# Griffan/FASTQuick

Measured on AMD Instinct MI355X. Metric: paired_150bp_reads_aligned_per_sec, higher is better.
Workload: dtype u32

## Files before the change

### fastquick_amd/csrc/fq_align.cpp

```cpp
#include <algorithm>
#include <atomic>
#include <ctime>
#include <chrono>
#include <climits>
#include <cstdint>
#include <cmath>
#include <cstdio>
#include <cstdlib>
#include <cstring>
#include <memory>
#include <string>
#include <unordered_map>
#include <mutex>
#include <thread>
#include <vector>
#include <pthread.h>
#include <sched.h>

#include "../../include/fastquick_amd.h"
#include "fq_backend.h"
#include "fq_index.h"
#include "fq_pipeline.h"
#include "fq_pool.h"
#include "fq_text_batch.h"

using std::vector;

namespace {
double now_ms() { return std::chrono::duration<double, std::milli>(std::chrono::steady_clock::now().time_since_epoch()).count(); }

int cal_maxdiff(int l, double err, double thres) {
  double elambda = exp(-l * err), sum = elambda, y = 1.0;
  int x = 1;
  for (int k = 1; k < 1000; ++k) {
    y *= l * err;
    x = (int)((unsigned)x * (unsigned)k);
    sum += elambda * y / x;
    if (1.0 - sum < thres) return k;
  }
  return 2;
}
thread_local double tl_grow = 1.0;
struct GrowScope { double prev; explicit GrowScope(double g) : prev(tl_grow) { tl_grow = g; } ~GrowScope() { tl_grow = prev; } };
inline size_t grown(size_t n) { return tl_grow > 1.0 ? (size_t)((double)n * tl_grow * 1.02) : 0; }

struct Retired {
  struct B { void *p; size_t bytes; uint64_t call; bool host; };
  std::vector<B> v;
  uint64_t call = 0;
  static constexpr size_t kRetiredMax = (size_t)6 << 30;
  size_t bytes(bool host) const { size_t t = 0; for (auto &b : v) if (b.host == host) t += b.bytes; return t; }
  void drain() { for (auto &b : v) { if (b.host) fqdev::hfree(b.p); else fqdev::dfree(b.p); } v.clear(); }
  void next_call() { ++call; if (bytes(false) > kRetiredMax || bytes(true) > kRetiredMax / 8) drain(); }
  ~Retired() { drain(); }
};
thread_local Retired *tl_retired = nullptr;
struct RetiredScope { Retired *prev; explicit RetiredScope(Retired *r) : prev(tl_retired) { tl_retired = r; } ~RetiredScope() { tl_retired = prev; } };
inline void retire(void *p, size_t bytes, bool host) {
  if (!p) return;
  if (tl_retired) tl_retired->v.push_back({p, bytes, tl_retired->call, host});
  else if (host) fqdev::hfree(p); else fqdev::dfree(p);
}
inline void *obtain(size_t bytes, bool host, size_t *got) {
  if (tl_retired) {
    int best = -1;
    for (int i = 0; i < (int)tl_retired->v.size(); ++i) {
      const Retired::B &b = tl_retired->v[(size_t)i];
      if (b.host == host && b.call < tl_retired->call && b.bytes >= bytes && b.bytes <= bytes + bytes / 2 && (best < 0 || b.bytes < tl_retired->v[(size_t)best].bytes)) best = i;
    }
    if (best >= 0) { void *q = tl_retired->v[(size_t)best].p; *got = tl_retired->v[(size_t)best].bytes; tl_retired->v.erase(tl_retired->v.begin() + best); return q; }
  }
  void *q = host ? fqdev::hmalloc(bytes) : fqdev::dmalloc(bytes);
  if (!q && tl_retired && !tl_retired->v.empty()) { tl_retired->drain(); q = host ? fqdev::hmalloc(bytes) : fqdev::dmalloc(bytes); }
  *got = bytes;
  return q;
}

template <class T> struct DevBuf {
  T *p = nullptr;
  size_t cap = 0;
  ~DevBuf() { fqdev::dfree(p); }
  bool take(size_t want) { size_t got = 0; p = (T *)obtain(want * sizeof(T), false, &got); cap = p ? got / sizeof(T) : 0; return p != nullptr; }
  static size_t slack(size_t n) { return std::max(std::min<size_t>(n / 4, (size_t)16 << 20), n / 16); }
  bool ensure(size_t n) {
    if (n <= cap) return true;
    retire(p, cap * sizeof(T), false);
    p = nullptr; cap = 0;
    if (const size_t g = grown(n)) { if (take(g + 64)) return true; }
    if (take(n + slack(n) + 64)) return true;
    return take(n);
  }
  bool ensure_roomy(size_t n) {
    if (n <= cap) return true;
    retire(p, cap * sizeof(T), false);
    p = nullptr; cap = 0;
    if (take(std::max(n + n / 8, grown(n)) + 64)) return true;
    if (take(n + n / 8 + 64)) return true;
    return take(n);
  }
  bool ensure_keep(size_t n, size_t keep) {
    if (n <= cap) return true;
    DevBuf<T> q;
    if (!q.take(std::max(n + slack(n), grown(n)) + 64) && !q.take(n + 64)) return false;
    if (keep && (fqdev::d2d(q.p, p, keep * sizeof(T)) || fqdev::sync())) return false;
    retire(p, cap * sizeof(T), false);
    p = q.p; cap = q.cap;
    q.p = nullptr; q.cap = 0;
    return true;
  }
};
}

template <class T> struct PinBuf {
  T *p = nullptr;
  size_t cap = 0;
  ~PinBuf() { fqdev::hfree(p); }
  bool take(size_t want) { size_t got = 0; p = (T *)obtain(want * sizeof(T), true, &got); cap = p ? got / sizeof(T) : 0; return p != nullptr; }
  bool ensure(size_t n) {
    if (n <= cap) return true;
    retire(p, cap * sizeof(T), true);
    p = nullptr; cap = 0;
    if (take(std::max(n + n / 4, grown(n)) + 64)) return true;
    return take(n + 64);
  }
  bool ensure_keep(size_t n, size_t keep) {
    if (n <= cap) return true;
    PinBuf<T> q;
    if (!q.take(std::max(n + n / 4, grown(n)) + 64) && !q.take(n + 64)) return false;
    if (keep) memcpy(q.p, p, keep * sizeof(T));
    retire(p, cap * sizeof(T), true);
    p = q.p; cap = q.cap;
    q.p = nullptr; q.cap = 0;
    return true;
  }
};

struct PinArena {
  struct Block { uint8_t *p; size_t cap; };
  std::vector<Block> blocks;
  size_t used = 0, total = 0;
  double last_grow = 1.0;
  struct Out { void *dst; const void *src; size_t bytes; };
  std::vector<Out> pending;
  ~PinArena() { for (auto &b : blocks) fqdev::hfree(b.p); }
  void reset() {
    pending.clear();
    if (blocks.size() > 1) {
      for (auto &b : blocks) retire(b.p, b.cap, true);
      blocks.clear();
      size_t want = std::max(total + total / 4, (size_t)((double)total * last_grow * 1.02));
      uint8_t *p = (uint8_t *)obtain(want, true, &want);
      if (p) blocks.push_back({p, want});
    }
    used = 0; total = 0; last_grow = tl_grow;
  }
  void *alloc(size_t bytes) {
    bytes = (bytes + 63) & ~(size_t)63;
    total += bytes;
    if (blocks.empty() || used + bytes > blocks.back().cap) {
      size_t cap = std::max<size_t>(std::max(bytes, grown(bytes)), (size_t)4 << 20);
      uint8_t *p = (uint8_t *)obtain(cap, true, &cap);
      if (!p) return nullptr;
      blocks.push_back({p, cap});
      used = 0;
    }
    void *r = blocks.back().p + used;
    used += bytes;
    return r;
  }
};

struct FqKnobs {
  uint32_t gap_long_pops = 256;
  int gap_long_always = 0;
  int64_t gap_skip_bound = -1;
  uint32_t gap_long_pops2 = 0;
  int64_t gap_split_hard = 0;
  int64_t gap_pipeline_min = -1;
  int gap_pipeline_segs = 8;
  int64_t gap_nogap_min = 131072;
  uint32_t gap_pool = 2048;
  int gap_no_order = 0;
  int device_turns = 2;
  int device_turn_slots = 1;
  int64_t device_turn_min = 1 << 20;
  int gap_round2_refill = 16;
  int gap_round1_refill = 0;
  int gap_round2_lane_major = 1;
  int gap_round2_waves = 2560;
  int sw_wave_max = 4096;
  int host_threads = -1;
  size_t host_par_min = 32768;
  int64_t md_mask_min = 4096;
  int64_t packed_bulk_min = -1;
  int trace = 0;
};

struct SearchBufs {
  DevBuf<int32_t> work;
  DevBuf<uint32_t> wfull; DevBuf<FqPos> prec; DevBuf<FqGapWork> winfo; DevBuf<uint8_t> bid_end;
  DevBuf<int32_t> order; DevBuf<uint32_t> order_cnt;
  DevBuf<FqAln> aln; DevBuf<uint32_t> naln, status;
  DevBuf<uint32_t> queue, heads; DevBuf<FqEntry> pool;
};

struct fq_ctx {
  FqWorkPool pool;
  const fq_index *ix = nullptr;
  fq_opts_t o{};
  FqKOpts ko{};
  FqKnobs kn;
  fqdev::State *dev = nullptr;
  int max_pairs = 0;
  int debug = 0;
  std::string err;
  fq_serial_hook before_serial = nullptr, after_serial = nullptr;
  void *hook_user = nullptr;
  bool serial_open = false, serial_done = false;
  bool stream_broken = false;
  uint64_t rng = 0;
  fq_isize_t last_ii{};
  std::unordered_map<uint64_t, vector<uint32_t>> kl_cache;
  int g_log_n[256];
  uint8_t maxdiff_lut[FQ_LMAX + 2];
  int n_pairs = 0, stride = 0;
  int in_kind = 0;
  fq_read_batch_t hb{};
  fq_packed_batch_t pb{};
  const fq_text_batch *tb = nullptr;
  PinBuf<uint8_t> p_cseq, p_cqual;
  PinBuf<int32_t> p_clen;
  PinBuf<char> p_cnames;
  DevBuf<char> d_cnames;
  vector<uint16_t> h_len_all;
  int c_stride = 0, c_name_stride = 0;
  DevBuf<uint64_t> d_head[2];
  DevBuf<uint16_t> d_hlen[2];
  DevBuf<uint8_t> d_qlast[2];
  int head_slot = 0;
  const fq_packed_batch_t *pend[2] = {nullptr, nullptr};
  uint64_t pend_serial[2] = {0, 0};
  bool is_pending(int i, const fq_packed_batch_t *b) const { return pend[i] == b && pend_serial[i] == b->serial; }
  DevBuf<uint8_t> d_body, d_pqual;
  DevBuf<uint64_t> d_exc;
  DevBuf<int32_t> d_row_map, d_crow, d_len_c, d_len_all;
  PinBuf<uint8_t> p_body, p_pqual;
  PinBuf<uint64_t> p_exc;
  PinBuf<uint16_t> p_hlen;
  DevBuf<uint16_t> d_blen;
  DevBuf<uint8_t> d_seq, d_qual, d_filtered, d_maxdiff;
  DevBuf<int32_t> d_len, d_len_trim, d_read_list, d_sidx, d_pair_list, d_counts;
  DevBuf<uint64_t> d_counters;
  std::vector<uint64_t> h_counters;
  SearchBufs sb[2];
  DevBuf<uint32_t> d_seg_cnt;
  DevBuf<FqAln> d_hits;
  DevBuf<uint64_t> d_aoff; DevBuf<uint32_t> d_an;
  DevBuf<uint64_t> d_off;
  DevBuf<FqDRec> d_rec, d_grec;
  DevBuf<uint32_t> d_nocc, d_qfirst, d_cnt[3], d_isz;
  DevBuf<uint16_t> d_ntop;
  DevBuf<uint8_t> d_enum, d_cls;
  DevBuf<uint64_t> d_row0, d_scan[3], d_rng, d_grow0;
  DevBuf<int32_t> d_list, d_refmax;
  DevBuf<fq_multi_t> d_multi, d_omulti;
  DevBuf<FqSwTask> d_swslot; DevBuf<FqSwCand> d_swcand;
  DevBuf<FqPairRead> d_greads; DevBuf<FqPairOut> d_gout;
  DevBuf<FqRefTgt> d_reftgt;
  DevBuf<uint16_t> d_cigs, d_ocig;
  DevBuf<fq_isize_t> d_iis;
  DevBuf<fq_result_t> d_orec;
  DevBuf<char> d_omd;
  PinBuf<fq_result_t> p_orec; PinBuf<uint16_t> p_ocig; PinBuf<char> p_omd; PinBuf<fq_multi_t> p_omulti;
  PinBuf<uint16_t> p_ntop; PinBuf<uint32_t> p_isz; PinBuf<int32_t> p_pairs;
  DevBuf<FqAln> d_qaln;
  DevBuf<uint32_t> d_qlen, d_pos, d_qpos, d_qrow, d_qinfo;
  DevBuf<FqPairIsize> d_pisize; DevBuf<int32_t> d_plut, d_glogn; DevBuf<uint64_t> d_pscratch;
  DevBuf<uint64_t> d_qoff;
  DevBuf<FqSwTask> d_swtask;
  DevBuf<FqSwOut> d_swout;
  DevBuf<FqRefTask> d_reftask;
  DevBuf<FqRefOut> d_refout;
  DevBuf<uint16_t> d_cig, d_cigarena;
  DevBuf<uint8_t> d_scratch;
  DevBuf<char> d_md;
  DevBuf<uint16_t> d_mdmask;
  vector<uint8_t> h_filtered;
  vector<int32_t> h_len_trim, h_sub_max;
  const int32_t *h_pair_list = nullptr;
  const FqSurvInfo *h_surv = nullptr;
  Retired retired;
  PinArena arena;
  PinBuf<int32_t> p_i32;
  PinBuf<FqSurvInfo> p_surv;
  PinBuf<uint32_t> p_u32a, p_u32b, p_pos;
  PinBuf<FqAln> p_aln;
  DevBuf<FqSurvInfo> d_surv;
  DevBuf<int32_t> d_sub_max;
  int64_t n_bases_in = 0;
  int emit_flags = 0;
  bool host_rows = true;
  DevBuf<uint8_t> d_equal; PinBuf<uint8_t> p_equal;
  DevBuf<char> d_enames; PinBuf<char> p_enames;
  DevBuf<uint32_t> d_samlen, d_sammeta; DevBuf<uint64_t> d_samoff; DevBuf<char> d_samtext;
  uint64_t sam_bytes = 0;
  bool sam_ready = false;
  fqdev::State *dev_emit[2] = {nullptr, nullptr};
  PinBuf<char> p_emit[2][2];
  fq_bam *bam = nullptr;
  DevBuf<uint32_t> d_bamlen, d_bammeta, d_zsize; DevBuf<uint64_t> d_bamoff, d_zoff; DevBuf<uint8_t> d_bamrec, d_zstage, d_bamz;
  FqBamCallOut bam_out;
  PinBuf<uint64_t> p_ztotal;
  uint32_t emit_nb = 0;
  std::mutex emit_mu;
  bool emit_pending = false;
  fq_qc *qc = nullptr;
  DevBuf<int32_t> d_qadded;
  DevBuf<uint32_t> d_istlen, d_ptcnt;
  DevBuf<uint64_t> d_istoff, d_ptoff, d_qcnt, d_dupkey;
  DevBuf<char> d_isttext; DevBuf<FqPileEntry> d_pile;
  PinBuf<uint64_t> p_qcnt, p_dupkey;
  FqQcCallOut qc_out;
  FqBatchState st;
  struct CallVecs {
    std::vector<int32_t> work, next_work;
  } cv;
  fq_stats_t stats{};
  double wait_ms = 0;
  ~fq_ctx();
};

extern "C" void fq_default_opts(fq_opts_t *o) {
  memset(o, 0, sizeof *o);
  o->s_mm = 3; o->s_gapo = 11; o->s_gape = 4;
  o->mode = FQ_MODE_GAPE | FQ_MODE_COMPREAD;
  o->indel_end_skip = 5; o->max_del_occ = 10; o->max_entries = 2000000;
  o->fnr = 0.02; o->max_diff = -1; o->max_gapo = 1; o->max_gape = 6;
  o->max_seed_diff = 2; o->seed_len = 32; o->max_top2 = 30; o->trim_qual = 0; o->filter_thresh = 3;
  o->max_isize = 500; o->force_isize = 0; o->max_occ = 100000; o->n_multi = 3; o->N_multi = 10; o->is_sw = 1;
  o->ap_prior = 1e-5; o->host_threads = 0; o->batch_pairs = 262144; o->single_end = 0; o->pad_opts = 0;
}

extern "C" const char *fq_version(void) { return "fastquick_amd 0.1 (gfx950)"; }
extern "C" const char *fq_ctx_last_error(const fq_ctx_t *c) { return c ? c->err.c_str() : "null context"; }

extern "C" int fq_ctx_create(const fq_index_t *ix, const fq_opts_t *opts, int32_t max_pairs, fq_ctx_t **out) {
  if (!ix || !opts || !out || max_pairs <= 0) return FQ_EINVAL;
  *out = nullptr;
  const fq_opts_t &o = *opts;
  if (o.max_gapo < 0 || o.max_gapo > 3 || o.max_gape < 0 || o.max_gape > 15 || o.seed_len < 1 || o.seed_len > FQ_SEED_MAX) return FQ_EINVAL;
  if (o.s_mm <= 0 || o.s_gapo <= 0 || o.s_gape <= 0) return FQ_EINVAL;
  if (o.fnr <= 0.0 && (o.max_diff < 0 || o.max_diff > 30)) return FQ_EINVAL;
  if (o.batch_pairs < 1) return FQ_EINVAL;
  if (o.max_seed_diff < 0 || o.max_seed_diff > 30) return FQ_EINVAL;
  if (o.max_entries < 1 || o.max_entries > (1 << 30)) return FQ_EINVAL;
  if (o.max_occ > (1u << 30) || o.n_multi < 0 || o.N_multi < 0 || o.n_multi > 4096 || o.N_multi > 4096) return FQ_EINVAL;
  std::unique_ptr<fq_ctx> c(new fq_ctx);
  c->ix = ix; c->o = o; c->max_pairs = max_pairs;
  int md_max = 0;
  for (int l = 0; l <= FQ_LMAX; ++l) {
    int md = o.fnr > 0.0 ? cal_maxdiff(l, 0.02, o.fnr) : o.max_diff;
    if (md > 30) return FQ_EINVAL;
    c->maxdiff_lut[l] = (uint8_t)md;
    md_max = std::max(md_max, md);
  }
  if ((md_max + 1) * o.s_mm + o.max_gapo * o.s_gapo + o.max_gape * o.s_gape >= FQ_MAX_BUCKETS) return FQ_EINVAL;
  if (o.max_gapo > c->maxdiff_lut[FQ_LMIN]) return FQ_EINVAL;
  c->g_log_n[0] = 0;
  for (int i = 1; i < 256; ++i) c->g_log_n[i] = (int)(4.343 * log(i) + 0.5);
  c->rng = ((uint64_t)ix->seed << 16) | 0x330EULL;
  c->last_ii.avg = -1.0;
  FqKOpts &k = c->ko;
  k.s_mm = o.s_mm; k.s_gapo = o.s_gapo; k.s_gape = o.s_gape; k.mode = o.mode;
  k.indel_end_skip = o.indel_end_skip; k.max_del_occ = o.max_del_occ; k.max_entries = o.max_entries;
  k.max_gapo = o.max_gapo; k.max_gape = o.max_gape; k.max_seed_diff = o.max_seed_diff; k.seed_len = o.seed_len;
  k.max_top2 = o.max_top2; k.trim_qual = o.trim_qual; k.filter_thresh = o.filter_thresh; k.n_buckets = FQ_MAX_BUCKETS;
  if (const char *e = getenv("FASTQUICK_CTX_TRACE")) c->kn.trace = atoi(e);
  c->dev = fqdev::state_create(ix->device);
  if (!c->dev || fqdev::bind(c->dev)) return FQ_ENODEV;
  if (!c->d_maxdiff.ensure(FQ_LMAX + 2) || !c->d_counters.ensure(FQ_C_STRIPES * FQ_C_STRIDE) || !c->d_counts.ensure(4) || !c->sb[0].queue.ensure(4) || !c->d_glogn.ensure(256)) return FQ_ENOMEM;
  if (fqdev::h2d(c->d_maxdiff.p, c->maxdiff_lut, FQ_LMAX + 2) || fqdev::h2d(c->d_glogn.p, c->g_log_n, 256 * 4) || fqdev::dzero(c->d_counters.p, (size_t)FQ_C_STRIPES * FQ_C_STRIDE * 8) || fqdev::sync()) return FQ_ENODEV;
  *out = c.release();
  return FQ_OK;
}
fq_ctx::~fq_ctx() { for (auto *e : dev_emit) if (e) fqdev::state_destroy(e); fqdev::state_destroy(dev); }
extern "C" void fq_ctx_destroy(fq_ctx_t *c) { delete c; }

extern "C" int fq_ctx_set_tuning(fq_ctx_t *c, const char *key, int64_t v) {
  if (!c || !key) return FQ_EINVAL;
  const std::string k = key;
  fqdev::Tune *t = fqdev::tune(c->dev);
  if (k == "gap_long_pops") c->kn.gap_long_pops = (uint32_t)v;
  else if (k == "gap_long_always") c->kn.gap_long_always = (int)v;
  else if (k == "gap_pool") c->kn.gap_pool = (uint32_t)v;
  else if (k == "gap_nogap_min") c->kn.gap_nogap_min = v;
  else if (k == "gap_pipeline_min") c->kn.gap_pipeline_min = v;
  else if (k == "gap_pipeline_segs") c->kn.gap_pipeline_segs = (int)std::max<int64_t>(2, std::min<int64_t>(v, 64));
  else if (k == "gap_split_hard") c->kn.gap_split_hard = v;
  else if (k == "gap_long_pops2") c->kn.gap_long_pops2 = (uint32_t)v;
  else if (k == "gap_skip_bound") c->kn.gap_skip_bound = v;
  else if (k == "gap_no_order") c->kn.gap_no_order = (int)v;
  else if (k == "device_turns") c->kn.device_turns = (int)v;
  else if (k == "device_turn_min") c->kn.device_turn_min = v;
  else if (k == "device_turn_slots") c->kn.device_turn_slots = (int)std::max<int64_t>(1, v);
  else if (k == "gap_round2_waves") c->kn.gap_round2_waves = (int)v;
  else if (k == "gap_round2_lane_major") c->kn.gap_round2_lane_major = (int)v;
  else if (k == "gap_round1_refill") c->kn.gap_round1_refill = (int)v;
  else if (k == "gap_round2_refill") c->kn.gap_round2_refill = (int)v;
  else if (k == "sw_wave_max") c->kn.sw_wave_max = (int)v;
  else if (k == "host_threads") c->kn.host_threads = (int)v;
  else if (k == "host_par_min") c->kn.host_par_min = (size_t)v;
  else if (k == "packed_bulk_min") c->kn.packed_bulk_min = v;
  else if (k == "md_mask_min") c->kn.md_mask_min = v;
  else if (k == "trace") c->kn.trace = (int)v;
  else if (k == "gap_order_asc") t->gap_order_asc = (int)v;
  else if (k == "gap_waves_per_cu") t->gap_waves_per_cu = (int)v;
  else if (k == "gap_coop_waves") t->gap_coop_waves = (int)v;
  else if (k == "gap_refill_min") t->gap_refill_min = (int)v;
  else if (k == "filter_no_turns") t->filter_no_turns = (int)v;
  else if (k == "prep_priority") t->prep_priority = (int)v;
  else if (k == "refine_lanes") t->refine_lanes = (int)v;
  else if (k == "gap_generic_opts") t->gap_generic_opts = (int)v;
  else if (k == "sw_serial_reverse") t->sw_serial_reverse = (int)v;
  else if (k == "width_both_strands") t->width_both_strands = (int)v;
  else if (k == "spin_sync") t->spin_sync = (int)v;
  else return FQ_EINVAL;
  return FQ_OK;
}

extern "C" void fq_stats_get(const fq_ctx_t *c, fq_stats_t *out) { if (c && out) *out = c->stats; }
extern "C" void fq_stats_reset(fq_ctx_t *c) { if (c) memset(&c->stats, 0, sizeof c->stats); }

#define CK(expr)                                                  \
  do {                                                            \
    if ((expr)) { c->err = std::string(#expr) + ": " + fqdev::last_error(); return FQ_ENODEV; } \
  } while (0)
#define CKM(expr)                                                 \
  do {                                                            \
    if (!(expr)) { c->err = std::string("out of device memory: ") + #expr; return FQ_ENOMEM; } \
  } while (0)

static int h2d_staged(fq_ctx *c, void *dst, const void *src, size_t bytes) {
  if (!bytes) return 0;
  void *p = c->arena.alloc(bytes);
  if (!p) { c->err = "out of pinned host memory"; return FQ_ENOMEM; }
  memcpy(p, src, bytes);
  if (fqdev::copy_pinned(dst, p, bytes, 1)) { c->err = std::string("h2d: ") + fqdev::last_error(); return FQ_ENODEV; }
  return 0;
}
static int d2h_staged(fq_ctx *c, void *dst, const void *src, size_t bytes) {
  if (!bytes) return 0;
  void *p = c->arena.alloc(bytes);
  if (!p) { c->err = "out of pinned host memory"; return FQ_ENOMEM; }
  if (fqdev::copy_pinned(p, src, bytes, 0)) { c->err = std::string("d2h: ") + fqdev::last_error(); return FQ_ENODEV; }
  c->arena.pending.push_back({dst, p, bytes});
  return 0;
}
static int sync_staged(fq_ctx *c) {
  const double t_wait = now_ms();
  if (fqdev::sync()) { c->err = std::string("sync: ") + fqdev::last_error(); return FQ_ENODEV; }
  c->wait_ms += now_ms() - t_wait;
  for (auto &o : c->arena.pending) memcpy(o.dst, o.src, o.bytes);
  c->arena.pending.clear();
  return 0;
}
static void fold_counters(const uint64_t *striped, uint64_t *cnt) {
  for (int k = 0; k < FQ_C_COUNT; ++k) {
    const bool is_max = k == FQ_C_MAXPOPS || k == FQ_C_MAXTRIPS;
    uint64_t v = 0;
    for (int st = 0; st < FQ_C_STRIPES; ++st) { const uint64_t x = striped[(size_t)st * FQ_C_STRIDE + k]; v = is_max ? std::max(v, x) : v + x; }
    cnt[k] = v;
  }
}
#define CKS(expr) do { const int rc_ = (expr); if (rc_) return rc_; } while (0)
static void dp_take(fq_ctx *c) {
  for (int v = 0; v < FQ_DP_COUNT; ++v) { c->stats.dp_launches[v] += fqdev::dp_launches[v]; fqdev::dp_launches[v] = 0; }
}
static int refuse_length(fq_ctx *c) { c->err = "read length outside [" + std::to_string(FQ_LMIN) + "," + std::to_string(FQ_LMAX) + "]"; return FQ_ELIMIT; }

extern "C" int fq_batch_upload(fq_ctx_t *c, const fq_read_batch_t *in) {
  if (!c || !in || in->n_pairs < 0 || !in->seq || !in->qual || !in->len) return FQ_EINVAL;
  if (in->n_pairs > c->max_pairs) { c->err = "batch larger than max_pairs_per_batch"; return FQ_ELIMIT; }
  if (fqdev::bind(c->dev)) return FQ_ENODEV;
  if (in->stride < 1 || in->stride > 4096) return FQ_EINVAL;
  const size_t n2 = (size_t)in->n_pairs * (c->o.single_end ? 1 : 2);
  int64_t nb = 0;
  for (size_t i = 0; i < n2; ++i) nb += in->len[i];
  c->n_bases_in = nb;
  for (size_t i = 0; i < n2; ++i)
    if (in->len[i] < FQ_LMIN || in->len[i] > FQ_LMAX || in->len[i] > in->stride) return refuse_length(c);
  CKM(c->d_seq.ensure((size_t)in->n_pairs * 2 * in->stride + 64));
  CKM(c->d_qual.ensure((size_t)in->n_pairs * 2 * in->stride + 64));
  CKM(c->d_len.ensure((size_t)in->n_pairs * 2 + 1));
  CK(fqdev::h2d(c->d_seq.p, in->seq, n2 * in->stride));
  CK(fqdev::h2d(c->d_qual.p, in->qual, n2 * in->stride));
  CK(fqdev::h2d(c->d_len.p, in->len, n2 * 4));
  CK(fqdev::sync());
// ... 160 lines not shown
  ii->std = sqrt(ii->std / n);
  double y;
  for (y = 1.0; y < 10.0; y += 0.01) if (.5 * erfc(y / M_SQRT2) < ap_prior / L * (y * ii->std + ii->avg)) break;
  ii->high_bayesian = (uint32_t)(y * ii->std + ii->avg + .499);
  uint64_t n_ap = 0;
  for (int i = 0; i < tot; ++i) if (is[i] > ii->high_bayesian) ++n_ap;
  ii->ap_prior = .01 * (n_ap + .01) / tot;
  if (ii->ap_prior < ap_prior) ii->ap_prior = ap_prior;
  if (std::isnan(ii->std) || p75 > 100000) { ii->low = ii->high = ii->high_bayesian = 0; ii->avg = ii->std = -1.0; }
}

void pair_penalty_lut(const fq_isize_t &ii, vector<int32_t> &lut) {
  if (!ii.high) return;
  for (uint32_t l = 0; l <= ii.high_bayesian; ++l) {
    const double v = -4.343 * log(0.5 * erfc(M_SQRT1_2 * fabs(l - ii.avg) / ii.std)) + 0.499;
    lut.push_back(v >= 2147483648.0 || v != v ? INT32_MIN : (int32_t)v);
  }
}
}

namespace {
struct EmitPlan {
  FqSamArgs sam{}; FqBamArgs bam{}; FqQcArgs qc{};
  uint64_t sam_total = 0, bam_total = 0, ist_total = 0, pt_total = 0;
};
struct Call {
  fq_ctx *c;
  EmitPlan plan_emit;
  fq_qc *gate = nullptr; uint64_t gate_ticket = 0; bool gate_entered = false, gate_left = false;
  void gate_take(fq_qc *q) { if (q) { gate = q; gate_ticket = fq_qc_gate_ticket(q); } }
  void gate_enter() { if (gate && !gate_entered) { fq_qc_gate_enter(gate, gate_ticket); gate_entered = true; } }
  void gate_leave() { if (gate && gate_entered && !gate_left) { fq_qc_gate_leave(gate); gate_left = true; } }
  void gate_release() { if (gate && !gate_left) { gate_enter(); gate_leave(); } }
  explicit Call(fq_ctx *ctx) : c(ctx), aln_off(ctx->st.aln_off), aln_n(ctx->st.aln_n) {}
  int n = 0, n2 = 0, B = 0, n_sub = 0, n_search = 0, n_surv = 0, max_len_all = 1, host_threads = 1;
  size_t par_min = 32768;
  const uint8_t *dseq = nullptr;
  int dstride = 0;
  const int32_t *dlen_trim = nullptr, *dread_list = nullptr;
  FqSamArgs emit{};
  bool emit_ready = false;
  vector<int> sub_max_len, sub_lo;
  vector<int32_t> sub_whole;
  vector<uint64_t> &aln_off;
  vector<uint32_t> &aln_n;
  FqRecArgs ra{};
  uint64_t n_q = 0, n_rows = 0;
  const uint32_t *h_pos = nullptr;
  bool have_pos = false;
  vector<fq_isize_t> iis;
  vector<FqPairIsize> pis;
  vector<int32_t> lut;
  int64_t n_host_pairs = 0;
  const int32_t *host_list = nullptr;
  const FqPairRead *host_reads = nullptr;
  const uint64_t *host_row0 = nullptr;
  uint64_t n_multi = 0, n_sw = 0, n_ref = 0, cig_used = 0;
  struct B1Plan { uint64_t *start = nullptr; size_t n_chunks = 0; uint64_t rng_end = 0; } plan;
  std::thread plan_thread;
  ~Call() { if (plan_thread.joinable()) plan_thread.join(); gate_release(); }
  double t_trace = 0, t_wall0 = 0, t_host0 = 0, t_serial1 = 0, t_host1 = 0, cpu_trace = 0, tcpu_trace = 0, w_trace = 0;
  double w_call0 = 0, w_host0 = 0, w_serial1 = 0, w_host1 = 0, cpu_call0 = 0;
  int sidx(size_t idx) const { return c->h_surv[idx].sidx; }
  const FqAln *aln_of(size_t idx, int *n_out) const {
    const int s = sidx(idx);
    if (s < 0) { *n_out = 0; return nullptr; }
    *n_out = (int)aln_n[s];
    return c->st.aln.data() + aln_off[s];
  }
  void trace(const char *label) {
    if (!c->kn.trace) return;
    const double t = now_ms();
    timespec ts;
    clock_gettime(CLOCK_PROCESS_CPUTIME_ID, &ts);
    const double cpu = 1e3 * (double)ts.tv_sec + 1e-6 * (double)ts.tv_nsec;
    clock_gettime(CLOCK_THREAD_CPUTIME_ID, &ts);
    const double tcpu = 1e3 * (double)ts.tv_sec + 1e-6 * (double)ts.tv_nsec;
    fprintf(stderr, "[fq] %-22s %8.3f ms   cpu %8.1f core-ms   this thread %6.3f ms   waited for the device %6.3f ms\n", label, t - t_trace, cpu - cpu_trace, tcpu - tcpu_trace, c->wait_ms - w_trace);
    t_trace = t; cpu_trace = cpu; tcpu_trace = tcpu; w_trace = c->wait_ms;
  }
};

struct FilterIn {
  const uint64_t *head = nullptr;
  const uint16_t *len = nullptr;
  const uint8_t *qual_last = nullptr;
  int uniform_len = 0;
  int body_stride = 0;
  const fq_text_batch *text = nullptr;
};

int stage0_filter(Call &K, const FilterIn &in) {
  fq_ctx *c = K.c;
  const int n = K.n, n2 = K.n2, n_sub = K.n_sub, B = K.B;
  const bool ascii = !in.head, se = c->o.single_end != 0, ragged = !ascii && in.uniform_len <= 0;
  const int n_in = se ? n : n2;
  const size_t n_max = (size_t)(ascii ? 1 : 3) * n_sub;
  CKM(c->d_filtered.ensure(n2 + 64) && c->d_read_list.ensure(n2) && c->d_sidx.ensure(n2) && c->d_pair_list.ensure(n) && c->d_sub_max.ensure(n_max) && (!ascii || c->d_len_trim.ensure(n2)));
  CK(fqdev::dzero(c->d_sub_max.p, n_max * 4));
  if (se) CK(fqdev::dfill(c->d_filtered.p + n, 1, (size_t)n));
  if (se && ascii) CK(fqdev::dzero(c->d_len_trim.p + n, (size_t)n * 4));
  fqdev::time_begin(FQ_K_PREP);
  if (ascii) {
    FqPrepArgs a{};
    a.ix = c->ix->dev; a.o = c->ko; a.seq = c->d_seq.p; a.qual = c->d_qual.p; a.len = c->d_len.p; a.stride = c->stride; a.n_reads = n_in;
    a.len_trim = c->d_len_trim.p; a.filtered = c->d_filtered.p; a.sub_max = c->d_sub_max.p; a.n_pairs = n; a.batch_pairs = B; a.counters = c->d_counters.p;
    CK(fqdev::launch_prep(a));
  } else {
    FqPrepPackedArgs a{};
    a.ix = c->ix->dev; a.o = c->ko; a.head = in.head; a.len = ragged ? in.len : nullptr; a.uniform_len = in.uniform_len; a.qual_last = in.qual_last; a.sub_whole = c->d_sub_max.p + n_sub;
    a.n_reads = n_in; a.filtered = c->d_filtered.p; a.sub_max = c->d_sub_max.p; a.n_pairs = n; a.batch_pairs = B; a.counters = c->d_counters.p;
    CK(fqdev::launch_prep_packed(a));
  }
  CK(fqdev::launch_compact(c->d_filtered.p, n, c->d_read_list.p, c->d_sidx.p, c->d_pair_list.p, c->d_counts.p));
  fqdev::time_end(FQ_K_PREP);
  int32_t counts[2] = {0, 0};
  c->h_sub_max.assign(n_sub, in.uniform_len);
  K.sub_whole.assign(n_sub, 0);
  std::vector<uint64_t> striped(ragged ? (size_t)FQ_C_STRIPES * FQ_C_STRIDE : 0);
  CKS(d2h_staged(c, counts, c->d_counts.p, 8));
  if (in.qual_last) CKS(d2h_staged(c, K.sub_whole.data(), c->d_sub_max.p + n_sub, (size_t)n_sub * 4));
  if (ascii || ragged) CKS(d2h_staged(c, c->h_sub_max.data(), c->d_sub_max.p, (size_t)n_sub * 4));
  if (ragged) CKS(d2h_staged(c, striped.data(), c->d_counters.p, striped.size() * 8));
  CKS(sync_staged(c));
  K.trace("  stage0: filter + compaction on the device");
  if (ragged) {
    uint64_t folded[FQ_C_COUNT];
    fold_counters(striped.data(), folded);
    if (folded[FQ_C_BADLEN]) return refuse_length(c);
    for (int sb = 0; in.body_stride && sb < n_sub; ++sb)
      if (((int64_t)c->h_sub_max[sb] + 3) / 4 > (int64_t)in.body_stride) { c->err = "a read is longer than body_stride holds"; return FQ_EINVAL; }
    c->n_bases_in = (int64_t)folded[FQ_C_BASES];
  } else if (!ascii) c->n_bases_in = (int64_t)n_in * in.uniform_len;
  K.n_search = counts[0]; K.n_surv = counts[1];
  K.dstride = ascii ? c->stride : (std::max(1, *std::max_element(c->h_sub_max.begin(), c->h_sub_max.end())) + 15) & ~15;
  return FQ_OK;
}

int stage0_debug_fetch(fq_ctx *c, int n2, const int32_t *d_len_all) {
  c->h_filtered.clear(); c->h_len_trim.clear();
  if (!c->debug) return FQ_OK;
  c->h_filtered.resize(n2);
  CKS(d2h_staged(c, c->h_filtered.data(), c->d_filtered.p, n2));
  if (d_len_all) { c->h_len_trim.resize(n2); CKS(d2h_staged(c, c->h_len_trim.data(), d_len_all, (size_t)n2 * 4)); }
  return FQ_OK;
}
int stage0_survivors(Call &K, bool compact, int32_t *crow) {
  fq_ctx *c = K.c;
  const int n_surv = K.n_surv;
  const size_t nrow = (size_t)n_surv * 2;
  CKM(c->d_surv.ensure(nrow + 1));
  if (compact) {
    CKM(c->d_row_map.ensure(nrow + 1) && c->d_len_c.ensure(nrow + 1) && c->d_len_trim.ensure(nrow + 1));
    CK(fqdev::launch_surv_map(c->d_pair_list.p, n_surv, K.n, c->d_filtered.p, c->d_sidx.p, c->d_surv.p, c->d_row_map.p, c->d_read_list.p, crow));
  } else CK(fqdev::launch_surv_gather(c->d_pair_list.p, n_surv, K.n, c->d_len_trim.p, c->d_filtered.p, c->d_sidx.p, c->d_surv.p));
  if (!compact) CKS(stage0_debug_fetch(c, K.n2, c->d_len_trim.p));
  CKM(c->p_pairs.ensure((size_t)n_surv + 1) && c->p_surv.ensure(nrow + 1));
  CK(fqdev::copy_pinned(c->p_pairs.p, c->d_pair_list.p, (size_t)n_surv * 4, 0));
  CK(fqdev::copy_pinned(c->p_surv.p, c->d_surv.p, nrow * sizeof(FqSurvInfo), 0));
  CKS(sync_staged(c));
  c->stats.d2h_bytes += (size_t)n_surv * (4 + 2 * sizeof(FqSurvInfo));
  c->h_pair_list = c->p_pairs.p; c->h_surv = c->p_surv.p;
  K.sub_lo.assign(K.n_sub + 1, 0);
  for (int sb = 0; sb <= K.n_sub; ++sb)
    K.sub_lo[sb] = (int)(std::lower_bound(c->h_pair_list, c->h_pair_list + n_surv, (int32_t)std::min<int64_t>((int64_t)sb * K.B, INT32_MAX)) - c->h_pair_list);
  K.sub_lo[K.n_sub] = n_surv;
  K.trace("  stage0: survivors' lists D2H");
  return FQ_OK;
}

FqTrimArgs stage0_trim_args(const Call &K, const uint8_t *qual, int qual_stride, const int32_t *row_map) {
  fq_ctx *c = K.c;
  FqTrimArgs ta{};
  ta.o = c->ko; ta.qual = qual; ta.qual_stride = qual_stride; ta.row_map = row_map; ta.len = c->d_len_c.p; ta.n_rows = 2 * K.n_surv; ta.len_trim = c->d_len_trim.p;
  ta.pair_list = c->d_pair_list.p; ta.batch_pairs = K.B; ta.sub_max = c->d_sub_max.p + 2 * K.n_sub;
  return ta;
}

int head_upload(fq_ctx *c, const fq_packed_batch_t *b, int slot) {
  const size_t n2 = (size_t)b->n_pairs * (b->single_end ? 1 : 2);
  CKM(c->d_head[slot].ensure(n2 * 3 + 8));
  CK(fqdev::h2d_copy(c->d_head[slot].p, b->head, n2 * 24));
  c->stats.h2d_bytes += n2 * 24;
  if (!b->uniform_len) {
    CKM(c->d_hlen[slot].ensure(n2 + 8));
    CK(fqdev::h2d_copy(c->d_hlen[slot].p, b->len, n2 * 2));
    c->stats.h2d_bytes += n2 * 2;
  }
  if (c->o.trim_qual >= 1 && b->qual_last) {
    CKM(c->d_qlast[slot].ensure(n2 + 8));
    CK(fqdev::h2d_copy(c->d_qlast[slot].p, b->qual_last, n2));
    c->stats.h2d_bytes += n2;
  }
  CK(fqdev::copy_record(slot));
  return FQ_OK;
}
int stage0_rows_packed(Call &K, bool bulk) {
  fq_ctx *c = K.c;
  const fq_packed_batch_t &pb = c->pb;
  const int n = K.n, n2 = K.n2, nrow = 2 * K.n_surv, body_stride = pb.body_stride, cstride = K.dstride;
  const bool se = c->o.single_end != 0, ragged = pb.uniform_len <= 0, trim = c->o.trim_qual >= 1;
  CKM(c->d_seq.ensure((size_t)nrow * cstride + 64));
  FqUnpackArgs ua{};
  ua.body_stride = body_stride; ua.uniform_len = pb.uniform_len; ua.n_rows = nrow; ua.seq = c->d_seq.p; ua.stride = cstride;
  ua.len_out = c->d_len_c.p; ua.len_trim = c->d_len_trim.p;
  FqPatchArgs pa{};
  pa.seq = c->d_seq.p; pa.stride = cstride;
  FqTrimArgs ta = stage0_trim_args(K, nullptr, pb.qual_stride, nullptr);
  if (nrow && bulk) {
    CKM(c->d_body.ensure((size_t)n2 * body_stride + 64));
    CK(fqdev::h2d(c->d_body.p, pb.body, (size_t)n2 * body_stride));
    c->stats.h2d_bytes += (size_t)n2 * body_stride;
    ua.body = c->d_body.p; ua.row_map = c->d_row_map.p;
    if (ragged) ua.len = c->d_hlen[c->head_slot].p;
    if (pb.n_exc) {
      CKM(c->d_exc.ensure((size_t)pb.n_exc + 1));
      CK(fqdev::h2d(c->d_exc.p, pb.exc, (size_t)pb.n_exc * 8));
      c->stats.h2d_bytes += (size_t)pb.n_exc * 8;
      pa.exc = c->d_exc.p; pa.n_exc = pb.n_exc; pa.crow_of = c->d_crow.p;
    }
    if (trim) {
      CKM(c->d_pqual.ensure((size_t)n2 * pb.qual_stride + 64));
      CK(fqdev::h2d(c->d_pqual.p, pb.qual, (size_t)n2 * pb.qual_stride));
      c->stats.h2d_bytes += (size_t)n2 * pb.qual_stride;
      ta.qual = c->d_pqual.p; ta.row_map = c->d_row_map.p;
    }
  } else if (nrow) {
    CKM(c->p_body.ensure((size_t)nrow * body_stride + 64) && c->d_body.ensure((size_t)nrow * body_stride + 64));
    const bool row_lens = ragged || se;
    if (row_lens) CKM(c->p_hlen.ensure((size_t)nrow + 8) && c->d_blen.ensure((size_t)nrow + 8));
    if (trim) CKM(c->p_pqual.ensure((size_t)nrow * pb.qual_stride + 64) && c->d_pqual.ensure((size_t)nrow * pb.qual_stride + 64));
    size_t ne = 0;
    vector<std::pair<size_t, size_t>> erange;
    if (pb.n_exc) erange.resize(nrow);
    for (int t = 0; t < nrow; ++t) {
      const size_t r = (size_t)(t & 1) * (size_t)n + (size_t)c->h_pair_list[t >> 1];
      if (se && (t & 1)) {
        memset(c->p_body.p + (size_t)t * body_stride, 0, (size_t)body_stride);
        c->p_hlen.p[t] = 0;
        if (trim) memset(c->p_pqual.p + (size_t)t * pb.qual_stride, 0, (size_t)pb.qual_stride);
        if (pb.n_exc) erange[t] = {0, 0};
        continue;
      }
      memcpy(c->p_body.p + (size_t)t * body_stride, pb.body + r * (size_t)body_stride, (size_t)body_stride);
      if (row_lens) c->p_hlen.p[t] = ragged ? pb.len[r] : (uint16_t)pb.uniform_len;
      if (trim) memcpy(c->p_pqual.p + (size_t)t * pb.qual_stride, pb.qual + r * (size_t)pb.qual_stride, (size_t)pb.qual_stride);
      if (pb.n_exc) {
        const uint64_t *lo = std::lower_bound(pb.exc, pb.exc + pb.n_exc, (uint64_t)r << 32);
        const uint64_t *hi = std::lower_bound(lo, pb.exc + pb.n_exc, (uint64_t)(r + 1) << 32);
        erange[t] = {(size_t)(lo - pb.exc), (size_t)(hi - pb.exc)};
        ne += (size_t)(hi - lo);
      }
    }
    CK(fqdev::copy_pinned(c->d_body.p, c->p_body.p, (size_t)nrow * body_stride, 1));
    c->stats.h2d_bytes += (size_t)nrow * body_stride;
    ua.body = c->d_body.p; ua.row_map = nullptr;
    if (row_lens) { CK(fqdev::copy_pinned(c->d_blen.p, c->p_hlen.p, (size_t)nrow * 2, 1)); ua.len = c->d_blen.p; c->stats.h2d_bytes += (size_t)nrow * 2; }
    if (ne) {
      CKM(c->p_exc.ensure(ne + 1) && c->d_exc.ensure(ne + 1));
      size_t at = 0;
      for (int t = 0; t < nrow; ++t)
        for (size_t q = erange[t].first; q < erange[t].second; ++q) c->p_exc.p[at++] = ((uint64_t)t << 32) | (pb.exc[q] & 0xffffffffull);
      CK(fqdev::copy_pinned(c->d_exc.p, c->p_exc.p, ne * 8, 1));
      c->stats.h2d_bytes += ne * 8;
      pa.exc = c->d_exc.p; pa.n_exc = (int64_t)ne; pa.crow_of = nullptr;
    }
    if (trim) {
      CK(fqdev::copy_pinned(c->d_pqual.p, c->p_pqual.p, (size_t)nrow * pb.qual_stride, 1));
      c->stats.h2d_bytes += (size_t)nrow * pb.qual_stride;
      ta.qual = c->d_pqual.p; ta.row_map = nullptr;
    }
  }
  fqdev::time_begin(FQ_K_PREP);
  if (nrow) {
    CK(fqdev::launch_unpack(ua));
    if (pa.n_exc) CK(fqdev::launch_patch(pa));
    if (trim) CK(fqdev::launch_trim(ta));
  }
  fqdev::time_end(FQ_K_PREP);
  return FQ_OK;
}

int stage0_rows_text(Call &K) {
  fq_ctx *c = K.c;
  const fq_text_batch &tb = *c->tb;
  const int nrow = 2 * K.n_surv, ns = tb.name_stride, cstride = K.dstride;
  c->c_stride = cstride; c->c_name_stride = ns;
  CKM(c->d_seq.ensure((size_t)nrow * cstride + 64) && c->d_pqual.ensure((size_t)nrow * cstride + 64) && c->d_cnames.ensure((size_t)nrow * ns + 64));
  const bool host_rows = !(c->emit_flags & FQ_EMIT_DEVICE_ONLY) || c->debug;
  c->host_rows = host_rows;
  if (host_rows) CKM(c->p_cseq.ensure((size_t)nrow * cstride + 64) && c->p_cqual.ensure((size_t)nrow * cstride + 64) && c->p_clen.ensure((size_t)nrow + 8) && c->p_cnames.ensure((size_t)nrow * ns + 64));
  fqdev::time_begin(FQ_K_PREP);
  if (nrow) {
    FqTextGatherArgs g{};
    g.text[0] = tb.d_text[0]; g.text[1] = tb.d_text[1]; g.rec = tb.d_rec; g.names = tb.d_names; g.name_stride = ns; g.n_pairs = K.n; g.single_end = c->o.single_end ? 1 : 0;
    g.pair_list = c->d_pair_list.p; g.n_out = nrow; g.seq = c->d_seq.p; g.qual = c->d_pqual.p; g.stride = cstride;
    g.len_out = c->d_len_c.p; g.len_trim = c->d_len_trim.p; g.names_out = c->d_cnames.p;
    CK(fqdev::launch_text_gather(g));
    if (c->o.trim_qual >= 1) CK(fqdev::launch_trim(stage0_trim_args(K, c->d_pqual.p, cstride, nullptr)));
    if (host_rows) {
      CK(fqdev::copy_pinned(c->p_cseq.p, c->d_seq.p, (size_t)nrow * cstride, 0));
      CK(fqdev::copy_pinned(c->p_cqual.p, c->d_pqual.p, (size_t)nrow * cstride, 0));
      CK(fqdev::copy_pinned(c->p_clen.p, c->d_len_c.p, (size_t)nrow * 4, 0));
      CK(fqdev::copy_pinned(c->p_cnames.p, c->d_cnames.p, (size_t)nrow * ns, 0));
      c->stats.d2h_bytes += (size_t)nrow * (2 * (size_t)cstride + 4 + (size_t)ns);
    }
  }
  fqdev::time_end(FQ_K_PREP);
  return FQ_OK;
}

int stage0_whole_batch(Call &K, const FilterIn &in) {
  fq_ctx *c = K.c;
  const fq_text_batch *tb = in.text;
  const int n = K.n, n2 = K.n2, n_sub = K.n_sub, nrow = 2 * K.n_surv;
  const bool se = c->o.single_end != 0, ragged = in.uniform_len <= 0, trim = c->o.trim_qual >= 1;
  const int n_in = se ? n : n2;
  bool need_all = trim && (tb || c->debug);
  if (trim && !tb) {
    vector<int32_t> surv_max(n_sub, 0);
    if (nrow) {
      CKS(d2h_staged(c, surv_max.data(), c->d_sub_max.p + 2 * n_sub, (size_t)n_sub * 4));
      CKS(sync_staged(c));
      c->stats.d2h_bytes += (size_t)n_sub * 4;
    }
    for (int sb = 0; sb < n_sub; ++sb) {
      surv_max[sb] = std::max(surv_max[sb], K.sub_whole[sb]);
      if (surv_max[sb] < c->h_sub_max[sb]) need_all = true;
    }
    if (!need_all) c->h_sub_max = surv_max;
  }
  if (need_all) {
    CKM(c->d_len_all.ensure(n2));
    if (!tb) {
      CKM(c->d_pqual.ensure((size_t)n_in * c->pb.qual_stride + 64));
      CK(fqdev::h2d(c->d_pqual.p, c->pb.qual, (size_t)n_in * c->pb.qual_stride));
      c->stats.h2d_bytes += (size_t)n_in * c->pb.qual_stride;
    }
    CK(fqdev::dzero(c->d_sub_max.p, (size_t)n_sub * 4));
    if (se) CK(fqdev::dzero(c->d_len_all.p + n, (size_t)n * 4));
    if (tb) {
      FqTextTrimArgs aa{};
      aa.o = c->ko; aa.text[0] = tb->d_text[0]; aa.text[1] = tb->d_text[1]; aa.rec = tb->d_rec; aa.n_rows = n_in; aa.n_pairs = n; aa.batch_pairs = K.B;
      aa.len_trim = c->d_len_all.p; aa.sub_max = c->d_sub_max.p;
      CK(fqdev::launch_text_trim_all(aa));
    } else {
      FqTrimAllArgs aa{};
      aa.o = c->ko; aa.qual = c->d_pqual.p; aa.qual_stride = c->pb.qual_stride; aa.len = ragged ? in.len : nullptr; aa.uniform_len = in.uniform_len;
      aa.n_reads = n_in; aa.n_pairs = n; aa.batch_pairs = K.B; aa.len_trim = c->d_len_all.p; aa.sub_max = c->d_sub_max.p;
      CK(fqdev::launch_trim_all(aa));
    }
    CKS(d2h_staged(c, c->h_sub_max.data(), c->d_sub_max.p, (size_t)n_sub * 4));
  }
  CKS(stage0_debug_fetch(c, n2, need_all ? c->d_len_all.p : nullptr));
  if (tb) c->h_len_all.clear();
  if (tb && c->debug) { c->h_len_all.assign(n2, 0); CKS(d2h_staged(c, c->h_len_all.data(), tb->d_hlen, (size_t)n_in * 2)); }
  if (need_all || c->debug || tb) CKS(sync_staged(c));
  if (c->debug && c->h_len_trim.empty()) {
    c->h_len_trim.resize(n2);
    for (int r = 0; r < n2; ++r) c->h_len_trim[r] = r >= n_in ? 0 : tb ? (int)c->h_len_all[r] : ragged ? (int)c->pb.len[r] : in.uniform_len;
  }
  return FQ_OK;
}

void stage0_finish(Call &K) {
  fq_ctx *c = K.c;
  K.max_len_all = 1;
  K.sub_max_len.assign(K.n_sub, 1);
  for (int sb = 0; sb < K.n_sub; ++sb) {
    K.sub_max_len[sb] = std::max(1, c->h_sub_max[sb]);
    K.max_len_all = std::max(K.max_len_all, K.sub_max_len[sb]);
  }
  K.dseq = c->d_seq.p; K.dlen_trim = c->d_len_trim.p; K.dread_list = c->d_read_list.p;
}

int stage0_ascii(Call &K) {
  CKS(stage0_filter(K, FilterIn{}));
  CKS(stage0_survivors(K, false, nullptr));
  stage0_finish(K);
  return FQ_OK;
}
int stage0_packed(Call &K) {
  fq_ctx *c = K.c;
  const fq_packed_batch_t &pb = c->pb;
  const int slot = c->head_slot;
  CK(fqdev::compute_wait_copy(slot));
  FilterIn in;
  in.head = c->d_head[slot].p; in.len = c->d_hlen[slot].p; in.uniform_len = pb.uniform_len; in.body_stride = pb.body_stride;
  in.qual_last = c->o.trim_qual >= 1 && pb.qual_last ? c->d_qlast[slot].p : nullptr;
  CKS(stage0_filter(K, in));
  const int64_t bulk_min = c->kn.packed_bulk_min >= 0 ? c->kn.packed_bulk_min : (int64_t)K.n / 8;
  const bool bulk = !c->o.single_end && K.n_surv > 0 && (int64_t)K.n_surv >= bulk_min;
  const bool need_crow = bulk && pb.n_exc > 0;
  if (need_crow) { CKM(c->d_crow.ensure(K.n2)); CK(fqdev::dfill(c->d_crow.p, 0xff, (size_t)K.n2 * 4)); }
  CKS(stage0_survivors(K, true, need_crow ? c->d_crow.p : nullptr));
  CKS(stage0_rows_packed(K, bulk));
  CKS(stage0_whole_batch(K, in));
  stage0_finish(K);
  return FQ_OK;
}
int stage0_text(Call &K) {
  fq_ctx *c = K.c;
  FilterIn in;
  in.head = c->tb->d_head; in.len = c->tb->d_hlen; in.uniform_len = c->tb->uniform_len; in.text = c->tb;
  CKS(stage0_filter(K, in));
  CKS(stage0_survivors(K, true, nullptr));
  CKS(stage0_rows_text(K));
  CKS(stage0_whole_batch(K, in));
  K.trace("  stage0: rows, qualities, names gathered");
  stage0_finish(K);
  return FQ_OK;
}

struct Turn { int slots = 1; bool held = false; void take() { if (!held) { fqdev::device_turn_begin(slots); held = true; } } void drop() { if (held) { fqdev::device_turn_end(); held = false; } } ~Turn() { drop(); } };
struct SearchGeom { int Lpad, Ppad, nb_need; };

bool search_bufs_ensure(SearchBufs &b, size_t nw, const SearchGeom &g, uint32_t aln_cap) {
  return b.work.ensure(nw) && b.wfull.ensure(nw * 2 * g.Lpad) && b.prec.ensure(nw * 2 * g.Ppad) && b.winfo.ensure(nw) && b.bid_end.ensure(nw * 2) && b.order.ensure(nw) &&
         b.order_cnt.ensure(2 * FQ_ORDER_KEYS + 2) && b.aln.ensure(nw * aln_cap) && b.naln.ensure(nw) && b.status.ensure(nw);
}
int launch_widths(Call &K, SearchBufs &b, const SearchGeom &g, const int32_t *d_work, int nw, int n_hard) {
  fq_ctx *c = K.c;
  FqWidthArgs wa{};
  wa.ix = c->ix->dev; wa.o = c->ko; wa.seq = K.dseq; wa.stride = K.dstride; wa.len_trim = K.dlen_trim; wa.read_list = K.dread_list;
  wa.work = d_work; wa.n_work = nw; wa.wfull = b.wfull.p; wa.wstride = g.Lpad;
  wa.prec = b.prec.p; wa.pstride = g.Ppad; wa.winfo = b.winfo.p; wa.maxdiff_lut = c->d_maxdiff.p; wa.bid_end = b.bid_end.p; wa.counters = c->d_counters.p;
  CK(fqdev::launch_width(wa));
  CK(fqdev::launch_order(b.bid_end.p, nw, n_hard, b.order.p, b.order_cnt.p));
  return FQ_OK;
}
FqGapArgs gap_args(fq_ctx *c, const SearchBufs &b, const SearchGeom &g, const FqGapTier &T, int nw) {
  FqGapArgs ga{};
  ga.ix = c->ix->dev; ga.o = c->ko; ga.o.n_buckets = g.nb_need; ga.n_work = nw; ga.winfo = b.winfo.p;
  ga.order = c->kn.gap_no_order ? nullptr : b.order.p; ga.split = c->kn.gap_no_order ? nullptr : b.order_cnt.p + 2 * FQ_ORDER_KEYS;
  ga.wfull = b.wfull.p; ga.wstride = g.Lpad; ga.prec = b.prec.p; ga.pstride = g.Ppad;
  ga.pool = b.pool.p; ga.heads = b.heads.p; ga.tier = T; ga.aln = b.aln.p; ga.n_aln = b.naln.p; ga.status = b.status.p;
  ga.counters = c->d_counters.p; ga.queue = b.queue.p;
  return ga;
}

struct HitLists { const uint32_t *status; uint64_t total; };
int collect_hits(Call &K, SearchBufs &b, const int32_t *wk, int nw, uint32_t aln_cap, bool room_later, Turn *turn, uint8_t *h_bid, HitLists *out) {
  fq_ctx *c = K.c;
  CK(fqdev::launch_scan(b.naln.p, c->d_off.p, (uint32_t)nw));
  CKM(c->p_u32a.ensure((size_t)nw + 2) && c->p_u32b.ensure((size_t)nw + 2));
  uint32_t *h_status = c->p_u32a.p, *h_naln = c->p_u32b.p;
  CK(fqdev::copy_pinned(h_status, b.status.p, (size_t)nw * 4, 0));
  CK(fqdev::copy_pinned(h_naln, b.naln.p, (size_t)nw * 4, 0));
  uint64_t *h_off = (uint64_t *)c->arena.alloc(((size_t)nw + 1) * 8);
  if (!h_off) { c->err = "out of pinned host memory"; return FQ_ENOMEM; }
  CK(fqdev::copy_pinned(h_off, c->d_off.p, ((size_t)nw + 1) * 8, 0));
  if (h_bid) CKS(d2h_staged(c, h_bid, b.bid_end.p, (size_t)nw * 2));
  CKS(sync_staged(c));
  if (turn) turn->drop();
  K.trace("  A: width + search kernels, counts D2H");
  const uint64_t total = h_off[nw], base = c->st.aln.n;
  const uint64_t hits_need = base + total + 1, hits_room = room_later ? hits_need + hits_need / 2 : hits_need;
  CKM(c->d_hits.ensure_keep(c->d_hits.cap >= hits_need ? hits_need : hits_room, base) && c->p_aln.ensure_keep(c->p_aln.cap >= hits_need ? hits_need : hits_room, base));
  CK(fqdev::launch_pack_aln(b.aln.p, b.naln.p, c->d_off.p, aln_cap, (uint32_t)nw, c->d_hits.p + base));
  CK(fqdev::launch_aln_index(b.work.p, b.status.p, c->d_off.p, b.naln.p, base, c->d_aoff.p, c->d_an.p, nw));
  CK(fqdev::copy_pinned(c->p_aln.p + base, c->d_hits.p + base, total * sizeof(FqAln), 0));
  CKS(sync_staged(c));
  c->st.aln.p = c->p_aln.p; c->st.aln.n = base + total;
  K.trace("  A: hit lists D2H");
  parallel_chunks((size_t)nw, K.host_threads, K.par_min, [&](size_t lo, size_t hi, int) {
    for (size_t w = lo; w < hi; ++w) {
      if (h_status[w]) continue;
      const int s = wk[w];
      K.aln_off[s] = base + h_off[w];
      K.aln_n[s] = h_naln[w];
    }
  });
  *out = {h_status, total};
  return FQ_OK;
}

int search_pipelined(Call &K, const SearchGeom &g, FqGapArgs ga, int nw, const FqGapTier &T2, uint32_t *n2, bool *piped) {
  fq_ctx *c = K.c;
  SearchBufs &b1 = c->sb[0], &b2 = c->sb[1];
  const int S = c->kn.gap_pipeline_segs;
  const size_t cap2 = std::max<size_t>(65536, (size_t)nw / 4);
  const size_t slots2 = (size_t)fqdev::gap_lane_slots(gap_args(c, b2, g, T2, (int32_t)cap2));
  *piped = search_bufs_ensure(b2, cap2, g, T2.aln_cap) && c->d_seg_cnt.ensure((size_t)S + 1) && b2.queue.ensure(4) && b2.heads.ensure(slots2 * FQ_MAX_BUCKETS) && b2.pool.ensure(slots2 * T2.pool_cap);
  if (!*piped) return FQ_OK;
  uint32_t n2_total = 0;
  CK(fqdev::dzero(c->d_seg_cnt.p, ((size_t)S + 1) * 4));
  fqdev::time_begin(FQ_K_GAP);
  bool room = true;
// ... 100 lines not shown
        ga.max_waves = waves / 2;
      }
      ga.pool = b.pool.p; ga.heads = b.heads.p;
      if (big_call) turn.take();
      uint32_t n2_total = 0;
      bool piped = false;
      const FqGapTier T2 = [&] { FqGapTier t = lane_tier; t.long_pops = 0; return t; }();
      if (T.nogap && c0 == 0 && (size_t)nw == work.size() && c->kn.gap_pipeline_min >= 0 && (int64_t)nw >= c->kn.gap_pipeline_min && nw >= 64 * c->kn.gap_pipeline_segs)
        CKS(search_pipelined(K, g, ga, nw, T2, &n2_total, &piped));
      if (!piped) {
        fqdev::time_begin(FQ_K_GAP);
        CK(fqdev::launch_gap(ga));
        fqdev::time_end(FQ_K_GAP);
      }
      vector<uint8_t> h_bid;
      if (T.nogap && c->kn.gap_split_hard > 0) h_bid.resize((size_t)nw * 2);
      HitLists h;
      CKS(collect_hits(K, b, wk, nw, T.aln_cap, true, &turn, h_bid.empty() ? nullptr : h_bid.data(), &h));
      c->stats.d2h_bytes += (size_t)nw * 8 + h.total * sizeof(FqAln);
      if (!h_bid.empty()) {
        bound_of.assign(n_search, 0);
        for (int w = 0; w < nw; ++w) bound_of[wk[w]] = std::min(h_bid[2 * w], h_bid[2 * w + 1]);
      }
      vector<char> in_round2;
      vector<int32_t> list2;
      if (n2_total) {
        list2.resize(n2_total);
        CKS(d2h_staged(c, list2.data(), c->sb[1].work.p, (size_t)n2_total * 4));
        CKS(sync_staged(c));
        in_round2.assign((size_t)n_search, 0);
        for (int32_t sidx : list2) in_round2[sidx] = 1;
      }
      {
        const int TT = std::max(1, K.host_threads);
        vector<vector<int32_t>> left((size_t)TT), left_easy((size_t)TT);
        vector<uint64_t> n_left((size_t)TT * 8, 0);
        const bool by_class = T.nogap != 0;
        parallel_chunks((size_t)nw, TT, K.par_min, [&](size_t lo, size_t hi, int t) {
          for (size_t w = lo; w < hi; ++w)
            if (h.status[w]) {
              ++n_left[(size_t)t * 8];
              if (in_round2.empty() || !in_round2[wk[w]]) (by_class && !(h.status[w] & FQ_SF_NOHIT) ? left_easy[t] : left[t]).push_back(wk[w]);
            }
        });
        for (int t = 0; t < TT; ++t) {
          c->stats.tier_retries += n_left[(size_t)t * 8];
          next_work.insert(next_work.end(), left[t].begin(), left[t].end());
          next_easy.insert(next_easy.end(), left_easy[t].begin(), left_easy[t].end());
        }
      }
      if (n2_total) {
        HitLists h2;
        CKS(collect_hits(K, c->sb[1], list2.data(), (int)n2_total, T2.aln_cap, false, nullptr, nullptr, &h2));
        c->stats.d2h_bytes += (size_t)n2_total * 20 + h2.total * sizeof(FqAln);
        for (uint32_t t = 0; t < n2_total; ++t)
          if (h2.status[t]) { next_work.push_back(list2[t]); ++c->stats.tier_retries; }
      }
    }
    n_hard = T.nogap ? next_work.size() : 0;
    next_work.insert(next_work.end(), next_easy.begin(), next_easy.end());
    work.swap(next_work);
    K.trace("  A: round bookkeeping");
  }
  if (!work.empty()) { c->err = "gap search: exact tier exhausted its pool (internal limit)"; return FQ_ELIMIT; }
  c->stats.reads_searched += n_search;
  return FQ_OK;
}

#define REC(op, n) CK(fqdev::launch_rec((op), K.ra, (int64_t)(n)))
static int fetch_u64(fq_ctx *c, uint64_t *dst, const uint64_t *src) { return d2h_staged(c, dst, src, 8); }

int stage_records(Call &K) {
  fq_ctx *c = K.c;
  const fq_opts_t &o = c->o;
  const int n_surv = K.n_surv;
  const size_t N = (size_t)n_surv * 2;
  FqRecArgs &A = K.ra;
  CKM(c->d_rec.ensure(N + 1) && c->d_nocc.ensure(N + 1) && c->d_ntop.ensure(N + 1) && c->d_enum.ensure(N + 1) && c->d_qfirst.ensure(N + 1) && c->d_row0.ensure(N + 1) &&
      c->d_cls.ensure((size_t)n_surv + 1) && c->d_isz.ensure((size_t)n_surv + 1) && c->d_cigs.ensure(64));
  for (int k = 0; k < 3; ++k) CKM(c->d_cnt[k].ensure(N + 1) && c->d_scan[k].ensure(N + 2));
  A.ix = c->ix->dev; A.n_surv = n_surv; A.n_pairs = K.n; A.batch_pairs = K.B; A.packed = c->in_kind >= 2 ? 1 : 0 ; A.single_end = o.single_end ? 1 : 0;
  A.max_occ = o.max_occ; A.multi_cap = o.single_end ? 4u : (uint32_t)std::max(o.n_multi, o.N_multi) + 1;
  A.n_multi = o.n_multi; A.N_multi = o.N_multi; A.max_isize = o.max_isize; A.s_mm = o.s_mm; A.is_sw = o.is_sw;
  A.pair_list = c->d_pair_list.p; A.surv = c->d_surv.p; A.len_trim = K.dlen_trim; A.full_len = A.packed ? c->d_len_c.p : c->d_len.p;
  A.hits = c->d_hits.p; A.aoff = c->d_aoff.p; A.an = c->d_an.p; A.maxdiff_lut = c->d_maxdiff.p; A.g_log_n = c->d_glogn.p;
  A.rec = c->d_rec.p; A.nocc = c->d_nocc.p; A.ntop = c->d_ntop.p; A.enumerated = c->d_enum.p; A.qfirst = c->d_qfirst.p; A.row0 = c->d_row0.p;
  A.pq_cnt = c->d_cnt[0].p; A.prow_cnt = c->d_cnt[1].p; A.pq = c->d_scan[0].p; A.prow = c->d_scan[1].p;
  A.counters = c->d_counters.p; A.cigs = c->d_cigs.p;
  REC(FQ_ROP_INIT, N);
  REC(FQ_ROP_NOCC, N);
  REC(FQ_ROP_ENUM_PLAN, n_surv);
  CK(fqdev::launch_scan(c->d_cnt[0].p, c->d_scan[0].p, (uint32_t)n_surv));
  CK(fqdev::launch_scan(c->d_cnt[1].p, c->d_scan[1].p, (uint32_t)n_surv));
  CKM(c->p_ntop.ensure(N + 1));
  CK(fqdev::copy_pinned(c->p_ntop.p, c->d_ntop.p, N * 2, 0));
  uint64_t tot[2] = {0, 0};
  CKS(fetch_u64(c, &tot[0], c->d_scan[0].p + n_surv));
  CKS(fetch_u64(c, &tot[1], c->d_scan[1].p + n_surv));
  CKS(sync_staged(c));
  c->stats.d2h_bytes += N * 2 + 16;
  K.n_q = tot[0]; K.n_rows = tot[1];
  if (K.n_q > 0xfffffff0ull) { c->err = "more than 2^32 hits to enumerate in one call"; return FQ_ELIMIT; }
  return FQ_OK;
}

int stage_sa_rows(Call &K) {
  fq_ctx *c = K.c;
  FqRecArgs &A = K.ra;
  const uint64_t n_q = K.n_q, rows = K.n_rows;
  CKM(c->d_qaln.ensure(n_q + 1) && c->d_qlen.ensure(n_q + 1) && c->d_qoff.ensure(n_q + 2) && c->d_pos.ensure(rows + 1) && c->d_pscratch.ensure(rows + 1));
  A.qaln = c->d_qaln.p; A.qlen = c->d_qlen.p; A.qoff = c->d_qoff.p; A.n_q = n_q; A.n_rows = rows; A.pos = c->d_pos.p; A.pscratch = c->d_pscratch.p;
  REC(FQ_ROP_ENUM_FILL, K.n_surv);
  if (rows) {
    FqSaArgs sa{};
    sa.ix = c->ix->dev; sa.aln = c->d_qaln.p; sa.aln_len = c->d_qlen.p; sa.row_off = c->d_qoff.p; sa.n_aln = (uint32_t)n_q;
    sa.n_rows = rows; sa.pos = c->d_pos.p; sa.counters = c->d_counters.p;
    fqdev::time_begin(FQ_K_SA);
    CK(fqdev::launch_sa(sa));
    fqdev::time_end(FQ_K_SA);
    c->stats.sa_rows += rows;
  }
  return FQ_OK;
}

struct Lcg48 { uint64_t a, c; };
static constexpr uint64_t kM48 = 0xFFFFFFFFFFFFULL;
static inline Lcg48 lcg_then(const Lcg48 &f, const Lcg48 &g) { return {(g.a * f.a) & kM48, (g.a * f.c + g.c) & kM48}; }
static Lcg48 lcg_pow(uint64_t n) {
  Lcg48 r{1, 0}, b{0x5DEECE66DULL, 0xBULL};
  for (; n; n >>= 1) { if (n & 1) r = lcg_then(r, b); b = lcg_then(b, b); }
  return r;
}
static uint64_t steps_to_zero(uint64_t x) {
  uint64_t n = 0;
  for (int k = 1; k <= 48; ++k) {
    const Lcg48 p = lcg_pow(n);
    const uint64_t xn = (p.a * x + p.c) & kM48;
    if (xn & ((1ULL << k) - 1)) n |= 1ULL << (k - 1);
  }
  const Lcg48 p = lcg_pow(n);
  if (((p.a * x + p.c) & kM48) != 0) return 0;
  return n ? n : (1ULL << 48);
}
void stageB1_plan(Call &K, uint64_t rng0) {
  fq_ctx *c = K.c;
  const size_t N = (size_t)K.n_surv * 2;
  const uint16_t *ntop = c->p_ntop.p;
  uint64_t *start = K.plan.start;
  const size_t per = 2 * FQ_RNG_CHUNK_PAIRS;
  constexpr uint64_t A1 = 0x5DEECE66DULL, C1 = 0xBULL, M48 = kM48, A2 = (A1 * A1) & M48, C2 = (A1 * C1 + C1) & M48;
  const Lcg48 jump = lcg_pow(2 * per);
  uint64_t to_zero = steps_to_zero(rng0);
  const bool can_jump = to_zero != 0 && per == 32;
  uint64_t x = rng0;
  auto advanced = [&](uint64_t steps) { if (to_zero) to_zero = to_zero > steps ? to_zero - steps : to_zero + (1ULL << 48) - steps; };
  for (size_t c0 = 0; c0 < N; c0 += per) {
    start[c0 / per] = x;
    const size_t c1 = std::min(N, c0 + per);
    if (can_jump && c1 - c0 == per && to_zero > 2 * per) {
      uint64_t w[8];
      memcpy(w, ntop + c0, 64);
      bool ones = true;
      for (int q = 0; q < 8; ++q) ones &= w[q] == 0x0001000100010001ULL;
      if (ones) { x = (jump.a * x + jump.c) & M48; advanced(2 * per); continue; }
    }
    for (size_t idx = c0; idx < c1; ++idx) {
      const int t = ntop[idx];
// ... 382 lines not shown
}

int snapshot_records(Call &K, vector<FqRead> &dst) {
  fq_ctx *c = K.c;
  const size_t N = (size_t)K.n_surv * 2;
  vector<FqDRec> rec(N);
  vector<fq_multi_t> multi((size_t)K.n_multi);
  vector<uint16_t> cigs((size_t)K.cig_used);
  CKS(d2h_staged(c, rec.data(), c->d_rec.p, N * sizeof(FqDRec)));
  CKS(d2h_staged(c, multi.data(), c->d_multi.p, multi.size() * sizeof(fq_multi_t)));
  CKS(d2h_staged(c, cigs.data(), c->d_cigs.p, cigs.size() * 2));
  CKS(sync_staged(c));
  dst.assign(N, FqRead());
  for (size_t i = 0; i < N; ++i) {
    const FqDRec &s = rec[i];
    FqRead &p = dst[i];
    p.r = (int)(i & 1) * K.n + c->h_pair_list[i >> 1];
    p.score = s.score; p.sa = s.sa; p.pos = s.pos; p.c1 = s.c1; p.c2 = s.c2; p.len = s.len; p.full_len = s.full_len; p.clip_len = s.clip_len;
    p.nm = (int16_t)s.nm; p.filtered = s.filtered; p.type = s.type; p.strand = s.strand; p.extra_flag = s.extra_flag;
    p.n_mm = s.n_mm; p.n_gapo = s.n_gapo; p.n_gape = s.n_gape; p.mapQ = s.mapQ; p.seQ = s.seQ; p.revived = s.revived != 0;
    p.cigar.assign(cigs.data() + (s.n_cigar ? s.cig_off : 0), cigs.data() + (s.n_cigar ? s.cig_off : 0) + s.n_cigar);
    for (uint32_t j = 0; j < s.n_multi; ++j) {
      const fq_multi_t &m = multi[s.multi_off + j];
      FqMulti q;
      q.pos = m.pos; q.gap = m.gap; q.mm = m.mm; q.strand = m.strand;
      if (m.n_cigar) q.cigar.assign(cigs.data() + m.cigar_off, cigs.data() + m.cigar_off + m.n_cigar);
      p.multi.push_back(q);
    }
  }
  return FQ_OK;
}

int emit_reads(Call &K, const uint8_t **qual, int *qual_stride, const char **names, int *name_stride) {
  fq_ctx *c = K.c;
  const size_t N = (size_t)K.n_surv * 2;
  if (c->in_kind == 3) { *qual = c->d_pqual.p; *qual_stride = c->c_stride; *names = c->d_cnames.p; *name_stride = c->c_name_stride; return FQ_OK; }
  const FqHostReads hb = fq_ctx_host_reads(c);
  if (N && !hb.has_qual()) { c->err = "SAM text on the device: the batch carries no qualities"; return FQ_EINVAL; }
  const int n = K.n;
  const bool se = c->o.single_end != 0;
  int max_len = 1, max_name = 1;
  std::vector<int> tl((size_t)std::max(1, K.host_threads), 1), tn((size_t)std::max(1, K.host_threads), 1);
  parallel_chunks(N, K.host_threads, K.par_min, [&](size_t lo, size_t hi, int t) {
    int ml = 1, mn = 1;
    for (size_t i = lo; i < hi; ++i) {
      const int e = (int)(i & 1), pair = c->h_pair_list[i >> 1];
      if (se && e) continue;
      ml = std::max(ml, hb.len((size_t)e * n + pair));
      if (hb.has_names()) mn = std::max(mn, (int)strnlen(hb.name_of(pair, e), (size_t)hb.name_stride));
    }
    tl[(size_t)t] = ml; tn[(size_t)t] = mn;
  });
  for (size_t t = 0; t < tl.size(); ++t) { max_len = std::max(max_len, tl[t]); max_name = std::max(max_name, tn[t]); }
  const int qs = (max_len + 15) & ~15, ns = (max_name + 1 + 7) & ~7;
  CKM(c->p_equal.ensure(N * qs + 64) && c->d_equal.ensure(N * qs + 64) && c->p_enames.ensure(N * ns + 64) && c->d_enames.ensure(N * ns + 64));
  parallel_chunks(N, K.host_threads, K.par_min, [&](size_t lo, size_t hi, int) {
    for (size_t i = lo; i < hi; ++i) {
      const int e = (int)(i & 1), pair = c->h_pair_list[i >> 1];
      uint8_t *q = c->p_equal.p + i * (size_t)qs;
      char *nm = c->p_enames.p + i * (size_t)ns;
      memset(nm, 0, (size_t)ns);
      if (se && e) { memset(q, 0, (size_t)qs); continue; }
      const size_t r = (size_t)e * n + pair;
      const int l = hb.len(r);
      memcpy(q, hb.qual(r), (size_t)l);
      memset(q + l, 0, (size_t)(qs - l));
      if (hb.has_names()) { const char *src = hb.name_of(pair, e); memcpy(nm, src, strnlen(src, (size_t)hb.name_stride)); }
      else nm[0] = '*';
    }
  });
  CK(fqdev::copy_pinned(c->d_equal.p, c->p_equal.p, N * qs, 1));
  CK(fqdev::copy_pinned(c->d_enames.p, c->p_enames.p, N * ns, 1));
  c->stats.h2d_bytes += N * ((size_t)qs + (size_t)ns);
  *qual = c->d_equal.p; *qual_stride = qs; *names = c->d_enames.p; *name_stride = ns;
  return FQ_OK;
}
int emit_args(Call &K, FqSamArgs &a) {
  fq_ctx *c = K.c;
  if (!K.emit_ready) {
    FqSamArgs &e = K.emit;
    e = FqSamArgs{};
    e.cg = c->ix->dev_contigs;
    e.n_surv = K.n_surv; e.n_pairs = K.n; e.packed = K.ra.packed; e.single_end = c->o.single_end; e.mode = c->o.mode; e.max_top2 = c->o.max_top2;
    e.pair_list = c->d_pair_list.p;
    e.rec = c->d_orec.p; e.cigar = c->d_ocig.p; e.md = c->d_omd.p; e.multi = c->d_omulti.p;
    e.seq = K.ra.seq; e.stride = K.ra.stride;
    CKS(emit_reads(K, &e.qual, &e.qual_stride, &e.names, &e.name_stride));
    K.emit_ready = true;
  }
  a = K.emit;
  return FQ_OK;
}
int emit_measure(Call &K) {
  fq_ctx *c = K.c;
  const size_t N = (size_t)K.n_surv * 2, P = (size_t)K.n_surv;
  EmitPlan &E = K.plan_emit;
  E = EmitPlan();
  c->sam_bytes = 0; c->sam_ready = false;
  c->bam_out = FqBamCallOut(); c->bam_out.owner = c->bam;
  c->qc_out = FqQcCallOut(); c->qc_out.owner = c->qc; c->qc_out.n_surv = K.n_surv;
  if (!N) return FQ_OK;
  if (c->emit_flags & FQ_EMIT_SAM) {
    CKS(emit_args(K, E.sam));
    CKM(c->d_samlen.ensure(N + 1) && c->d_samoff.ensure(N + 2) && c->d_sammeta.ensure(N + 1));
    E.sam.len = c->d_samlen.p; E.sam.off = c->d_samoff.p; E.sam.meta = c->d_sammeta.p;
    CK(fqdev::launch_sam(FQ_EOP_SAM_LEN, E.sam, (int64_t)N));
    CK(fqdev::launch_scan(c->d_samlen.p, c->d_samoff.p, (uint32_t)N));
    CKS(fetch_u64(c, &E.sam_total, c->d_samoff.p + N));
  }
  if (c->bam) {
    CKS(emit_args(K, E.bam.s));
    { const int rc = fq_bam_device_prepare(c->bam, &E.bam); if (rc) { c->err = "the BAM writer could not stage its tables on the device"; return rc; } }
    CKM(c->d_bamlen.ensure(N + 1) && c->d_bamoff.ensure(N + 2) && c->d_bammeta.ensure(N + 1));
    E.bam.len = c->d_bamlen.p; E.bam.off = c->d_bamoff.p; E.bam.meta = c->d_bammeta.p; E.bam.split = 1;
    CK(fqdev::launch_bam(FQ_EOP_BAM_LEN, E.bam, (int64_t)N));
    CK(fqdev::launch_scan(c->d_bamlen.p, c->d_bamoff.p, (uint32_t)N));
    CKS(fetch_u64(c, &E.bam_total, c->d_bamoff.p + N));
  }
  if (c->qc) {
    FqQcArgs &a = E.qc;
    CKS(emit_args(K, a.s));
    a.ix = c->ix->dev;
    K.gate_enter();
    { const int rc = fq_qc_device_prepare(c->qc, &a, K.n_surv); if (rc) { c->err = std::string("the QC consumer could not take the call: ") + fq_qc_last_error(c->qc); return rc; } }
    const size_t NC = (size_t)FQ_C_STRIPES * FQ_C_STRIDE;
    CKM(c->d_qadded.ensure(N + 1) && c->d_istlen.ensure(P + 1) && c->d_istoff.ensure(P + 2) && c->d_ptcnt.ensure(N + 1) && c->d_ptoff.ensure(N + 2) && c->d_qcnt.ensure(NC) && c->p_qcnt.ensure(NC));
    if (a.shard) { CKM(c->d_dupkey.ensure(P + 1) && c->p_dupkey.ensure(P + 1)); }
    CK(fqdev::dzero(c->d_qcnt.p, NC * 8));
    a.counters = c->d_qcnt.p; a.added = c->d_qadded.p; a.ist_len = c->d_istlen.p; a.ist_off = c->d_istoff.p; a.pt_cnt = c->d_ptcnt.p; a.pt_off = c->d_ptoff.p;
    a.dup_key = a.shard ? c->d_dupkey.p : nullptr;
    CK(fqdev::launch_qc(FQ_QOP_PAIR, a, (int64_t)P));
    CK(fqdev::launch_scan(c->d_istlen.p, c->d_istoff.p, (uint32_t)P));
    CK(fqdev::launch_scan(c->d_ptcnt.p, c->d_ptoff.p, (uint32_t)N));
    CKS(fetch_u64(c, &E.ist_total, c->d_istoff.p + P));
    CKS(fetch_u64(c, &E.pt_total, c->d_ptoff.p + N));
  }
  CKS(sync_staged(c));
  K.gate_leave();
  K.trace("consumers: lengths, decisions, prefix sums");
  return FQ_OK;
}
int emit_fill(Call &K) {
  fq_ctx *c = K.c;
  const size_t N = (size_t)K.n_surv * 2, P = (size_t)K.n_surv;
  EmitPlan &E = K.plan_emit;
  if (!N) {
    if (c->emit_flags & FQ_EMIT_SAM) c->sam_ready = true;
    c->bam_out.ready = c->bam != nullptr; c->qc_out.ready = c->qc != nullptr;
    return FQ_OK;
  }
  std::lock_guard<std::mutex> lk(c->emit_mu);
  if (c->emit_flags & FQ_EMIT_SAM) {
    CKM(c->d_samtext.ensure_roomy(E.sam_total + 64));
    E.sam.text = c->d_samtext.p;
    static const bool body_split = [] { const char *e = getenv("FASTQUICK_SAM_BODY"); return !(e && *e == '0'); }();
    E.sam.split = body_split ? 1 : 0;
    CK(fqdev::launch_sam(FQ_EOP_SAM_FILL, E.sam, (int64_t)N));
    if (body_split) CK(fqdev::launch_sam(FQ_EOP_SAM_BODY, E.sam, (int64_t)N));
    c->sam_bytes = E.sam_total;
    c->sam_ready = true;
  }
  if (c->bam) {
    const uint64_t total = E.bam_total;
    CKM(c->d_bamrec.ensure_roomy(total + 64));
    E.bam.out = c->d_bamrec.p;
    CK(fqdev::launch_bam(FQ_EOP_BAM_FILL, E.bam, (int64_t)N));
    CK(fqdev::launch_bam(FQ_EOP_BAM_BODY, E.bam, (int64_t)N));
// ... 32 lines not shown
  static const bool emit_sync = [] { const char *e = getenv("FASTQUICK_EMIT_SYNC"); return e && *e && *e != '0'; }();
  if (emit_sync) CKS(sync_staged(c));
  K.trace("consumers: fill kernels enqueued");
  return FQ_OK;
}

int stage_finish(Call &K, fq_result_batch_t *out) {
  fq_ctx *c = K.c;
  FqBatchState &S = c->st;
  FqRecArgs &A = K.ra;
  const int n_sub = K.n_sub, n_surv = K.n_surv;
  const size_t N = (size_t)n_surv * 2;
  S.isize_sub = K.iis;
  S.isize = K.iis[n_sub - 1];
  uint64_t cc = 0, mm = 0, xx = 0;
  if (N) {
    A.fc_cnt = c->d_cnt[0].p; A.fm_cnt = c->d_cnt[1].p; A.fx_cnt = c->d_cnt[2].p;
    A.fc_off = c->d_scan[0].p; A.fm_off = c->d_scan[1].p; A.fx_off = c->d_scan[2].p;
    REC(FQ_ROP_FLAT_COUNT, N);
    for (int k = 0; k < 3; ++k) CK(fqdev::launch_scan(c->d_cnt[k].p, c->d_scan[k].p, (uint32_t)N));
    CKS(fetch_u64(c, &cc, c->d_scan[0].p + N));
    CKS(fetch_u64(c, &mm, c->d_scan[1].p + N));
    CKS(fetch_u64(c, &xx, c->d_scan[2].p + N));
    CKS(sync_staged(c));
    if (cc > 0xffffffffull || mm > 0xfffffffeull || xx > 0xffffffffull) { c->err = "result arenas exceed 32-bit offsets"; return FQ_ELIMIT; }
  }
  const bool host_arrays = !(c->emit_flags & FQ_EMIT_DEVICE_ONLY) || c->debug;
  CKM(c->d_orec.ensure(N + 1) && c->d_ocig.ensure(cc + 1) && c->d_omd.ensure(mm + 1) && c->d_omulti.ensure(xx + 1));
  if (host_arrays) CKM(c->p_orec.ensure(N + 1) && c->p_ocig.ensure(cc + 1) && c->p_omd.ensure(mm + 1) && c->p_omulti.ensure(xx + 1));
  if (N) {
    A.o_rec = c->d_orec.p; A.o_cigar = c->d_ocig.p; A.o_md = c->d_omd.p; A.o_multi = c->d_omulti.p;
    REC(FQ_ROP_FLAT_FILL, N);
    if ((c->emit_flags & FQ_EMIT_SAM) || c->qc || c->bam) CKS(emit_measure(K));
    if (host_arrays) {
      CK(fqdev::copy_pinned(c->p_orec.p, c->d_orec.p, N * sizeof(fq_result_t), 0));
      CK(fqdev::copy_pinned(c->p_ocig.p, c->d_ocig.p, cc * 2, 0));
      CK(fqdev::copy_pinned(c->p_omd.p, c->d_omd.p, mm, 0));
      CK(fqdev::copy_pinned(c->p_omulti.p, c->d_omulti.p, xx * sizeof(fq_multi_t), 0));
      c->stats.d2h_bytes += N * sizeof(fq_result_t) + cc * 2 + mm + xx * sizeof(fq_multi_t);
    }
  }
  uint64_t cnt[FQ_C_COUNT];
  c->h_counters.resize((size_t)FQ_C_STRIPES * FQ_C_STRIDE);
  CKS(d2h_staged(c, c->h_counters.data(), c->d_counters.p, c->h_counters.size() * 8));
  CKS(sync_staged(c));
  fold_counters(c->h_counters.data(), cnt);
  CK(fqdev::dzero(c->d_counters.p, c->h_counters.size() * 8));
  if (!N && ((c->emit_flags & FQ_EMIT_SAM) || c->qc || c->bam)) CKS(emit_measure(K));
  if (host_arrays) {
    if (!cc) c->p_ocig.p[0] = 0;
    if (!mm) c->p_omd.p[0] = 0;
    if (!xx) c->p_omulti.p[0] = fq_multi_t{};
  }
  K.trace("result arrays D2H");
  if (cnt[FQ_C_ERR_DRAW0]) {
    c->err = "the drand48 stream drew exactly 0 for the first best hit of a read (once in 2^48 draws): bwa_aln2seq_core then takes no hit and the reference's "
             "record keeps the SA row of the read slot's previous occupant (libbwa/bwase.c:29-41) -- its result is undefined, and so this call is refused";
    return FQ_ELIMIT;
  }
  if (cnt[FQ_C_ERR_CIGAR]) { c->err = "refine: CIGAR longer than the device slot"; return FQ_ELIMIT; }
  if (cnt[FQ_C_ERR_MD]) { c->err = "MD string longer than the device slot"; return FQ_ELIMIT; }
  if (host_arrays) { S.rec = c->p_orec.p; S.cigar = c->p_ocig.p; S.md = c->p_omd.p; S.multi = c->p_omulti.p; }
  else { S.rec = nullptr; S.cigar = nullptr; S.md = nullptr; S.multi = nullptr; }
  S.n_both_unmapped = (int)cnt[FQ_C_UNMAPPED];
  out->n_survivors = n_surv;
  out->n_both_filtered = K.n - n_surv;
  out->n_both_unmapped = S.n_both_unmapped;
  out->pair_idx = S.pair_idx;
  out->rec = S.rec;
  out->cigar = S.cigar;
  out->md = S.md;
  out->multi = S.multi;
  out->isize = K.iis[n_sub - 1];
  out->n_sub = n_sub;
  out->isize_sub = S.isize_sub.data();
  out->n_bases = c->n_bases_in;
  fqdev::time_collect(c->stats.kernel_ms, c->stats.kernel_launches, FQ_K_COUNT);
  c->stats.occ_block_touches += cnt[FQ_C_OCC_WIDTH] + cnt[FQ_C_OCC_GAP] + cnt[FQ_C_OCC_SA];
  c->stats.gap_occ_touches += cnt[FQ_C_OCC_GAP];
  c->stats.width_occ_touches += cnt[FQ_C_OCC_WIDTH];
  c->stats.md_reads += cnt[FQ_C_MD_READS];
  c->stats.host_pairs += (uint64_t)K.n_host_pairs;
  c->stats.gap_nogap_touches += cnt[FQ_C_OCC_NOGAP];
  c->stats.filter_probes += cnt[FQ_C_PROBES];
  c->stats.stack_pops += cnt[FQ_C_POPS];
  c->stats.stack_pushes += cnt[FQ_C_PUSHES];
  if (cnt[FQ_C_MAXPOPS] > c->stats.max_pops_per_read) c->stats.max_pops_per_read = cnt[FQ_C_MAXPOPS];
  c->stats.reads_over_4k_pops += cnt[FQ_C_POPS_GT4K];
  if (cnt[FQ_C_MAXTRIPS] > c->stats.max_wave_trips) c->stats.max_wave_trips = cnt[FQ_C_MAXTRIPS];
  c->stats.wave_trips += cnt[FQ_C_SUMTRIPS];
  c->stats.lane_trips += cnt[FQ_C_LANETRIPS];
  c->stats.sa_rows += cnt[FQ_C_SA_DIRECT];
  c->stats.pairs_on_device += cnt[FQ_C_PAIRS_DEV];
  for (int k = 0; k < 16; ++k) c->stats.dbg[k] += cnt[FQ_C_DBG0 + k];
  c->stats.pairs += K.n;
  c->stats.host_ms_serial += (K.t_serial1 - K.t_host0) - (K.w_serial1 - K.w_host0);
  c->stats.host_ms_pair += (K.t_host1 - K.t_serial1) - (K.w_host1 - K.w_serial1);
  c->stats.host_ms_total += (K.t_host1 - K.t_host0) - (K.w_host1 - K.w_host0);
  c->stats.wall_ms_total += now_ms() - K.t_wall0;
  c->stats.device_wait_ms += c->wait_ms - K.w_call0;
  { timespec ts; clock_gettime(CLOCK_THREAD_CPUTIME_ID, &ts); c->stats.host_cpu_ms += 1e3 * (double)ts.tv_sec + 1e-6 * (double)ts.tv_nsec - K.cpu_call0; }
  K.trace("counters+timers");
  if ((c->emit_flags & FQ_EMIT_SAM) || c->qc || c->bam) CKS(emit_fill(K));
  return FQ_OK;
}
#undef REC

int run_call_stages(fq_ctx *c, fq_result_batch_t *out);
int run_call(fq_ctx *c, fq_result_batch_t *out) {
  c->serial_open = c->serial_done = false;
  const int rc = run_call_stages(c, out);
  if (rc && (c->before_serial || c->after_serial)) {
    c->stream_broken = true;
    if (!c->serial_open && !c->serial_done && c->before_serial) c->before_serial(c->hook_user);
    if (!c->serial_done && c->after_serial) c->after_serial(c->hook_user);
  }
  if (rc) {
    fqdev::copy_discard();
    (void)fqdev::stream_aux(0);
    (void)fqdev::dzero(c->d_counters.p, (size_t)FQ_C_STRIPES * FQ_C_STRIDE * 8);
    (void)fqdev::sync();
    (void)fqdev::copy_wait(0);
    (void)fqdev::copy_wait(1);
  }
  return rc;
}
int run_call_stages(fq_ctx *c, fq_result_batch_t *out) {
  CallInFlight in_flight(c->ix);
  Call K(c);
  K.t_trace = K.t_wall0 = now_ms();
  K.w_call0 = c->wait_ms;
  { timespec ts; clock_gettime(CLOCK_THREAD_CPUTIME_ID, &ts); K.cpu_call0 = 1e3 * (double)ts.tv_sec + 1e-6 * (double)ts.tv_nsec; }
  NodePin pin;
  struct PoolScope { FqWorkPool *prev; explicit PoolScope(FqWorkPool *p) : prev(tl_pool) { tl_pool = p; } ~PoolScope() { tl_pool = prev; } } pool_scope(&c->pool);
  (void)fqdev::stream_aux(0);
  const double grow = c->in_kind == 3 && c->tb && c->n_pairs > 0 && std::min<double>((double)c->max_pairs, (double)c->tb->pairs_behind) > (double)c->n_pairs
                          ? std::min(16.0, std::min<double>((double)c->max_pairs, (double)c->tb->pairs_behind) / (double)c->n_pairs) : 1.0;
  GrowScope grow_scope(grow);
  c->retired.next_call();
  RetiredScope retired_scope(&c->retired);
  if (c->kn.trace) { fprintf(stderr, "[fq]   arena: %zu blocks, last call used %zu bytes:", c->arena.blocks.size(), c->arena.total); for (auto &b : c->arena.blocks) fprintf(stderr, " %zu", b.cap); fprintf(stderr, "\n"); }
  c->arena.reset();
  const fq_opts_t &o = c->o;
  FqBatchState &S = c->st;
  S.clear();
  S.n_pairs = c->n_pairs;
  memset(out, 0, sizeof *out);
  out->n_pairs = c->n_pairs;
  if (c->n_pairs == 0) {
    const int rc0 = emit_measure(K);
    return rc0 ? rc0 : emit_fill(K);
  }
  K.n = c->n_pairs; K.n2 = 2 * K.n; K.B = o.batch_pairs; K.n_sub = (K.n + K.B - 1) / K.B;
  K.par_min = c->kn.host_par_min;
  K.host_threads = c->kn.host_threads >= 0 ? c->kn.host_threads : o.host_threads > 0 ? o.host_threads : default_host_threads(c->ix);
  int rc = c->in_kind == 3 ? stage0_text(K) : c->in_kind == 2 ? stage0_packed(K) : stage0_ascii(K);
  if (rc) return rc;
  S.n_surv = K.n_surv;
  S.batch_pairs = K.B;
  S.sub_lo = K.sub_lo;
  S.pair_idx = c->h_pair_list;
  S.surv = c->h_surv;
  K.trace("stage0 prep+compact");
  if ((rc = stageA_search(K))) return rc;
  K.trace("stageA width+gap");
  if ((rc = stage_records(K))) return rc;
  K.trace("records, SA plan, best-hit counts D2H");
  K.plan.n_chunks = ((size_t)K.n_surv + FQ_RNG_CHUNK_PAIRS - 1) / FQ_RNG_CHUNK_PAIRS;
  K.plan.start = (uint64_t *)c->arena.alloc((K.plan.n_chunks + 1) * 8);
  if (!K.plan.start) { c->err = "out of pinned host memory"; return FQ_ENOMEM; }
  if (!c->before_serial && (size_t)K.n_surv * 2 >= K.par_min) K.plan_thread = std::thread([&K, c] { stageB1_plan(K, c->rng); });
  if ((rc = stage_sa_rows(K))) return rc;
  K.trace("SA enumerate+kernel");
  K.t_host0 = now_ms(); K.w_host0 = c->wait_ms;
  if (c->before_serial) c->before_serial(c->hook_user);
  c->serial_open = true;
  if (c->stream_broken) { c->err = "the stream's state comes from a call that failed (on this rank or on the one before)"; return FQ_EIO; }
  if ((rc = stageB1_main_hit(K))) return rc;
  K.trace("B1 replay + main hit");
  if (o.single_end) K.iis.assign(K.n_sub, fq_isize_t{});
  else {
    stageB2_isize(K);
    c->last_ii = K.iis[K.n_sub - 1];
    if ((rc = stage_kl_cache(K))) return rc;
  }
  K.gate_take(c->qc);
  if (c->after_serial) c->after_serial(c->hook_user);
  c->serial_done = true;
  if (c->stream_broken) { c->err = "the hook that hands the stream's state on failed (fq_ctx_mark_stream_broken)"; return FQ_EIO; }
  K.t_serial1 = now_ms(); K.w_serial1 = c->wait_ms;
  K.trace("B2 isize, (k,l) cache");
  if ((rc = stageB3_pairing(K))) return rc;
  K.trace("B3 pairing+XA");
  if (c->debug && (rc = snapshot_records(K, S.stage_P))) return rc;
  if (!o.single_end && (rc = stageC_mate_sw(K))) return rc;
  K.trace("C mate SW");
  if (c->debug && (rc = snapshot_records(K, S.stage_S))) return rc;
  if ((rc = stageD_refine(K))) return rc;
  K.trace("D refine+MD");
  K.t_host1 = now_ms(); K.w_host1 = c->wait_ms;
  return stage_finish(K, out);
}
}

extern "C" int fq_host_cpus(void) { return (int)effective_cpus(); }
extern "C" int fq_runtime_configure(int hw_queues, int blocking_waits) { return fqdev::runtime_configure(hw_queues, blocking_waits); }
extern "C" int fq_device_count(void) { return fqdev::device_count(); }

extern "C" int fq_align_resident(fq_ctx_t *c, fq_result_batch_t *out) {
  if (!c || !out) return FQ_EINVAL;
  if (c->in_kind != 1) { c->err = "fq_align_resident: no batch uploaded (fq_batch_upload)"; return FQ_EINVAL; }
  if (fqdev::bind(c->dev)) return FQ_ENODEV;
  return run_call(c, out);
}

static int packed_check(fq_ctx_t *c, const fq_packed_batch_t *in) {
  if (!in || in->n_pairs < 0 || (in->n_pairs > 0 && (!in->head || !in->body || in->body_stride < 1 || (in->uniform_len <= 0 && !in->len)))) return FQ_EINVAL;
  if (in->n_exc < 0 || (in->n_exc > 0 && !in->exc)) return FQ_EINVAL;
  if (in->n_pairs > c->max_pairs) { c->err = "batch larger than max_pairs_per_batch"; return FQ_ELIMIT; }
  if (in->uniform_len > 0 && (in->uniform_len < FQ_LMIN || in->uniform_len > FQ_LMAX || (in->uniform_len + 3) / 4 > in->body_stride)) return refuse_length(c);
  if (c->o.trim_qual >= 1 && in->n_pairs > 0 && (!in->qual || in->qual_stride < 1)) { c->err = "quality trimming needs the batch's qualities"; return FQ_EINVAL; }
  if (in->n_pairs > 0 && in->qual_last && !in->qual) { c->err = "qual_last without the quality rows"; return FQ_EINVAL; }
  if ((in->single_end != 0) != (c->o.single_end != 0)) { c->err = c->o.single_end ? "a single-end context takes single-end batches (fq_pack_single_reads_into)" : "a paired-end context takes paired batches"; return FQ_EINVAL; }
  return FQ_OK;
}
extern "C" int fq_packed_prefetch(fq_ctx_t *c, const fq_packed_batch_t *next) {
  if (!c) return FQ_EINVAL;
  int rc = packed_check(c, next);
  if (rc) return rc;
  if (fqdev::bind(c->dev)) return FQ_ENODEV;
  if (next->n_pairs == 0 || c->is_pending(0, next) || c->is_pending(1, next)) return FQ_OK;
  for (int i = 0; i < 2; ++i) if (c->pend[i] == next) c->pend[i] = nullptr;
  const int slot = !c->pend[0] ? 0 : !c->pend[1] ? 1 : -1;
  if (slot < 0) return FQ_OK;
  rc = head_upload(c, next, slot);
  if (rc) return rc;
  c->pend[slot] = next; c->pend_serial[slot] = next->serial;
  return FQ_OK;
}
extern "C" int fq_packed_cancel(fq_ctx_t *c, const fq_packed_batch_t *b) {
  if (!c || !b) return FQ_EINVAL;
  for (int i = 0; i < 2; ++i)
    if (c->pend[i] == b) {
      if (fqdev::bind(c->dev)) return FQ_ENODEV;
      CK(fqdev::copy_wait(i));
      c->pend[i] = nullptr;
    }
  return FQ_OK;
}
extern "C" int fq_align_packed(fq_ctx_t *c, const fq_packed_batch_t *in, fq_result_batch_t *out) {
  if (!c || !out) return FQ_EINVAL;
  int rc = packed_check(c, in);
  if (rc) return broken_stream_call(c, rc);
  if (fqdev::bind(c->dev)) return FQ_ENODEV;
  c->pb = *in;
  c->n_pairs = in->n_pairs;
  c->in_kind = 2;
  if (in->n_pairs > 0) {
    if (c->is_pending(0, in)) { c->head_slot = 0; c->pend[0] = nullptr; }
    else if (c->is_pending(1, in)) { c->head_slot = 1; c->pend[1] = nullptr; }
    else {
      for (int i = 0; i < 2; ++i) if (c->pend[i] == in) c->pend[i] = nullptr;
      c->head_slot = !c->pend[0] ? 0 : 1;
      c->pend[c->head_slot] = nullptr;
      rc = head_upload(c, in, c->head_slot);
      if (rc) return broken_stream_call(c, rc);
    }
  }
  return run_call(c, out);
}

extern "C" int fq_stream_run(fq_ctx_t *const *ctxs, int32_t n_streams, const fq_packed_batch_t *const *const *batches, const int32_t *n_batches, const int32_t *first,
                             int32_t n_calls, int32_t flags, fq_stream_call_fn on_call, void *user, int64_t *survivors_out) {
  if (!ctxs || n_streams < 1 || !batches || !n_batches || n_calls < 0) return FQ_EINVAL;
  for (int s = 0; s < n_streams; ++s) if (!ctxs[s] || !batches[s] || n_batches[s] < 1) return FQ_EINVAL;
  for (int s = 0; s < n_streams; ++s) for (int t = 0; t < s; ++t) if (ctxs[s] == ctxs[t]) return FQ_EINVAL;
  std::vector<int> rcs((size_t)n_streams, FQ_OK);
  std::vector<int64_t> surv((size_t)n_streams, 0);
  static const bool trace_cpu = [] { const char *e = getenv("FASTQUICK_TRACE"); return e && *e && *e != '0'; }();
  std::vector<double> cpu_pre((size_t)n_streams, 0.0), cpu_call((size_t)n_streams, 0.0);
  auto thread_cpu_ms = [] { timespec ts; clock_gettime(CLOCK_THREAD_CPUTIME_ID, &ts); return 1e3 * (double)ts.tv_sec + 1e-6 * (double)ts.tv_nsec; };
  auto run = [&](int s) {
    fq_ctx_t *c = ctxs[s];
    const int nb = n_batches[s];
    int cur = (first ? first[s] : 0) % nb;
    if (cur < 0) cur += nb;
    fq_result_batch_t res;
    for (int k = 0; k < n_calls; ++k) {
      const int nxt = (cur + 1) % nb;
      int rc = FQ_OK;
      const bool pre = nxt != cur && (k + 1 < n_calls || (flags & FQ_STREAM_PREFETCH_BEYOND));
      const double c0 = trace_cpu ? thread_cpu_ms() : 0.0;
      if (pre) rc = fq_packed_prefetch(c, batches[s][nxt]);
      const double c1 = trace_cpu ? thread_cpu_ms() : 0.0;
      if (!rc) rc = fq_align_packed(c, batches[s][cur], &res);
      if (trace_cpu) { cpu_pre[(size_t)s] += c1 - c0; cpu_call[(size_t)s] += thread_cpu_ms() - c1; }
      if (!rc) { surv[(size_t)s] += res.n_survivors; if (on_call) rc = on_call(user, s, k, &res); }
      if (rc) { rcs[(size_t)s] = rc; if (pre) (void)fq_packed_cancel(c, batches[s][nxt]); return; }
      cur = nxt;
    }
  };
  std::vector<std::thread> th;
  for (int s = 1; s < n_streams; ++s) th.emplace_back(run, s);
  run(0);
  for (auto &t : th) t.join();
  if (survivors_out) for (int s = 0; s < n_streams; ++s) survivors_out[s] = surv[(size_t)s];
  if (trace_cpu && n_calls > 0) {
    double a = 0, b = 0;
    for (int s = 0; s < n_streams; ++s) { a += cpu_pre[(size_t)s]; b += cpu_call[(size_t)s]; }
    fprintf(stderr, "TRACE - fq_stream_run: %d streams x %d calls; CPU time of a stream's thread per call: prefetch %.3f ms, call %.3f ms\n", n_streams, n_calls,
            a / ((double)n_streams * n_calls), b / ((double)n_streams * n_calls));
  }
  for (int rc : rcs) if (rc) return rc;
  return FQ_OK;
}

extern "C" int fq_align_text(fq_ctx_t *c, const fq_text_batch *tb, fq_result_batch_t *out) {
  if (!c || !out || !tb) return FQ_EINVAL;
  int rc = FQ_OK;
  if (tb->n_pairs < 0 || (tb->n_pairs > 0 && (!tb->d_head || !tb->d_rec || !tb->d_text[0] || !tb->d_names))) rc = FQ_EINVAL;
  else if (tb->n_pairs > c->max_pairs) { c->err = "batch larger than max_pairs_per_batch"; rc = FQ_ELIMIT; }
  else if ((tb->single_end != 0) != (c->o.single_end != 0)) { c->err = "single-end / paired-end batch on a context of the other kind"; rc = FQ_EINVAL; }
  else if (tb->device != c->ix->device) { c->err = "the batch lives on another device than the context's index"; rc = FQ_EINVAL; }
  else if (tb->uniform_len > 0 && (tb->uniform_len < FQ_LMIN || tb->uniform_len > FQ_LMAX)) rc = refuse_length(c);
  if (rc) return broken_stream_call(c, rc);
  if (fqdev::bind(c->dev)) return FQ_ENODEV;
  c->tb = tb;
  c->n_pairs = tb->n_pairs;
  c->in_kind = 3;
  return run_call(c, out);
}

static const uint64_t kStateGood = 0x31545351465full, kStateBroken = 0x58545351465full;
extern "C" int64_t fq_ctx_state_export(const fq_ctx_t *c, void *buf, int64_t cap) {
  if (!c) return FQ_EINVAL;
  int64_t need = 8 + 8 + (int64_t)sizeof(fq_isize_t) + 8;
  for (const auto &kv : c->kl_cache) need += 16 + 4 * (int64_t)kv.second.size();
  if (!buf || cap < need) return need;
  uint8_t *p = (uint8_t *)buf;
  const uint64_t mark = c->stream_broken ? kStateBroken : kStateGood;
  memcpy(p, &mark, 8); p += 8;
  memcpy(p, &c->rng, 8); p += 8;
  memcpy(p, &c->last_ii, sizeof(fq_isize_t)); p += sizeof(fq_isize_t);
  const uint64_t n = c->kl_cache.size();
  memcpy(p, &n, 8); p += 8;
  for (const auto &kv : c->kl_cache) {
    const uint64_t m = kv.second.size();
// ... 145 lines not shown
```

### fastquick_amd/csrc/fq_backend.h

```cpp
#pragma once
#include "fq_kernels.h"
#include "fq_records.h"
#include "fq_frontend.h"
#include "fq_emit.h"
#include "fq_deflate.h"

namespace fqdev {

struct State;
struct Tune {
  int gap_coop_waves = 0;
  int gap_waves_per_cu = 0, gap_refill_min = 0, gap_order_asc = 0, filter_no_turns = 0, refine_lanes = 0;
  int spin_sync = 0;
  int gap_generic_opts = 0;
  int width_both_strands = 0;
  int prep_priority = 0;
  int sw_serial_reverse = 0;
};
int runtime_configure(int hw_queues, int blocking_waits);
int device_count();
State *state_create(int device_ordinal);
void state_destroy(State *s);
int bind(State *s);
Tune *tune(State *s);
const char *last_error();
bool is_real_gpu();
void device_turn_begin(int slots = 1);
void device_turn_end();

void *dmalloc(size_t bytes);
void dfree(void *p);
void *hmalloc(size_t bytes);
void hfree(void *p);
int h2d(void *dst, const void *src, size_t bytes);
int d2h(void *dst, const void *src, size_t bytes);
int copy_pinned(void *dst, const void *src, size_t bytes, int to_device);
int d2d(void *dst, const void *src, size_t bytes);
int dzero(void *dst, size_t bytes);
int dfill(void *dst, int byte, size_t bytes);
int sync();
int h2d_copy(void *dst, const void *src, size_t bytes);
int copy_record(int slot);
int copy_wait(int slot);
void copy_discard();
int compute_wait_copy(int slot);
int copy_flush_now();

void time_begin(int kid);
void time_end(int kid);
void time_collect(double ms[], uint64_t launches[], int n_ids);
inline thread_local uint64_t dp_launches[FQ_DP_COUNT] = {};

int launch_prep(const FqPrepArgs &a);
int launch_compact(const uint8_t *filtered, int n_pairs, int32_t *read_list, int32_t *sidx, int32_t *pair_list, int32_t *counts);
int launch_surv_gather(const int32_t *pair_list, int n_surv, int n_pairs, const int32_t *len_trim, const uint8_t *filtered, const int32_t *sidx, FqSurvInfo *out);
int launch_prep_packed(const FqPrepPackedArgs &a);
int launch_surv_map(const int32_t *pair_list, int n_surv, int n_pairs, const uint8_t *filtered, const int32_t *sidx, FqSurvInfo *out,
                    int32_t *row_map, int32_t *read_list_c, int32_t *crow_of);
int launch_unpack(const FqUnpackArgs &a);
int launch_patch(const FqPatchArgs &a);
int launch_trim(const FqTrimArgs &a);
int launch_trim_all(const FqTrimAllArgs &a);
int launch_width(const FqWidthArgs &a);
int launch_order(const uint8_t *bid_end, int n, int n_hard, int32_t *order, uint32_t *cnt);
int gap_lane_slots(const FqGapArgs &a);
int launch_gap(const FqGapArgs &a);
int launch_scan(const uint32_t *in, uint64_t *out, uint32_t n);
int launch_pack_aln(const FqAln *aln, const uint32_t *n_aln, const uint64_t *off, uint32_t cap, uint32_t n_work, FqAln *packed);
int launch_sa(const FqSaArgs &a);
int stream_aux(int on);
int stream_fork();
int stream_join();
int stream_mark(int k);
int stream_wait_mark(int k);
int launch_collect(const int32_t *order, const uint32_t *split, int n_work, int seg, int n_seg, const uint32_t *status, const int32_t *work, int32_t *out, uint32_t *count);
int launch_rec(int op, const FqRecArgs &a, int64_t n);
int launch_aln_index(const int32_t *work, const uint32_t *status, const uint64_t *off, const uint32_t *naln, uint64_t base, uint64_t *aoff, uint32_t *an, int n);
int launch_sam(int op, const FqSamArgs &a, int64_t n);
int launch_bam(int op, const FqBamArgs &a, int64_t n);
int launch_deflate(const FqDeflateArgs &a);
int launch_deflate_pack(const FqDeflatePackArgs &a);
int launch_qc(int op, const FqQcArgs &a, int64_t n);
int launch_dup_rehash(const uint64_t *old, uint64_t old_cap, uint64_t *tab, uint64_t mask);
int launch_sw(const FqSwArgs &a);
int launch_sw_serial(const FqSwArgs &a);
int launch_refine(const FqRefineArgs &a);

const FqzCrcConst *crc_const();
int launch_inflate(const FqInflateArgs &a);
int launch_inflate2(const FqInflateArgs &a, const FqInflateArgs &b);
int launch_nl_index(const uint8_t *text, uint32_t n, uint32_t lo, uint32_t *nl, uint32_t cap, uint32_t *count);
int launch_tok_rec(const FqTokArgs &a);
int launch_tok_pieces(const FqTokArgs &a);
int launch_slot_bases(const FqSlotArgs &a);
int launch_slot_names(const FqSlotArgs &a);
int launch_text_gather(const FqTextGatherArgs &a);
int launch_text_trim_all(const FqTextTrimArgs &a);
int dfill32(void *dst, uint32_t v, size_t n_words);

}
```

### fastquick_amd/csrc/fq_device.hip

```cpp
#include <hip/hip_runtime.h>
#include <hip/hip_ext.h>

#include <algorithm>
#include <condition_variable>
#include <atomic>
#include <cstdio>
#include <cstdlib>
#include <cstring>
#include <mutex>
#include <string>
#include <unordered_map>
#include <vector>
#include <sys/mman.h>
#include <sys/syscall.h>
#include <unistd.h>

#include "fq_backend.h"

namespace fqdev {

struct Pending { int kid; hipEvent_t a, b; };
struct State {
  int device = 0;
  hipStream_t stream = nullptr;
  hipStream_t main_stream = nullptr, aux_stream = nullptr;
  hipEvent_t fork_ev = nullptr, join_ev = nullptr;
  hipEvent_t marks[4] = {nullptr, nullptr, nullptr, nullptr};
  hipEvent_t prio_fork = nullptr;
  hipStream_t copy_stream = nullptr;
  hipEvent_t copy_done[2] = {nullptr, nullptr};
  hipEvent_t prep_done = nullptr;
  hipEvent_t sync_ev = nullptr;
  std::vector<Pending> pending;
  std::vector<hipEvent_t> free_events;
  hipEvent_t open_begin[16] = {};
  struct SmallCopy { uint8_t *dst; const uint8_t *src; size_t bytes; };
  SmallCopy small[8];
  int n_small = 0;
  uint64_t *scan_tmp = nullptr; size_t scan_tmp_n = 0;
  uint32_t *cmp_cnt = nullptr; uint64_t *cmp_off = nullptr; size_t cmp_n = 0;
  Tune tune;
};
static thread_local State *g_cur = nullptr;
static thread_local std::string g_err;
#define g_stream (g_cur->stream)

#define FQ_HIP(call)                                                                         \
  do {                                                                                       \
    hipError_t e_ = (call);                                                                  \
    if (e_ != hipSuccess) {                                                                  \
      g_err = std::string(#call) + ": " + hipGetErrorString(e_);                             \
      return -3;                                                                             \
    }                                                                                        \
  } while (0)

int copy_flush();
#define FQ_PRE() do { if (copy_flush()) return -3; } while (0)
void copy_discard() { if (g_cur) g_cur->n_small = 0; }
int copy_flush_now() { FQ_PRE(); return 0; }

const char *last_error() { return g_err.c_str(); }
bool is_real_gpu() { return true; }

static int set_kernel_attributes();
static std::mutex g_dev_mu;
static bool g_dev_ready[64];
static hipEvent_t g_prep_last[64];
static State *g_prep_owner[64];
static hipStream_t g_copy_streams[64][2];
static unsigned g_copy_next[64];
static std::mutex g_turn_mu[64];
static std::condition_variable g_turn_cv[64];
static int g_turn_held[64];
static int g_ctx_count[64];
static hipStream_t g_prio_stream[64];
static bool g_queue_warned = false;
static int g_rt_blocking_waits = 0;
int runtime_configure(int hw_queues, int blocking_waits) {
  if (hw_queues > 0) {
    char b[16];
    snprintf(b, sizeof b, "%d", hw_queues);
    setenv("GPU_MAX_HW_QUEUES", b, 0);
  }
  g_rt_blocking_waits = blocking_waits ? 1 : 0;
  return 0;
}

int device_count() { int n = 0; if (hipGetDeviceCount(&n) != hipSuccess) { (void)hipGetLastError(); return 0; } return n < 0 ? 0 : n; }
void device_turn_begin(int slots) {
  const int d = g_cur->device;
  std::unique_lock<std::mutex> lk(g_turn_mu[d]);
  g_turn_cv[d].wait(lk, [&] { return g_turn_held[d] < (slots < 1 ? 1 : slots); });
  ++g_turn_held[d];
}
void device_turn_end() {
  const int d = g_cur->device;
  { std::lock_guard<std::mutex> lk(g_turn_mu[d]); --g_turn_held[d]; }
  g_turn_cv[d].notify_all();
}

State *state_create(int dev) {
  int n = 0;
  if (hipGetDeviceCount(&n) != hipSuccess || n <= 0) { g_err = "no HIP device visible"; return nullptr; }
  if (dev < 0 || dev >= n || dev >= 64) { g_err = "device ordinal out of range"; return nullptr; }
  if (hipSetDevice(dev) != hipSuccess) { g_err = "hipSetDevice failed"; return nullptr; }
  g_cur = nullptr;
  {
    std::lock_guard<std::mutex> lk(g_dev_mu);
    if (!g_dev_ready[dev]) {
      if (g_rt_blocking_waits) { (void)hipSetDeviceFlags(hipDeviceScheduleBlockingSync); (void)hipGetLastError(); }
      if (set_kernel_attributes()) return nullptr;
      g_dev_ready[dev] = true;
    }
    const char *q = getenv("GPU_MAX_HW_QUEUES");
    const int queues = q && atoi(q) > 0 ? atoi(q) : 4;
    if (++g_ctx_count[dev] + 2 > queues && !g_queue_warned) {
      g_queue_warned = true;
      fprintf(stderr, "fastquick_amd: %d alignment contexts on device %d with GPU_MAX_HW_QUEUES=%d: contexts will share hardware queues and wait for each other's kernels "
                      "(fq_runtime_configure(contexts + 4, ..) or GPU_MAX_HW_QUEUES before the process makes its first HIP call)\n", g_ctx_count[dev], dev, queues);
    }
  }
  State *s = new State;
  s->device = dev;
  bool ok = hipStreamCreateWithFlags(&s->stream, hipStreamNonBlocking) == hipSuccess &&
            hipEventCreateWithFlags(&s->copy_done[0], hipEventDisableTiming | hipEventBlockingSync) == hipSuccess &&
            hipEventCreateWithFlags(&s->copy_done[1], hipEventDisableTiming | hipEventBlockingSync) == hipSuccess &&
            hipEventCreateWithFlags(&s->prep_done, hipEventDisableTiming) == hipSuccess &&
            hipEventCreateWithFlags(&s->sync_ev, hipEventDisableTiming | hipEventBlockingSync) == hipSuccess;
  if (!ok) { g_err = "stream / event creation failed"; state_destroy(s); return nullptr; }
  s->main_stream = s->stream;
  return s;
}
void state_destroy(State *s) {
  if (!s) return;
  (void)hipSetDevice(s->device);
  g_cur = nullptr;
  s->stream = s->main_stream ? s->main_stream : s->stream;
  if (s->aux_stream) { (void)hipStreamSynchronize(s->aux_stream); (void)hipStreamDestroy(s->aux_stream); }
  if (s->sync_ev) (void)hipEventDestroy(s->sync_ev);
  if (s->fork_ev) (void)hipEventDestroy(s->fork_ev);
  if (s->join_ev) (void)hipEventDestroy(s->join_ev);
  for (hipEvent_t m : s->marks) if (m) (void)hipEventDestroy(m);
  if (s->prio_fork) (void)hipEventDestroy(s->prio_fork);
  if (s->stream) (void)hipStreamSynchronize(s->stream);
  if (s->copy_stream) (void)hipStreamSynchronize(s->copy_stream);
  {
    std::lock_guard<std::mutex> lk(g_dev_mu);
    if (g_prep_owner[s->device] == s) { g_prep_owner[s->device] = nullptr; g_prep_last[s->device] = nullptr; }
    if (g_ctx_count[s->device] > 0) --g_ctx_count[s->device];
  }
  for (auto &p : s->pending) { (void)hipEventDestroy(p.a); (void)hipEventDestroy(p.b); }
  for (auto e : s->free_events) (void)hipEventDestroy(e);
  for (auto e : s->copy_done) if (e) (void)hipEventDestroy(e);
  if (s->prep_done) (void)hipEventDestroy(s->prep_done);
  if (s->scan_tmp) (void)hipFree(s->scan_tmp);
  if (s->cmp_cnt) (void)hipFree(s->cmp_cnt);
  if (s->cmp_off) (void)hipFree(s->cmp_off);
  if (s->stream) (void)hipStreamDestroy(s->stream);
  delete s;
}
Tune *tune(State *s) { return &s->tune; }
int bind(State *s) {
  if (!s) { g_err = "no device state"; return -3; }
  if (g_cur != s) { FQ_HIP(hipSetDevice(s->device)); g_cur = s; }
  return 0;
}

void *dmalloc(size_t bytes) {
  void *p = nullptr;
  if (hipMalloc(&p, bytes ? bytes : 16) != hipSuccess) { g_err = "hipMalloc failed (" + std::to_string(bytes) + " B)"; return nullptr; }
  return p;
}
void dfree(void *p) { if (p) (void)hipFree(p); }
static const size_t kRegisterMin = (size_t)4 << 20;
static std::mutex g_reg_mu;
static std::unordered_map<void *, size_t> g_registered;
static int device_numa_node(int dev) {
  static std::mutex mu;
  static std::unordered_map<int, int> cache;
  std::lock_guard<std::mutex> lk(mu);
  auto it = cache.find(dev);
  if (it != cache.end()) return it->second;
  int node = -1;
  char bus[64] = {0};
  if (hipDeviceGetPCIBusId(bus, (int)sizeof bus, dev) == hipSuccess) {
    for (char *c = bus; *c; ++c) if (*c >= 'A' && *c <= 'F') *c = (char)(*c - 'A' + 'a');
    const std::string path = std::string("/sys/bus/pci/devices/") + bus + "/numa_node";
    if (FILE *f = fopen(path.c_str(), "r")) { if (fscanf(f, "%d", &node) != 1) node = -1; fclose(f); }
  } else (void)hipGetLastError();
  cache[dev] = node;
  return node;
}
static void prefer_node(void *m, size_t len, int node) {
  if (node < 0 || node >= 1024) return;
  unsigned long mask[16] = {0};
  mask[node / (8 * sizeof(unsigned long))] |= 1ul << (node % (8 * sizeof(unsigned long)));
  (void)syscall(SYS_mbind, m, len, 1 , mask, (unsigned long)(8 * sizeof mask + 1), 0u);
}
void *hmalloc(size_t bytes) {
  static const bool use_register = [] { const char *e = getenv("FASTQUICK_PIN_REGISTER"); return !(e && *e == '0'); }();
  if (use_register && bytes >= kRegisterMin) {
    const size_t len = (bytes + ((size_t)2 << 20) - 1) & ~(((size_t)2 << 20) - 1);
    void *m = mmap(nullptr, len, PROT_READ | PROT_WRITE, MAP_PRIVATE | MAP_ANONYMOUS, -1, 0);
    if (m != MAP_FAILED) {
      (void)madvise(m, len, MADV_HUGEPAGE);
      int dev = 0;
      if (hipGetDevice(&dev) == hipSuccess) prefer_node(m, len, device_numa_node(dev)); else (void)hipGetLastError();
      if (hipHostRegister(m, len, hipHostRegisterDefault) == hipSuccess) {
        std::lock_guard<std::mutex> lk(g_reg_mu);
        g_registered[m] = len;
        return m;
      }
      (void)hipGetLastError();
      munmap(m, len);
    }
  }
  void *p = nullptr;
  if (hipHostMalloc(&p, bytes ? bytes : 16, hipHostMallocDefault) != hipSuccess) { g_err = "hipHostMalloc failed"; return nullptr; }
  return p;
}
void hfree(void *p) {
  if (!p) return;
  size_t len = 0;
  {
    std::lock_guard<std::mutex> lk(g_reg_mu);
    auto it = g_registered.find(p);
    if (it != g_registered.end()) { len = it->second; g_registered.erase(it); }
  }
  if (len) { (void)hipHostUnregister(p); munmap(p, len); }
  else (void)hipHostFree(p);
}
int h2d(void *dst, const void *src, size_t bytes) { FQ_PRE(); if (bytes) FQ_HIP(hipMemcpyAsync(dst, src, bytes, hipMemcpyHostToDevice, g_stream)); return 0; }
int d2h(void *dst, const void *src, size_t bytes) { FQ_PRE(); if (bytes) FQ_HIP(hipMemcpyAsync(dst, src, bytes, hipMemcpyDeviceToHost, g_stream)); return 0; }
int d2d(void *dst, const void *src, size_t bytes) { FQ_PRE(); if (bytes) FQ_HIP(hipMemcpyAsync(dst, src, bytes, hipMemcpyDeviceToDevice, g_stream)); return 0; }
int dzero(void *dst, size_t bytes) { FQ_PRE(); if (bytes) FQ_HIP(hipMemsetAsync(dst, 0, bytes, g_stream)); return 0; }
int dfill(void *dst, int byte, size_t bytes) { FQ_PRE(); if (bytes) FQ_HIP(hipMemsetAsync(dst, byte, bytes, g_stream)); return 0; }
int sync() {
  FQ_PRE();
  if (g_cur->tune.spin_sync || !g_cur->sync_ev) { FQ_HIP(hipStreamSynchronize(g_stream)); return 0; }
  FQ_HIP(hipEventRecord(g_cur->sync_ev, g_stream));
  FQ_HIP(hipEventSynchronize(g_cur->sync_ev));
  return 0;
}
int stream_aux(int on) {
  FQ_PRE();
  if (on && !g_cur->aux_stream) {
    FQ_HIP(hipStreamCreateWithFlags(&g_cur->aux_stream, hipStreamNonBlocking));
    FQ_HIP(hipEventCreateWithFlags(&g_cur->fork_ev, hipEventDisableTiming));
    FQ_HIP(hipEventCreateWithFlags(&g_cur->join_ev, hipEventDisableTiming));
  }
  g_cur->stream = on ? g_cur->aux_stream : g_cur->main_stream;
  return 0;
}
int stream_fork() {
  FQ_PRE();
  if (!g_cur->aux_stream) return 0;
  FQ_HIP(hipEventRecord(g_cur->fork_ev, g_cur->main_stream));
  FQ_HIP(hipStreamWaitEvent(g_cur->aux_stream, g_cur->fork_ev, 0));
  return 0;
}
int stream_join() {
  FQ_PRE();
  if (!g_cur->aux_stream) return 0;
  FQ_HIP(hipEventRecord(g_cur->join_ev, g_cur->aux_stream));
  FQ_HIP(hipStreamWaitEvent(g_cur->main_stream, g_cur->join_ev, 0));
  return 0;
}
int stream_mark(int k) {
  FQ_PRE();
  hipEvent_t &m = g_cur->marks[k & 3];
  if (!m) FQ_HIP(hipEventCreateWithFlags(&m, hipEventDisableTiming));
  FQ_HIP(hipEventRecord(m, g_stream));
  return 0;
}
int stream_wait_mark(int k) {
  FQ_PRE();
  hipEvent_t m = g_cur->marks[k & 3];
  if (m) FQ_HIP(hipStreamWaitEvent(g_stream, m, 0));
  return 0;
}
static int copy_stream_get() {
  if (g_cur->copy_stream) return 0;
  std::lock_guard<std::mutex> lk(g_dev_mu);
  const int dev = g_cur->device;
  for (int k = 0; k < 2; ++k)
    if (!g_copy_streams[dev][k]) FQ_HIP(hipStreamCreateWithFlags(&g_copy_streams[dev][k], hipStreamNonBlocking));
  g_cur->copy_stream = g_copy_streams[dev][g_copy_next[dev]++ & 1];
  return 0;
}
int h2d_copy(void *dst, const void *src, size_t bytes) {
  if (copy_stream_get()) return -3;
  if (bytes) FQ_HIP(hipMemcpyAsync(dst, src, bytes, hipMemcpyHostToDevice, g_cur->copy_stream));
  return 0;
}
int copy_record(int slot) { if (copy_stream_get()) return -3; FQ_HIP(hipEventRecord(g_cur->copy_done[slot & 1], g_cur->copy_stream)); return 0; }
int copy_wait(int slot) { FQ_HIP(hipEventSynchronize(g_cur->copy_done[slot & 1])); return 0; }
int compute_wait_copy(int slot) { FQ_PRE(); FQ_HIP(hipStreamWaitEvent(g_stream, g_cur->copy_done[slot & 1], 0)); return 0; }

struct FqCopySet { uint8_t *dst[8]; const uint8_t *src[8]; size_t bytes[8]; };
__global__ void __launch_bounds__(256) k_copy_bytes(FqCopySet cs) {
  uint8_t *dst = cs.dst[blockIdx.y];
  const uint8_t *src = cs.src[blockIdx.y];
  const size_t bytes = cs.bytes[blockIdx.y];
  const size_t n16 = ((((uintptr_t)dst | (uintptr_t)src) & 15) == 0) ? bytes / 16 : 0;
  const size_t t = (size_t)blockIdx.x * blockDim.x + threadIdx.x, stride = (size_t)gridDim.x * blockDim.x;
  for (size_t i = t; i < n16; i += stride) ((uint4 *)dst)[i] = ((const uint4 *)src)[i];
  for (size_t i = n16 * 16 + t; i < bytes; i += stride) dst[i] = src[i];
}
static const size_t kSmallCopy = (size_t)8 << 20;
int copy_flush() {
  State *s = g_cur;
  if (!s || s->n_small == 0) return 0;
  FqCopySet cs;
  size_t most = 0;
  for (int k = 0; k < 8; ++k) {
    const bool on = k < s->n_small;
    cs.dst[k] = on ? s->small[k].dst : nullptr; cs.src[k] = on ? s->small[k].src : nullptr; cs.bytes[k] = on ? s->small[k].bytes : 0;
    if (on) most = std::max(most, s->small[k].bytes);
  }
  const int n = s->n_small;
  s->n_small = 0;
  const unsigned blocks = (unsigned)std::min<size_t>(256, (most / 16 + 255) / 256 + 1);
  hipLaunchKernelGGL(k_copy_bytes, dim3(blocks, (unsigned)n), dim3(256), 0, s->stream, cs);
  FQ_HIP(hipGetLastError());
  return 0;
}
int copy_pinned(void *dst, const void *src, size_t bytes, int to_device) {
  if (!bytes) return 0;
  if (bytes > kSmallCopy) { FQ_PRE(); FQ_HIP(hipMemcpyAsync(dst, src, bytes, to_device ? hipMemcpyHostToDevice : hipMemcpyDeviceToHost, g_stream)); return 0; }
  if (g_cur->n_small == 8) FQ_PRE();
  g_cur->small[g_cur->n_small++] = {(uint8_t *)dst, (const uint8_t *)src, bytes};
  return 0;
}

static hipEvent_t get_event() {
  if (!g_cur->free_events.empty()) { hipEvent_t e = g_cur->free_events.back(); g_cur->free_events.pop_back(); return e; }
  hipEvent_t e;
  (void)hipEventCreate(&e);
  return e;
}
void time_begin(int kid) { (void)copy_flush(); hipEvent_t e = get_event(); (void)hipEventRecord(e, g_stream); g_cur->open_begin[kid] = e; }
void time_end(int kid) { (void)copy_flush(); hipEvent_t e = get_event(); (void)hipEventRecord(e, g_stream); g_cur->pending.push_back({kid, g_cur->open_begin[kid], e}); }
static void kernel_events(int kid, hipEvent_t *a, hipEvent_t *b) { *a = get_event(); *b = get_event(); g_cur->pending.push_back({kid, *a, *b}); }
void time_collect(double ms[], uint64_t launches[], int n_ids) {
  std::vector<decltype(g_cur->pending)::value_type> later;
  for (auto &p : g_cur->pending) {
    if (hipEventQuery(p.b) == hipErrorNotReady) { later.push_back(p); continue; }
    float t = 0.f;
    if (hipEventElapsedTime(&t, p.a, p.b) == hipSuccess && p.kid < n_ids) { ms[p.kid] += t; launches[p.kid] += 1; }
    g_cur->free_events.push_back(p.a);
    g_cur->free_events.push_back(p.b);
  }
  g_cur->pending.swap(later);
}

static inline unsigned nblk(uint64_t n, unsigned b) { return (unsigned)((n + b - 1) / b); }

__global__ void __launch_bounds__(256) k_prep(FqPrepArgs a) {
  const int r = blockIdx.x * blockDim.x + threadIdx.x;
  if (r < a.n_reads) fq_prep_thread(a, r);
}
extern __shared__ __align__(16) unsigned char fq_dyn_lds[];
__global__ void __launch_bounds__(256) k_width(FqWidthArgs a) {
  uint8_t *seed_bits = (uint8_t *)fq_dyn_lds;
  const int w = blockIdx.x * blockDim.x + threadIdx.x;
  if (w < a.n_work) fq_width_read(a, w, seed_bits + threadIdx.x, 256);
}
__global__ void __launch_bounds__(256) k_width_strand(FqWidthArgs a) {
  uint8_t *seed_bits = (uint8_t *)fq_dyn_lds;
  const int xcd = blockIdx.x & 7, strand = xcd >> 2;
  const int q = (int)(blockIdx.x >> 3) * 4 + (xcd & 3);
  const int w = q * 256 + threadIdx.x;
  if (w < a.n_work) fq_width_strand(a, w, strand, seed_bits + threadIdx.x, 256);
}
struct FqQueueFetch {
  uint32_t *cursor;
  int n_work;
  __device__ uint32_t operator()(uint32_t n) const { return atomicAdd(cursor, n); }
};
#if defined(FQ_GAP_WPE)
// ... 288 lines not shown
  const int t = blockIdx.x, lane = threadIdx.x;
  const FqRefineLds L(a.RL, a.QL);
  int *RM = (int *)(fq_dyn_lds + L.rM), *RI = (int *)(fq_dyn_lds + L.rI), *RD = (int *)(fq_dyn_lds + L.rD);
  uint8_t *ref = fq_dyn_lds + L.ref, *qry = fq_dyn_lds + L.qry, *ops = fq_dyn_lds + L.ops, *trace = fq_dyn_lds + L.trace;
  const FqRefTask T = a.task[t];
  const FqRefineWin w = fq_refine_window(a, T);
  fq_refine_fetch(a, T, w, qry, ref, lane, 64);
  __syncthreads();
  int n_ops = 0, fi, fj;
  fq_global_align_wave<true>(ref, w.l, qry, w.len, FQ_BAND, FQ_GAP_END, RM, RI, RD, trace, ops, &n_ops, &fi, &fj);
  if (lane == 0) fq_refine_emit(a, t, T, w.pos, ops, n_ops);
}
__global__ void __launch_bounds__(64) k_refine(FqRefineArgs a) {
  const int t = blockIdx.x * blockDim.x + threadIdx.x;
  if (t < a.n_task) fq_refine_thread(a, t);
}
__global__ void __launch_bounds__(256) k_pack_aln(const FqAln *aln, const uint32_t *n_aln, const uint64_t *off, uint32_t cap, uint32_t n_work, FqAln *packed) {
  const uint32_t w = blockIdx.x * blockDim.x + threadIdx.x;
  if (w >= n_work) return;
  const uint32_t n = n_aln[w];
  const uint64_t o = off[w];
  for (uint32_t j = 0; j < n; ++j) packed[o + j] = aln[(size_t)w * cap + j];
}

__device__ __forceinline__ uint32_t block_excl_scan(uint32_t v, uint32_t *total) {
  __shared__ uint32_t wsum[4];
  const int lane = threadIdx.x & 63, wid = threadIdx.x >> 6;
  uint32_t x = v;
#pragma unroll
  for (int d = 1; d < 64; d <<= 1) {
    const uint32_t y = __shfl_up(x, d, 64);
    if (lane >= d) x += y;
  }
  if (lane == 63) wsum[wid] = x;
  __syncthreads();
  uint32_t base = 0, tot = 0;
#pragma unroll
  for (int k = 0; k < 4; ++k) { if (k < wid) base += wsum[k]; tot += wsum[k]; }
  __syncthreads();
  *total = tot;
  return base + x - v;
}

__global__ void __launch_bounds__(256) k_scan_a(const uint32_t *in, uint32_t n, uint64_t *blk_tot) {
  const uint32_t i = blockIdx.x * 256 + threadIdx.x;
  uint32_t tot;
  (void)block_excl_scan(i < n ? in[i] : 0u, &tot);
  if (threadIdx.x == 0) blk_tot[blockIdx.x] = tot;
}
__global__ void __launch_bounds__(256) k_scan_b(uint64_t *blk_tot, uint32_t nb) {
  __shared__ uint64_t carry;
  if (threadIdx.x == 0) carry = 0;
  __syncthreads();
  for (uint32_t base = 0; base < nb; base += 256) {
    const uint32_t i = base + threadIdx.x;
    const uint64_t v = i < nb ? blk_tot[i] : 0;
    const int lane = threadIdx.x & 63, wid = threadIdx.x >> 6;
    __shared__ uint64_t ws[4];
    uint64_t x = v;
#pragma unroll
    for (int d = 1; d < 64; d <<= 1) {
      const uint64_t y = __shfl_up(x, d, 64);
      if (lane >= d) x += y;
    }
    if (lane == 63) ws[wid] = x;
    __syncthreads();
    uint64_t b = carry, tot = 0;
    for (int k = 0; k < 4; ++k) { if (k < wid) b += ws[k]; tot += ws[k]; }
    if (i < nb) blk_tot[i] = b + x - v;
    __syncthreads();
    if (threadIdx.x == 0) carry += tot;
    __syncthreads();
  }
  if (threadIdx.x == 0) blk_tot[nb] = carry;
}
__global__ void __launch_bounds__(256) k_scan_c(const uint32_t *in, uint32_t n, const uint64_t *blk_off, uint64_t *out) {
  const uint32_t i = blockIdx.x * 256 + threadIdx.x;
  uint32_t tot;
  const uint32_t e = block_excl_scan(i < n ? in[i] : 0u, &tot);
  if (i < n) out[i] = blk_off[blockIdx.x] + e;
  if (i == 0) out[n] = blk_off[gridDim.x];
}

#define g_scan_tmp (g_cur->scan_tmp)
#define g_scan_tmp_n (g_cur->scan_tmp_n)
int launch_scan(const uint32_t *in, uint64_t *out, uint32_t n) {
  FQ_PRE();
  if (n == 0) { uint64_t z = 0; return h2d(out, &z, 8) ? -3 : sync(); }
  const unsigned nb = nblk(n, 256);
  if (g_scan_tmp_n < nb + 1) {
    dfree(g_scan_tmp);
    g_scan_tmp_n = (size_t)nb * 2 + 64;
    g_scan_tmp = (uint64_t *)dmalloc(g_scan_tmp_n * 8);
    if (!g_scan_tmp) return -4;
  }
  hipLaunchKernelGGL(k_scan_a, dim3(nb), dim3(256), 0, g_stream, in, n, g_scan_tmp);
  hipLaunchKernelGGL(k_scan_b, dim3(1), dim3(256), 0, g_stream, g_scan_tmp, nb);
  hipLaunchKernelGGL(k_scan_c, dim3(nb), dim3(256), 0, g_stream, in, n, g_scan_tmp, out);
  FQ_HIP(hipGetLastError());
  return 0;
}

__global__ void __launch_bounds__(256) k_compact_a(const uint8_t *filt, int n_pairs, uint32_t *pair_cnt, uint32_t *read_cnt) {
  const int p = blockIdx.x * 256 + threadIdx.x;
  uint32_t keep = 0, nr = 0;
  if (p < n_pairs) {
    const uint32_t f0 = filt[p], f1 = filt[n_pairs + p];
    keep = !(f0 && f1);
    nr = (!f0) + (!f1);
  }
  const unsigned long long bal = __ballot(keep);
  __shared__ uint32_t s_pairs[4], s_reads[4];
  uint32_t x = nr;
#pragma unroll
  for (int d = 32; d >= 1; d >>= 1) x += __shfl_xor(x, d, 64);
  if ((threadIdx.x & 63) == 0) { s_pairs[threadIdx.x >> 6] = (uint32_t)__popcll(bal); s_reads[threadIdx.x >> 6] = x; }
  __syncthreads();
  if (threadIdx.x == 0) {
    pair_cnt[blockIdx.x] = s_pairs[0] + s_pairs[1] + s_pairs[2] + s_pairs[3];
    read_cnt[blockIdx.x] = s_reads[0] + s_reads[1] + s_reads[2] + s_reads[3];
  }
}
__global__ void __launch_bounds__(256) k_compact_c(const uint8_t *filt, int n_pairs, const uint64_t *pair_off, const uint64_t *read_off,
                                                   int32_t *read_list, int32_t *sidx, int32_t *pair_list, int32_t *counts) {
  const int p = blockIdx.x * 256 + threadIdx.x;
  uint32_t keep = 0, f0 = 1, f1 = 1;
  if (p < n_pairs) { f0 = filt[p]; f1 = filt[n_pairs + p]; keep = !(f0 && f1); }
  const uint32_t nr = (!f0) + (!f1);
  uint32_t tot_p, tot_r;
  const uint32_t rank_p = block_excl_scan(keep, &tot_p);
  const uint32_t rank_r = block_excl_scan(nr, &tot_r);
  if (p < n_pairs) {
    if (keep) pair_list[pair_off[blockIdx.x] + rank_p] = p;
    uint32_t s = (uint32_t)read_off[blockIdx.x] + rank_r;
    if (!f0) { read_list[s] = p; sidx[p] = (int32_t)s; ++s; } else sidx[p] = -1;
    if (!f1) { read_list[s] = n_pairs + p; sidx[n_pairs + p] = (int32_t)s; } else sidx[n_pairs + p] = -1;
  }
  if (p == 0) { counts[0] = (int32_t)read_off[gridDim.x]; counts[1] = (int32_t)pair_off[gridDim.x]; }
}
#define g_cmp_cnt (g_cur->cmp_cnt)
#define g_cmp_off (g_cur->cmp_off)
#define g_cmp_n (g_cur->cmp_n)
int launch_compact(const uint8_t *filtered, int n_pairs, int32_t *read_list, int32_t *sidx, int32_t *pair_list, int32_t *counts) {
  FQ_PRE();
  if (n_pairs <= 0) return dzero(counts, 8);
  const unsigned nb = nblk((uint64_t)n_pairs, 256);
  if (g_cmp_n < nb) {
    dfree(g_cmp_cnt); dfree(g_cmp_off);
    g_cmp_n = (size_t)nb * 2 + 64;
    g_cmp_cnt = (uint32_t *)dmalloc(g_cmp_n * 2 * 4);
    g_cmp_off = (uint64_t *)dmalloc((g_cmp_n + 2) * 2 * 8);
    if (!g_cmp_cnt || !g_cmp_off) return -4;
  }
  uint32_t *pc = g_cmp_cnt, *rc = g_cmp_cnt + g_cmp_n;
  uint64_t *po = g_cmp_off, *ro = g_cmp_off + g_cmp_n + 2;
  hipLaunchKernelGGL(k_compact_a, dim3(nb), dim3(256), 0, g_stream, filtered, n_pairs, pc, rc);
  int rc1 = launch_scan(pc, po, nb);
  if (rc1) return rc1;
  rc1 = launch_scan(rc, ro, nb);
  if (rc1) return rc1;
  hipLaunchKernelGGL(k_compact_c, dim3(nb), dim3(256), 0, g_stream, filtered, n_pairs, po, ro, read_list, sidx, pair_list, counts);
  FQ_HIP(hipGetLastError());
  return 0;
}

__global__ void __launch_bounds__(256) k_bitmap_scatter(uint8_t *bitmap, const uint32_t *bits, uint64_t n) {
  const uint64_t i = (uint64_t)blockIdx.x * blockDim.x + threadIdx.x;
  if (i >= n) return;
  const uint32_t x = bits[i];
  atomicOr((unsigned int *)(bitmap + ((x >> 5) << 2)), 1u << (x & 31));
}
int launch_bitmap_scatter(uint8_t *bitmap, const uint32_t *bits, uint64_t n) {
  FQ_PRE();
  if (!n) return 0;
  hipLaunchKernelGGL(k_bitmap_scatter, dim3(nblk(n, 256)), dim3(256), 0, g_stream, bitmap, bits, n);
  FQ_HIP(hipGetLastError());
  return 0;
}

__global__ void __launch_bounds__(256) k_bitmap_kmers(FqBitmapArgs a) {
  const int64_t idx = (int64_t)blockIdx.x * 256 + threadIdx.x;
  if (idx >= 2 * a.l_pac) return;
  fq_bitmap_kmer_thread(a, idx, [&](int t, uint32_t x) { atomicOr(&a.bitmap[t][x >> 5], 1u << (x & 31)); });
}
int launch_bitmap_kmers(const FqBitmapArgs &a) {
  FQ_PRE();
  if (a.l_pac <= 0 || a.n_rec <= 0) return 0;
  hipLaunchKernelGGL(k_bitmap_kmers, dim3(nblk((uint64_t)(2 * a.l_pac), 256)), dim3(256), 0, g_stream, a);
  FQ_HIP(hipGetLastError());
  return 0;
}

static FqzCrcConst *g_crc_const[64];
const FqzCrcConst *crc_const() {
  std::lock_guard<std::mutex> lk(g_dev_mu);
  const int dev = g_cur->device;
  if (!g_crc_const[dev]) {
    FqzCrcConst *h = new FqzCrcConst;
    fqz_crc_const_make(h);
    void *d = nullptr;
    if (hipMalloc(&d, sizeof(FqzCrcConst)) != hipSuccess || hipMemcpy(d, h, sizeof(FqzCrcConst), hipMemcpyHostToDevice) != hipSuccess) { g_err = "crc_const: hipMalloc / hipMemcpy failed"; delete h; return nullptr; }
    delete h;
    g_crc_const[dev] = (FqzCrcConst *)d;
  }
  return g_crc_const[dev];
}
#ifndef FQZ_WAVES_PER_EU
#define FQZ_WAVES_PER_EU 6
#endif
__global__ void __launch_bounds__(64) __attribute__((amdgpu_waves_per_eu(FQZ_WAVES_PER_EU))) k_inflate_bgzf(FqInflateArgs a, FqInflateArgs b) {
  __shared__ __attribute__((aligned(FQZ_RING))) FqzLds lds;
  const bool second = (int)blockIdx.x >= a.n_mem;
  const FqInflateArgs &A = second ? b : a;
  const int m = second ? (int)blockIdx.x - a.n_mem : (int)blockIdx.x;
  const uint32_t st = fqz_inflate_member(A, m, lds);
  if (threadIdx.x == 0) A.status[m] = st;
}
int launch_inflate2(const FqInflateArgs &a, const FqInflateArgs &b) {
  FQ_PRE();
  const int n = (a.n_mem > 0 ? a.n_mem : 0) + (b.n_mem > 0 ? b.n_mem : 0);
  if (n <= 0) return 0;
  FqInflateArgs x = a, y = b;
  if (x.n_mem < 0) x.n_mem = 0;
  if (y.n_mem < 0) y.n_mem = 0;
  hipLaunchKernelGGL(k_inflate_bgzf, dim3((unsigned)n), dim3(64), 0, g_stream, x, y);
// ... 83 lines not shown
}
__global__ void __launch_bounds__(256) k_tok_pieces(FqTokArgs a, int64_t n) {
  const int64_t g = (int64_t)blockIdx.x * 256 + threadIdx.x;
  if (g < n) fqt_piece_thread(a, g);
}
__global__ void __launch_bounds__(256) k_slot_bases(FqSlotArgs a) {
  const int s = blockIdx.x * 256 + threadIdx.x;
  if (s < a.n_slots) fqt_slot_bases_thread(a, s);
}
__global__ void __launch_bounds__(256) k_slot_names(FqSlotArgs a) {
  const int s = blockIdx.x * 256 + threadIdx.x;
  if (s < a.n_slots) fqt_slot_names_thread(a, s);
}
__global__ void __launch_bounds__(256) k_text_gather(FqTextGatherArgs a, int64_t n) {
  const int64_t g = (int64_t)blockIdx.x * 256 + threadIdx.x;
  if (g < n) fqt_gather_piece(a, g);
}
__global__ void __launch_bounds__(256) k_text_trim_all(FqTextTrimArgs a) {
  const int r = blockIdx.x * 256 + threadIdx.x;
  if (r < a.n_rows) fqt_trim_all_thread(a, r);
}
int launch_tok_rec(const FqTokArgs &a) {
  FQ_PRE();
  if (a.n_rec <= 0) return 0;
  hipLaunchKernelGGL(k_tok_rec, dim3(nblk((uint64_t)a.n_rec, 256)), dim3(256), 0, g_stream, a);
  FQ_HIP(hipGetLastError());
  return 0;
}
int launch_tok_pieces(const FqTokArgs &a) {
  FQ_PRE();
  const int64_t n = (int64_t)a.n_rec * ((a.max_len + 31) >> 5);
  if (n <= 0) return 0;
  hipLaunchKernelGGL(k_tok_pieces, dim3(nblk((uint64_t)n, 256)), dim3(256), 0, g_stream, a, n);
  FQ_HIP(hipGetLastError());
  return 0;
}
int launch_slot_bases(const FqSlotArgs &a) {
  FQ_PRE();
  if (a.n_rec <= 0) return 0;
  hipLaunchKernelGGL(k_slot_bases, dim3(nblk((uint64_t)a.n_slots, 256)), dim3(256), 0, g_stream, a);
  FQ_HIP(hipGetLastError());
  return 0;
}
__global__ void __launch_bounds__(256) k_names_plain(FqSlotArgs a) {
  const int i = blockIdx.x * 256 + threadIdx.x;
  if (i < a.n_rec) fqt_names_plain_thread(a, i);
}
int launch_slot_names(const FqSlotArgs &a) {
  FQ_PRE();
  if (a.n_rec <= 0) return 0;
  if (a.plain_names) {
    hipLaunchKernelGGL(k_names_plain, dim3(nblk((uint64_t)a.n_rec, 256)), dim3(256), 0, g_stream, a);
    if (a.mode != 0) { FQ_HIP(hipGetLastError()); return 0; }
  }
  hipLaunchKernelGGL(k_slot_names, dim3(nblk((uint64_t)a.n_slots, 256)), dim3(256), 0, g_stream, a);
  FQ_HIP(hipGetLastError());
  return 0;
}
int launch_text_gather(const FqTextGatherArgs &a) {
  FQ_PRE();
  const int64_t n = (int64_t)a.n_out * (a.stride >> 4);
  if (n <= 0) return 0;
  hipLaunchKernelGGL(k_text_gather, dim3(nblk((uint64_t)n, 256)), dim3(256), 0, g_stream, a, n);
  FQ_HIP(hipGetLastError());
  return 0;
}
int launch_text_trim_all(const FqTextTrimArgs &a) {
  FQ_PRE();
  if (a.n_rows <= 0) return 0;
  hipLaunchKernelGGL(k_text_trim_all, dim3(nblk((uint64_t)a.n_rows, 256)), dim3(256), 0, g_stream, a);
  FQ_HIP(hipGetLastError());
  return 0;
}
int dfill32(void *dst, uint32_t v, size_t n_words) { FQ_PRE(); if (n_words) FQ_HIP(hipMemsetD32Async((hipDeviceptr_t)dst, (int)v, n_words, g_stream)); return 0; }

int launch_prep(const FqPrepArgs &a) {
  FQ_PRE();
  if (a.n_reads <= 0) return 0;
  hipEvent_t e0, e1;
  kernel_events(FQ_K_PREP_KERNEL, &e0, &e1);
  if (!g_cur->tune.filter_no_turns) {
    const int dev = g_cur->device;
    std::lock_guard<std::mutex> lk(g_dev_mu);
    if (g_prep_last[dev] && g_prep_owner[dev] != g_cur) FQ_HIP(hipStreamWaitEvent(g_stream, g_prep_last[dev], 0));
    hipExtLaunchKernelGGL(k_prep, dim3(nblk((uint64_t)a.n_reads, 256)), dim3(256), 0, g_stream, e0, e1, 0, a);
    FQ_HIP(hipEventRecord(g_cur->prep_done, g_stream));
    g_prep_last[dev] = g_cur->prep_done; g_prep_owner[dev] = g_cur;
  } else {
    hipExtLaunchKernelGGL(k_prep, dim3(nblk((uint64_t)a.n_reads, 256)), dim3(256), 0, g_stream, e0, e1, 0, a);
  }
  FQ_HIP(hipGetLastError());
  return 0;
}
__global__ void __launch_bounds__(256) k_surv_gather(const int32_t *pair_list, int n_surv, int n_pairs, const int32_t *len_trim, const uint8_t *filtered, const int32_t *sidx, FqSurvInfo *out) {
  const int t = blockIdx.x * blockDim.x + threadIdx.x;
  if (t < 2 * n_surv) fq_surv_gather_thread(pair_list, n_pairs, len_trim, filtered, sidx, out, t);
}
int launch_surv_gather(const int32_t *pair_list, int n_surv, int n_pairs, const int32_t *len_trim, const uint8_t *filtered, const int32_t *sidx, FqSurvInfo *out) {
  FQ_PRE();
  if (n_surv <= 0) return 0;
  hipLaunchKernelGGL(k_surv_gather, dim3(nblk((uint64_t)n_surv * 2, 256)), dim3(256), 0, g_stream, pair_list, n_surv, n_pairs, len_trim, filtered, sidx, out);
  FQ_HIP(hipGetLastError());
  return 0;
}
__global__ void __launch_bounds__(256) k_prep_packed(FqPrepPackedArgs a) {
  const int r = blockIdx.x * blockDim.x + threadIdx.x;
  if (r < a.n_reads) fq_prep_packed_thread(a, r);
}
int launch_prep_packed(const FqPrepPackedArgs &a) {
  FQ_PRE();
  if (a.n_reads <= 0) return 0;
  hipEvent_t e0, e1;
  kernel_events(FQ_K_PREP_KERNEL, &e0, &e1);
  const dim3 grid(nblk((uint64_t)a.n_reads, 256));
  hipStream_t st = g_stream;
  if (g_cur->tune.prep_priority) {
    {
      std::lock_guard<std::mutex> lk(g_dev_mu);
      if (!g_prio_stream[g_cur->device]) {
        int lo = 0, hi = 0;
        FQ_HIP(hipDeviceGetStreamPriorityRange(&lo, &hi));
        FQ_HIP(hipStreamCreateWithPriority(&g_prio_stream[g_cur->device], hipStreamNonBlocking, hi));
      }
    }
    if (!g_cur->prio_fork) FQ_HIP(hipEventCreateWithFlags(&g_cur->prio_fork, hipEventDisableTiming));
    FQ_HIP(hipEventRecord(g_cur->prio_fork, g_stream));
    FQ_HIP(hipStreamWaitEvent(g_prio_stream[g_cur->device], g_cur->prio_fork, 0));
    st = g_prio_stream[g_cur->device];
  }
  if (!g_cur->tune.filter_no_turns) {
    const int dev = g_cur->device;
    std::lock_guard<std::mutex> lk(g_dev_mu);
    if (g_prep_last[dev] && g_prep_owner[dev] != g_cur) FQ_HIP(hipStreamWaitEvent(st, g_prep_last[dev], 0));
    hipExtLaunchKernelGGL(k_prep_packed, grid, dim3(256), 0, st, e0, e1, 0, a);
    FQ_HIP(hipEventRecord(g_cur->prep_done, st));
    g_prep_last[dev] = g_cur->prep_done; g_prep_owner[dev] = g_cur;
    if (st != g_stream) FQ_HIP(hipStreamWaitEvent(g_stream, g_cur->prep_done, 0));
  } else {
    hipExtLaunchKernelGGL(k_prep_packed, grid, dim3(256), 0, st, e0, e1, 0, a);
    if (st != g_stream) { FQ_HIP(hipEventRecord(g_cur->prep_done, st)); FQ_HIP(hipStreamWaitEvent(g_stream, g_cur->prep_done, 0)); }
  }
  FQ_HIP(hipGetLastError());
  return 0;
}
__global__ void __launch_bounds__(256) k_surv_map(const int32_t *pair_list, int n_surv, int n_pairs, const uint8_t *filtered, const int32_t *sidx, FqSurvInfo *out,
                                                  int32_t *row_map, int32_t *read_list_c, int32_t *crow_of) {
  const int t = blockIdx.x * blockDim.x + threadIdx.x;
  if (t < 2 * n_surv) fq_surv_map_thread(pair_list, n_pairs, filtered, sidx, out, row_map, read_list_c, crow_of, t);
}
int launch_surv_map(const int32_t *pair_list, int n_surv, int n_pairs, const uint8_t *filtered, const int32_t *sidx, FqSurvInfo *out,
                    int32_t *row_map, int32_t *read_list_c, int32_t *crow_of) {
  FQ_PRE();
  if (n_surv <= 0) return 0;
  hipLaunchKernelGGL(k_surv_map, dim3(nblk((uint64_t)n_surv * 2, 256)), dim3(256), 0, g_stream, pair_list, n_surv, n_pairs, filtered, sidx, out, row_map, read_list_c, crow_of);
  FQ_HIP(hipGetLastError());
  return 0;
}
__global__ void __launch_bounds__(256) k_unpack(FqUnpackArgs a) {
  const int64_t g = (int64_t)blockIdx.x * blockDim.x + threadIdx.x;
  if (g < (int64_t)a.n_rows * (a.stride >> 4)) fq_unpack_piece(a, g);
}
int launch_unpack(const FqUnpackArgs &a) {
  FQ_PRE();
  if (a.n_rows <= 0) return 0;
  if (a.stride & 15) { g_err = "launch_unpack: the compact row stride must be a multiple of 16"; return -1; }
  hipLaunchKernelGGL(k_unpack, dim3(nblk((uint64_t)a.n_rows * (uint64_t)(a.stride >> 4), 256)), dim3(256), 0, g_stream, a);
  FQ_HIP(hipGetLastError());
  return 0;
}
__global__ void __launch_bounds__(256) k_patch(FqPatchArgs a) {
  const int64_t q = (int64_t)blockIdx.x * blockDim.x + threadIdx.x;
  if (q < a.n_exc) fq_patch_thread(a, q);
}
int launch_patch(const FqPatchArgs &a) {
  FQ_PRE();
  if (a.n_exc <= 0) return 0;
  hipLaunchKernelGGL(k_patch, dim3(nblk((uint64_t)a.n_exc, 256)), dim3(256), 0, g_stream, a);
  FQ_HIP(hipGetLastError());
  return 0;
}
__global__ void __launch_bounds__(256) k_trim(FqTrimArgs a) {
  const int t = blockIdx.x * blockDim.x + threadIdx.x;
  if (t < a.n_rows) fq_trim_thread(a, t);
}
int launch_trim(const FqTrimArgs &a) {
  FQ_PRE();
  if (a.n_rows <= 0) return 0;
  hipLaunchKernelGGL(k_trim, dim3(nblk((uint64_t)a.n_rows, 256)), dim3(256), 0, g_stream, a);
  FQ_HIP(hipGetLastError());
  return 0;
}
__global__ void __launch_bounds__(256) k_trim_all(FqTrimAllArgs a) {
  const int r = blockIdx.x * blockDim.x + threadIdx.x;
  if (r < a.n_reads) fq_trim_all_thread(a, r);
}
int launch_trim_all(const FqTrimAllArgs &a) {
  FQ_PRE();
  if (a.n_reads <= 0) return 0;
  hipLaunchKernelGGL(k_trim_all, dim3(nblk((uint64_t)a.n_reads, 256)), dim3(256), 0, g_stream, a);
  FQ_HIP(hipGetLastError());
  return 0;
}
int launch_width(const FqWidthArgs &a) {
  FQ_PRE();
  if (a.n_work <= 0) return 0;
  hipEvent_t e0, e1;
  kernel_events(FQ_K_WIDTH_KERNEL, &e0, &e1);
  if (!g_cur->tune.width_both_strands) {
    const unsigned per_strand = nblk((uint64_t)a.n_work, 256);
    const unsigned grid = ((per_strand + 3) / 4) * 8;
    hipExtLaunchKernelGGL(k_width_strand, dim3(grid), dim3(256), (size_t)a.o.seed_len * 256, g_stream, e0, e1, 0, a);
  } else
  hipExtLaunchKernelGGL(k_width, dim3(nblk((uint64_t)a.n_work, 256)), dim3(256), (size_t)2 * (size_t)a.o.seed_len * 256, g_stream, e0, e1, 0, a);
  FQ_HIP(hipGetLastError());
  return 0;
}
__global__ void __launch_bounds__(256) k_order_count(const uint8_t *bid_end, int n, int n_hard, uint32_t *cnt) {
  __shared__ uint32_t h[FQ_ORDER_KEYS];
  if (threadIdx.x < FQ_ORDER_KEYS) h[threadIdx.x] = 0;
// ... 380 lines not shown
```

Baseline: 750.7 million.

## Run next batch's filter stage ahead on a separate stream with double-buffered slots

Result: slower. 631.9 million (-15.8%).

```diff
diff --git a/fastquick_amd/csrc/fq_align.cpp b/fastquick_amd/csrc/fq_align.cpp
--- a/fastquick_amd/csrc/fq_align.cpp
+++ b/fastquick_amd/csrc/fq_align.cpp
@@ -26,6 +26,12 @@
 
 using std::vector;
 
+namespace fqdev {
+__attribute__((weak)) int filter_ahead_begin(int) { return is_real_gpu() ? -3 : 0; }
+__attribute__((weak)) int filter_ahead_end(int) { return is_real_gpu() ? -3 : 0; }
+__attribute__((weak)) int filter_ahead_wait(int) { return is_real_gpu() ? -3 : 0; }
+}
+
 namespace {
 double now_ms() { return std::chrono::duration<double, std::milli>(std::chrono::steady_clock::now().time_since_epoch()).count(); }
 
@@ -181,6 +187,7 @@
   int64_t gap_nogap_min = 131072;
   uint32_t gap_pool = 2048;
   int gap_no_order = 0;
+  int filter_ahead = 1;
   int device_turns = 2;
   int device_turn_slots = 1;
   int64_t device_turn_min = 1 << 20;
@@ -248,8 +255,21 @@
   PinBuf<uint64_t> p_exc;
   PinBuf<uint16_t> p_hlen;
   DevBuf<uint16_t> d_blen;
-  DevBuf<uint8_t> d_seq, d_qual, d_filtered, d_maxdiff;
-  DevBuf<int32_t> d_len, d_len_trim, d_read_list, d_sidx, d_pair_list, d_counts;
+  DevBuf<uint8_t> d_seq, d_qual, d_maxdiff;
+  DevBuf<int32_t> d_len, d_len_trim;
+  struct FilterSlot {
+    DevBuf<uint8_t> d_filtered;
+    DevBuf<int32_t> d_read_list, d_sidx, d_pair_list, d_counts;
+    DevBuf<uint64_t> d_zeroed;
+    int32_t *d_sub_max = nullptr;
+    PinBuf<uint64_t> p_out;
+    bool ahead = false;
+    FqKOpts ko{}; int batch_pairs = 0, single_end = 0, n_pairs = 0;
+  } fs[2];
+  int fslot = 0;
+  bool call_ahead = false;
+  uint64_t call_probes = 0;
+  FilterSlot &flt() { return fs[fslot]; }
   DevBuf<uint64_t> d_counters;
   std::vector<uint64_t> h_counters;
   SearchBufs sb[2];
@@ -296,7 +316,6 @@
   PinBuf<uint32_t> p_u32a, p_u32b, p_pos;
   PinBuf<FqAln> p_aln;
   DevBuf<FqSurvInfo> d_surv;
-  DevBuf<int32_t> d_sub_max;
   int64_t n_bases_in = 0;
   int emit_flags = 0;
   bool host_rows = true;
@@ -378,7 +397,7 @@
   if (const char *e = getenv("FASTQUICK_CTX_TRACE")) c->kn.trace = atoi(e);
   c->dev = fqdev::state_create(ix->device);
   if (!c->dev || fqdev::bind(c->dev)) return FQ_ENODEV;
-  if (!c->d_maxdiff.ensure(FQ_LMAX + 2) || !c->d_counters.ensure(FQ_C_STRIPES * FQ_C_STRIDE) || !c->d_counts.ensure(4) || !c->sb[0].queue.ensure(4) || !c->d_glogn.ensure(256)) return FQ_ENOMEM;
+  if (!c->d_maxdiff.ensure(FQ_LMAX + 2) || !c->d_counters.ensure(FQ_C_STRIPES * FQ_C_STRIDE) || !c->sb[0].queue.ensure(4) || !c->d_glogn.ensure(256)) return FQ_ENOMEM;
   if (fqdev::h2d(c->d_maxdiff.p, c->maxdiff_lut, FQ_LMAX + 2) || fqdev::h2d(c->d_glogn.p, c->g_log_n, 256 * 4) || fqdev::dzero(c->d_counters.p, (size_t)FQ_C_STRIPES * FQ_C_STRIDE * 8) || fqdev::sync()) return FQ_ENODEV;
   *out = c.release();
   return FQ_OK;
@@ -413,6 +432,7 @@
   else if (k == "packed_bulk_min") c->kn.packed_bulk_min = v;
   else if (k == "md_mask_min") c->kn.md_mask_min = v;
   else if (k == "trace") c->kn.trace = (int)v;
+  else if (k == "filter_ahead") c->kn.filter_ahead = (int)v;
   else if (k == "gap_order_asc") t->gap_order_asc = (int)v;
   else if (k == "gap_waves_per_cu") t->gap_waves_per_cu = (int)v;
   else if (k == "gap_coop_waves") t->gap_coop_waves = (int)v;
@@ -739,6 +759,7 @@
 };
 
 struct FilterIn {
+  int n_pairs = 0;
   const uint64_t *head = nullptr;
   const uint16_t *len = nullptr;
   const uint8_t *qual_last = nullptr;
@@ -747,43 +768,78 @@
   const fq_text_batch *text = nullptr;
 };
 
-int stage0_filter(Call &K, const FilterIn &in) {
-  fq_ctx *c = K.c;
-  const int n = K.n, n2 = K.n2, n_sub = K.n_sub, B = K.B;
+static int filter_n_sub(const fq_ctx *c, int n) { return (n + c->o.batch_pairs - 1) / c->o.batch_pairs; }
+int filter_enqueue(fq_ctx *c, const FilterIn &in, int slot, bool ahead) {
+  fq_ctx::FilterSlot &F = c->fs[slot];
+  const int n = in.n_pairs, n2 = 2 * n, B = c->o.batch_pairs, n_sub = filter_n_sub(c, n);
   const bool ascii = !in.head, se = c->o.single_end != 0, ragged = !ascii && in.uniform_len <= 0;
   const int n_in = se ? n : n2;
-  const size_t n_max = (size_t)(ascii ? 1 : 3) * n_sub;
-  CKM(c->d_filtered.ensure(n2 + 64) && c->d_read_list.ensure(n2) && c->d_sidx.ensure(n2) && c->d_pair_list.ensure(n) && c->d_sub_max.ensure(n_max) && (!ascii || c->d_len_trim.ensure(n2)));
-  CK(fqdev::dzero(c->d_sub_max.p, n_max * 4));
-  if (se) CK(fqdev::dfill(c->d_filtered.p + n, 1, (size_t)n));
+  const size_t n_max = (size_t)(ascii ? 1 : 3) * n_sub, NC = (size_t)FQ_C_STRIPES * FQ_C_STRIDE;
+  CKM(F.d_filtered.ensure(n2 + 64) && F.d_read_list.ensure(n2) && F.d_sidx.ensure(n2) && F.d_pair_list.ensure(n) && F.d_counts.ensure(4) && F.d_zeroed.ensure(NC + (n_max + 1) / 2) &&
+      F.p_out.ensure(NC + 1 + (size_t)n_sub) && (!ascii || c->d_len_trim.ensure(n2)));
+  F.d_sub_max = (int32_t *)(F.d_zeroed.p + NC);
+  struct Ahead {
+    int slot; bool on = false;
+    ~Ahead() { if (on) (void)fqdev::filter_ahead_end(slot); }
+  } scope{slot};
+  if (ahead) { CK(fqdev::filter_ahead_begin(slot)); scope.on = true; }
+  CK(fqdev::dzero(F.d_zeroed.p, NC * 8 + n_max * 4));
+  if (se) CK(fqdev::dfill(F.d_filtered.p + n, 1, (size_t)n));
   if (se && ascii) CK(fqdev::dzero(c->d_len_trim.p + n, (size_t)n * 4));
   fqdev::time_begin(FQ_K_PREP);
   if (ascii) {
     FqPrepArgs a{};
     a.ix = c->ix->dev; a.o = c->ko; a.seq = c->d_seq.p; a.qual = c->d_qual.p; a.len = c->d_len.p; a.stride = c->stride; a.n_reads = n_in;
-    a.len_trim = c->d_len_trim.p; a.filtered = c->d_filtered.p; a.sub_max = c->d_sub_max.p; a.n_pairs = n; a.batch_pairs = B; a.counters = c->d_counters.p;
+    a.len_trim = c->d_len_trim.p; a.filtered = F.d_filtered.p; a.sub_max = F.d_sub_max; a.n_pairs = n; a.batch_pairs = B; a.counters = F.d_zeroed.p;
     CK(fqdev::launch_prep(a));
   } else {
     FqPrepPackedArgs a{};
-    a.ix = c->ix->dev; a.o = c->ko; a.head = in.head; a.len = ragged ? in.len : nullptr; a.uniform_len = in.uniform_len; a.qual_last = in.qual_last; a.sub_whole = c->d_sub_max.p + n_sub;
-    a.n_reads = n_in; a.filtered = c->d_filtered.p; a.sub_max = c->d_sub_max.p; a.n_pairs = n; a.batch_pairs = B; a.counters = c->d_counters.p;
+    a.ix = c->ix->dev; a.o = c->ko; a.head = in.head; a.len = ragged ? in.len : nullptr; a.uniform_len = in.uniform_len; a.qual_last = in.qual_last; a.sub_whole = F.d_sub_max + n_sub;
+    a.n_reads = n_in; a.filtered = F.d_filtered.p; a.sub_max = F.d_sub_max; a.n_pairs = n; a.batch_pairs = B; a.counters = F.d_zeroed.p;
     CK(fqdev::launch_prep_packed(a));
   }
-  CK(fqdev::launch_compact(c->d_filtered.p, n, c->d_read_list.p, c->d_sidx.p, c->d_pair_list.p, c->d_counts.p));
+  CK(fqdev::launch_compact(F.d_filtered.p, n, F.d_read_list.p, F.d_sidx.p, F.d_pair_list.p, F.d_counts.p));
   fqdev::time_end(FQ_K_PREP);
-  int32_t counts[2] = {0, 0};
+  int32_t *counts = (int32_t *)(F.p_out.p + NC), *sub_max = counts + 2, *sub_whole = sub_max + n_sub;
+  CK(fqdev::copy_pinned(F.p_out.p, F.d_zeroed.p, NC * 8, 0));
+  CK(fqdev::copy_pinned(counts, F.d_counts.p, 8, 0));
+  if (in.qual_last) CK(fqdev::copy_pinned(sub_whole, F.d_sub_max + n_sub, (size_t)n_sub * 4, 0));
+  if (ascii || ragged) CK(fqdev::copy_pinned(sub_max, F.d_sub_max, (size_t)n_sub * 4, 0));
+  if (ahead) {
+    scope.on = false;
+    CK(fqdev::filter_ahead_end(slot));
+    F.ahead = true; F.ko = c->ko; F.batch_pairs = B; F.single_end = se; F.n_pairs = n;
+  }
+  return FQ_OK;
+}
+void filter_drop(fq_ctx *c, int slot) {
+  if (!c->fs[slot].ahead) return;
+  (void)fqdev::filter_ahead_wait(slot);
+  c->fs[slot].ahead = false;
+}
+int filter_collect(Call &K, const FilterIn &in, int slot) {
+  fq_ctx *c = K.c;
+  fq_ctx::FilterSlot &F = c->fs[slot];
+  const int n = K.n, n2 = K.n2, n_sub = K.n_sub;
+  const bool ascii = !in.head, se = c->o.single_end != 0, ragged = !ascii && in.uniform_len <= 0;
+  const int n_in = se ? n : n2;
+  const size_t NC = (size_t)FQ_C_STRIPES * FQ_C_STRIDE;
+  if (c->call_ahead) {
+    c->call_ahead = false; F.ahead = false;
+    const double t_wait = now_ms();
+    CK(fqdev::filter_ahead_wait(slot));
+    c->wait_ms += now_ms() - t_wait;
+  } else CKS(sync_staged(c));
+  K.trace("  stage0: filter + compaction on the device");
+  const int32_t *counts = (const int32_t *)(F.p_out.p + NC), *sub_max = counts + 2, *sub_whole = sub_max + n_sub;
   c->h_sub_max.assign(n_sub, in.uniform_len);
   K.sub_whole.assign(n_sub, 0);
-  std::vector<uint64_t> striped(ragged ? (size_t)FQ_C_STRIPES * FQ_C_STRIDE : 0);
-  CKS(d2h_staged(c, counts, c->d_counts.p, 8));
-  if (in.qual_last) CKS(d2h_staged(c, K.sub_whole.data(), c->d_sub_max.p + n_sub, (size_t)n_sub * 4));
-  if (ascii || ragged) CKS(d2h_staged(c, c->h_sub_max.data(), c->d_sub_max.p, (size_t)n_sub * 4));
-  if (ragged) CKS(d2h_staged(c, striped.data(), c->d_counters.p, striped.size() * 8));
-  CKS(sync_staged(c));
-  K.trace("  stage0: filter + compaction on the device");
+  if (in.qual_last) K.sub_whole.assign(sub_whole, sub_whole + n_sub);
+  if (ascii || ragged) c->h_sub_max.assign(sub_max, sub_max + n_sub);
+  uint64_t folded[FQ_C_COUNT];
+  fold_counters(F.p_out.p, folded);
+  c->call_probes = folded[FQ_C_PROBES];
   if (ragged) {
-    uint64_t folded[FQ_C_COUNT];
-    fold_counters(striped.data(), folded);
     if (folded[FQ_C_BADLEN]) return refuse_length(c);
     for (int sb = 0; in.body_stride && sb < n_sub; ++sb)
       if (((int64_t)c->h_sub_max[sb] + 3) / 4 > (int64_t)in.body_stride) { c->err = "a read is longer than body_stride holds"; return FQ_EINVAL; }
@@ -793,12 +849,17 @@
   K.dstride = ascii ? c->stride : (std::max(1, *std::max_element(c->h_sub_max.begin(), c->h_sub_max.end())) + 15) & ~15;
   return FQ_OK;
 }
+int stage0_filter(Call &K, const FilterIn &in, int slot) {
+  K.c->fslot = slot;
+  if (!K.c->call_ahead) { filter_drop(K.c, slot); CKS(filter_enqueue(K.c, in, slot, false)); }
+  return filter_collect(K, in, slot);
+}
 
 int stage0_debug_fetch(fq_ctx *c, int n2, const int32_t *d_len_all) {
   c->h_filtered.clear(); c->h_len_trim.clear();
   if (!c->debug) return FQ_OK;
   c->h_filtered.resize(n2);
-  CKS(d2h_staged(c, c->h_filtered.data(), c->d_filtered.p, n2));
+  CKS(d2h_staged(c, c->h_filtered.data(), c->flt().d_filtered.p, n2));
   if (d_len_all) { c->h_len_trim.resize(n2); CKS(d2h_staged(c, c->h_len_trim.data(), d_len_all, (size_t)n2 * 4)); }
   return FQ_OK;
 }
@@ -809,11 +870,11 @@
   CKM(c->d_surv.ensure(nrow + 1));
   if (compact) {
     CKM(c->d_row_map.ensure(nrow + 1) && c->d_len_c.ensure(nrow + 1) && c->d_len_trim.ensure(nrow + 1));
-    CK(fqdev::launch_surv_map(c->d_pair_list.p, n_surv, K.n, c->d_filtered.p, c->d_sidx.p, c->d_surv.p, c->d_row_map.p, c->d_read_list.p, crow));
-  } else CK(fqdev::launch_surv_gather(c->d_pair_list.p, n_surv, K.n, c->d_len_trim.p, c->d_filtered.p, c->d_sidx.p, c->d_surv.p));
+    CK(fqdev::launch_surv_map(c->flt().d_pair_list.p, n_surv, K.n, c->flt().d_filtered.p, c->flt().d_sidx.p, c->d_surv.p, c->d_row_map.p, c->flt().d_read_list.p, crow));
+  } else CK(fqdev::launch_surv_gather(c->flt().d_pair_list.p, n_surv, K.n, c->d_len_trim.p, c->flt().d_filtered.p, c->flt().d_sidx.p, c->d_surv.p));
   if (!compact) CKS(stage0_debug_fetch(c, K.n2, c->d_len_trim.p));
   CKM(c->p_pairs.ensure((size_t)n_surv + 1) && c->p_surv.ensure(nrow + 1));
-  CK(fqdev::copy_pinned(c->p_pairs.p, c->d_pair_list.p, (size_t)n_surv * 4, 0));
+  CK(fqdev::copy_pinned(c->p_pairs.p, c->flt().d_pair_list.p, (size_t)n_surv * 4, 0));
   CK(fqdev::copy_pinned(c->p_surv.p, c->d_surv.p, nrow * sizeof(FqSurvInfo), 0));
   CKS(sync_staged(c));
   c->stats.d2h_bytes += (size_t)n_surv * (4 + 2 * sizeof(FqSurvInfo));
@@ -830,7 +891,7 @@
   fq_ctx *c = K.c;
   FqTrimArgs ta{};
   ta.o = c->ko; ta.qual = qual; ta.qual_stride = qual_stride; ta.row_map = row_map; ta.len = c->d_len_c.p; ta.n_rows = 2 * K.n_surv; ta.len_trim = c->d_len_trim.p;
-  ta.pair_list = c->d_pair_list.p; ta.batch_pairs = K.B; ta.sub_max = c->d_sub_max.p + 2 * K.n_sub;
+  ta.pair_list = c->flt().d_pair_list.p; ta.batch_pairs = K.B; ta.sub_max = c->flt().d_sub_max + 2 * K.n_sub;
   return ta;
 }
 
@@ -951,7 +1012,7 @@
   if (nrow) {
     FqTextGatherArgs g{};
     g.text[0] = tb.d_text[0]; g.text[1] = tb.d_text[1]; g.rec = tb.d_rec; g.names = tb.d_names; g.name_stride = ns; g.n_pairs = K.n; g.single_end = c->o.single_end ? 1 : 0;
-    g.pair_list = c->d_pair_list.p; g.n_out = nrow; g.seq = c->d_seq.p; g.qual = c->d_pqual.p; g.stride = cstride;
+    g.pair_list = c->flt().d_pair_list.p; g.n_out = nrow; g.seq = c->d_seq.p; g.qual = c->d_pqual.p; g.stride = cstride;
     g.len_out = c->d_len_c.p; g.len_trim = c->d_len_trim.p; g.names_out = c->d_cnames.p;
     CK(fqdev::launch_text_gather(g));
     if (c->o.trim_qual >= 1) CK(fqdev::launch_trim(stage0_trim_args(K, c->d_pqual.p, cstride, nullptr)));
@@ -977,7 +1038,7 @@
   if (trim && !tb) {
     vector<int32_t> surv_max(n_sub, 0);
     if (nrow) {
-      CKS(d2h_staged(c, surv_max.data(), c->d_sub_max.p + 2 * n_sub, (size_t)n_sub * 4));
+      CKS(d2h_staged(c, surv_max.data(), c->flt().d_sub_max + 2 * n_sub, (size_t)n_sub * 4));
       CKS(sync_staged(c));
       c->stats.d2h_bytes += (size_t)n_sub * 4;
     }
@@ -994,20 +1055,20 @@
       CK(fqdev::h2d(c->d_pqual.p, c->pb.qual, (size_t)n_in * c->pb.qual_stride));
       c->stats.h2d_bytes += (size_t)n_in * c->pb.qual_stride;
     }
-    CK(fqdev::dzero(c->d_sub_max.p, (size_t)n_sub * 4));
+    CK(fqdev::dzero(c->flt().d_sub_max, (size_t)n_sub * 4));
     if (se) CK(fqdev::dzero(c->d_len_all.p + n, (size_t)n * 4));
     if (tb) {
       FqTextTrimArgs aa{};
       aa.o = c->ko; aa.text[0] = tb->d_text[0]; aa.text[1] = tb->d_text[1]; aa.rec = tb->d_rec; aa.n_rows = n_in; aa.n_pairs = n; aa.batch_pairs = K.B;
-      aa.len_trim = c->d_len_all.p; aa.sub_max = c->d_sub_max.p;
+      aa.len_trim = c->d_len_all.p; aa.sub_max = c->flt().d_sub_max;
       CK(fqdev::launch_text_trim_all(aa));
     } else {
       FqTrimAllArgs aa{};
       aa.o = c->ko; aa.qual = c->d_pqual.p; aa.qual_stride = c->pb.qual_stride; aa.len = ragged ? in.len : nullptr; aa.uniform_len = in.uniform_len;
-      aa.n_reads = n_in; aa.n_pairs = n; aa.batch_pairs = K.B; aa.len_trim = c->d_len_all.p; aa.sub_max = c->d_sub_max.p;
+      aa.n_reads = n_in; aa.n_pairs = n; aa.batch_pairs = K.B; aa.len_trim = c->d_len_all.p; aa.sub_max = c->flt().d_sub_max;
       CK(fqdev::launch_trim_all(aa));
     }
-    CKS(d2h_staged(c, c->h_sub_max.data(), c->d_sub_max.p, (size_t)n_sub * 4));
+    CKS(d2h_staged(c, c->h_sub_max.data(), c->flt().d_sub_max, (size_t)n_sub * 4));
   }
   CKS(stage0_debug_fetch(c, n2, need_all ? c->d_len_all.p : nullptr));
   if (tb) c->h_len_all.clear();
@@ -1028,24 +1089,33 @@
     K.sub_max_len[sb] = std::max(1, c->h_sub_max[sb]);
     K.max_len_all = std::max(K.max_len_all, K.sub_max_len[sb]);
   }
-  K.dseq = c->d_seq.p; K.dlen_trim = c->d_len_trim.p; K.dread_list = c->d_read_list.p;
-}
-
+  K.dseq = c->d_seq.p; K.dlen_trim = c->d_len_trim.p; K.dread_list = c->flt().d_read_list.p;
+}
+
+static int free_filter_slot(const fq_ctx *c) { return !c->fs[0].ahead ? 0 : !c->fs[1].ahead ? 1 : 0; }
 int stage0_ascii(Call &K) {
-  CKS(stage0_filter(K, FilterIn{}));
+  FilterIn in;
+  in.n_pairs = K.n;
+  K.c->call_ahead = false;
+  CKS(stage0_filter(K, in, free_filter_slot(K.c)));
   CKS(stage0_survivors(K, false, nullptr));
   stage0_finish(K);
   return FQ_OK;
+}
+FilterIn packed_filter_in(fq_ctx *c, const fq_packed_batch_t &pb, int slot) {
+  FilterIn in;
+  in.n_pairs = pb.n_pairs;
+  in.head = c->d_head[slot].p; in.len = c->d_hlen[slot].p; in.uniform_len = pb.uniform_len; in.body_stride = pb.body_stride;
+  in.qual_last = c->o.trim_qual >= 1 && pb.qual_last ? c->d_qlast[slot].p : nullptr;
+  return in;
 }
 int stage0_packed(Call &K) {
   fq_ctx *c = K.c;
   const fq_packed_batch_t &pb = c->pb;
   const int slot = c->head_slot;
   CK(fqdev::compute_wait_copy(slot));
-  FilterIn in;
-  in.head = c->d_head[slot].p; in.len = c->d_hlen[slot].p; in.uniform_len = pb.uniform_len; in.body_stride = pb.body_stride;
-  in.qual_last = c->o.trim_qual >= 1 && pb.qual_last ? c->d_qlast[slot].p : nullptr;
-  CKS(stage0_filter(K, in));
+  const FilterIn in = packed_filter_in(c, pb, slot);
+  CKS(stage0_filter(K, in, slot));
   const int64_t bulk_min = c->kn.packed_bulk_min >= 0 ? c->kn.packed_bulk_min : (int64_t)K.n / 8;
   const bool bulk = !c->o.single_end && K.n_surv > 0 && (int64_t)K.n_surv >= bulk_min;
   const bool need_crow = bulk && pb.n_exc > 0;
@@ -1059,8 +1129,10 @@
 int stage0_text(Call &K) {
   fq_ctx *c = K.c;
   FilterIn in;
+  in.n_pairs = K.n;
   in.head = c->tb->d_head; in.len = c->tb->d_hlen; in.uniform_len = c->tb->uniform_len; in.text = c->tb;
-  CKS(stage0_filter(K, in));
+  c->call_ahead = false;
+  CKS(stage0_filter(K, in, free_filter_slot(c)));
   CKS(stage0_survivors(K, true, nullptr));
   CKS(stage0_rows_text(K));
   CKS(stage0_whole_batch(K, in));
@@ -1327,7 +1399,7 @@
   A.ix = c->ix->dev; A.n_surv = n_surv; A.n_pairs = K.n; A.batch_pairs = K.B; A.packed = c->in_kind >= 2 ? 1 : 0 ; A.single_end = o.single_end ? 1 : 0;
   A.max_occ = o.max_occ; A.multi_cap = o.single_end ? 4u : (uint32_t)std::max(o.n_multi, o.N_multi) + 1;
   A.n_multi = o.n_multi; A.N_multi = o.N_multi; A.max_isize = o.max_isize; A.s_mm = o.s_mm; A.is_sw = o.is_sw;
-  A.pair_list = c->d_pair_list.p; A.surv = c->d_surv.p; A.len_trim = K.dlen_trim; A.full_len = A.packed ? c->d_len_c.p : c->d_len.p;
+  A.pair_list = c->flt().d_pair_list.p; A.surv = c->d_surv.p; A.len_trim = K.dlen_trim; A.full_len = A.packed ? c->d_len_c.p : c->d_len.p;
   A.hits = c->d_hits.p; A.aoff = c->d_aoff.p; A.an = c->d_an.p; A.maxdiff_lut = c->d_maxdiff.p; A.g_log_n = c->d_glogn.p;
   A.rec = c->d_rec.p; A.nocc = c->d_nocc.p; A.ntop = c->d_ntop.p; A.enumerated = c->d_enum.p; A.qfirst = c->d_qfirst.p; A.row0 = c->d_row0.p;
   A.pq_cnt = c->d_cnt[0].p; A.prow_cnt = c->d_cnt[1].p; A.pq = c->d_scan[0].p; A.prow = c->d_scan[1].p;
@@ -1876,7 +1948,7 @@
     e = FqSamArgs{};
     e.cg = c->ix->dev_contigs;
     e.n_surv = K.n_surv; e.n_pairs = K.n; e.packed = K.ra.packed; e.single_end = c->o.single_end; e.mode = c->o.mode; e.max_top2 = c->o.max_top2;
-    e.pair_list = c->d_pair_list.p;
+    e.pair_list = c->flt().d_pair_list.p;
     e.rec = c->d_orec.p; e.cigar = c->d_ocig.p; e.md = c->d_omd.p; e.multi = c->d_omulti.p;
     e.seq = K.ra.seq; e.stride = K.ra.stride;
     CKS(emit_reads(K, &e.qual, &e.qual_stride, &e.names, &e.name_stride));
@@ -2075,7 +2147,7 @@
   c->stats.md_reads += cnt[FQ_C_MD_READS];
   c->stats.host_pairs += (uint64_t)K.n_host_pairs;
   c->stats.gap_nogap_touches += cnt[FQ_C_OCC_NOGAP];
-  c->stats.filter_probes += cnt[FQ_C_PROBES];
+  c->stats.filter_probes += c->call_probes;
   c->stats.stack_pops += cnt[FQ_C_POPS];
   c->stats.stack_pushes += cnt[FQ_C_PUSHES];
   if (cnt[FQ_C_MAXPOPS] > c->stats.max_pops_per_read) c->stats.max_pops_per_read = cnt[FQ_C_MAXPOPS];
@@ -2113,6 +2185,8 @@
     (void)fqdev::stream_aux(0);
     (void)fqdev::dzero(c->d_counters.p, (size_t)FQ_C_STRIPES * FQ_C_STRIDE * 8);
     (void)fqdev::sync();
+    for (int i = 0; i < 2; ++i) filter_drop(c, i);
+    c->call_ahead = false;
     (void)fqdev::copy_wait(0);
     (void)fqdev::copy_wait(1);
   }
@@ -2223,12 +2297,14 @@
   if (rc) return rc;
   if (fqdev::bind(c->dev)) return FQ_ENODEV;
   if (next->n_pairs == 0 || c->is_pending(0, next) || c->is_pending(1, next)) return FQ_OK;
-  for (int i = 0; i < 2; ++i) if (c->pend[i] == next) c->pend[i] = nullptr;
+  for (int i = 0; i < 2; ++i) if (c->pend[i] == next) { c->pend[i] = nullptr; filter_drop(c, i); }
   const int slot = !c->pend[0] ? 0 : !c->pend[1] ? 1 : -1;
   if (slot < 0) return FQ_OK;
+  filter_drop(c, slot);
   rc = head_upload(c, next, slot);
   if (rc) return rc;
   c->pend[slot] = next; c->pend_serial[slot] = next->serial;
+  if (c->kn.filter_ahead) return filter_enqueue(c, packed_filter_in(c, *next, slot), slot, true);
   return FQ_OK;
 }
 extern "C" int fq_packed_cancel(fq_ctx_t *c, const fq_packed_batch_t *b) {
@@ -2237,6 +2313,7 @@
     if (c->pend[i] == b) {
       if (fqdev::bind(c->dev)) return FQ_ENODEV;
       CK(fqdev::copy_wait(i));
+      filter_drop(c, i);
       c->pend[i] = nullptr;
     }
   return FQ_OK;
@@ -2250,12 +2327,18 @@
   c->n_pairs = in->n_pairs;
   c->in_kind = 2;
   if (in->n_pairs > 0) {
-    if (c->is_pending(0, in)) { c->head_slot = 0; c->pend[0] = nullptr; }
-    else if (c->is_pending(1, in)) { c->head_slot = 1; c->pend[1] = nullptr; }
-    else {
-      for (int i = 0; i < 2; ++i) if (c->pend[i] == in) c->pend[i] = nullptr;
+    c->call_ahead = false;
+    if (c->is_pending(0, in) || c->is_pending(1, in)) {
+      const int slot = c->is_pending(0, in) ? 0 : 1;
+      c->head_slot = slot; c->pend[slot] = nullptr;
+      const fq_ctx::FilterSlot &F = c->fs[slot];
+      c->call_ahead = F.ahead && !memcmp(&F.ko, &c->ko, sizeof c->ko) && F.batch_pairs == c->o.batch_pairs && F.single_end == (c->o.single_end != 0) && F.n_pairs == in->n_pairs;
+      if (!c->call_ahead) filter_drop(c, slot);
+    } else {
+      for (int i = 0; i < 2; ++i) if (c->pend[i] == in) { c->pend[i] = nullptr; filter_drop(c, i); }
       c->head_slot = !c->pend[0] ? 0 : 1;
       c->pend[c->head_slot] = nullptr;
+      filter_drop(c, c->head_slot);
       rc = head_upload(c, in, c->head_slot);
       if (rc) return broken_stream_call(c, rc);
     }
diff --git a/fastquick_amd/csrc/fq_backend.h b/fastquick_amd/csrc/fq_backend.h
--- a/fastquick_amd/csrc/fq_backend.h
+++ b/fastquick_amd/csrc/fq_backend.h
@@ -45,6 +45,9 @@
 void copy_discard();
 int compute_wait_copy(int slot);
 int copy_flush_now();
+int filter_ahead_begin(int slot);
+int filter_ahead_end(int slot);
+int filter_ahead_wait(int slot);
 
 void time_begin(int kid);
 void time_end(int kid);
diff --git a/fastquick_amd/csrc/fq_device.hip b/fastquick_amd/csrc/fq_device.hip
--- a/fastquick_amd/csrc/fq_device.hip
+++ b/fastquick_amd/csrc/fq_device.hip
@@ -37,8 +37,13 @@
   struct SmallCopy { uint8_t *dst; const uint8_t *src; size_t bytes; };
   SmallCopy small[8];
   int n_small = 0;
-  uint64_t *scan_tmp = nullptr; size_t scan_tmp_n = 0;
-  uint32_t *cmp_cnt = nullptr; uint64_t *cmp_off = nullptr; size_t cmp_n = 0;
+  struct Scratch { uint64_t *scan_tmp = nullptr; size_t scan_tmp_n = 0; uint32_t *cmp_cnt = nullptr; uint64_t *cmp_off = nullptr; size_t cmp_n = 0; } scr[2];
+  int scr_cur = 0;
+  bool ahead = false;
+  hipStream_t own_stream = nullptr;
+  hipStream_t filter_stream = nullptr;
+  hipEvent_t ahead_fork = nullptr;
+  hipEvent_t filter_done[2] = {nullptr, nullptr};
   Tune tune;
 };
 static thread_local State *g_cur = nullptr;
@@ -67,6 +72,9 @@
 static bool g_dev_ready[64];
 static hipEvent_t g_prep_last[64];
 static State *g_prep_owner[64];
+static hipStream_t g_prep_stream[64];
+static hipStream_t g_filter_stream[64];
+static std::mutex g_filter_mu[64];
 static hipStream_t g_copy_streams[64][2];
 static unsigned g_copy_next[64];
 static std::mutex g_turn_mu[64];
@@ -144,6 +152,7 @@
   if (s->prio_fork) (void)hipEventDestroy(s->prio_fork);
   if (s->stream) (void)hipStreamSynchronize(s->stream);
   if (s->copy_stream) (void)hipStreamSynchronize(s->copy_stream);
+  if (s->filter_stream) (void)hipStreamSynchronize(s->filter_stream);
   {
     std::lock_guard<std::mutex> lk(g_dev_mu);
     if (g_prep_owner[s->device] == s) { g_prep_owner[s->device] = nullptr; g_prep_last[s->device] = nullptr; }
@@ -153,9 +162,13 @@
   for (auto e : s->free_events) (void)hipEventDestroy(e);
   for (auto e : s->copy_done) if (e) (void)hipEventDestroy(e);
   if (s->prep_done) (void)hipEventDestroy(s->prep_done);
-  if (s->scan_tmp) (void)hipFree(s->scan_tmp);
-  if (s->cmp_cnt) (void)hipFree(s->cmp_cnt);
-  if (s->cmp_off) (void)hipFree(s->cmp_off);
+  if (s->ahead_fork) (void)hipEventDestroy(s->ahead_fork);
+  for (auto e : s->filter_done) if (e) (void)hipEventDestroy(e);
+  for (auto &t : s->scr) {
+    if (t.scan_tmp) (void)hipFree(t.scan_tmp);
+    if (t.cmp_cnt) (void)hipFree(t.cmp_cnt);
+    if (t.cmp_off) (void)hipFree(t.cmp_off);
+  }
   if (s->stream) (void)hipStreamDestroy(s->stream);
   delete s;
 }
@@ -296,6 +309,56 @@
 int copy_record(int slot) { if (copy_stream_get()) return -3; FQ_HIP(hipEventRecord(g_cur->copy_done[slot & 1], g_cur->copy_stream)); return 0; }
 int copy_wait(int slot) { FQ_HIP(hipEventSynchronize(g_cur->copy_done[slot & 1])); return 0; }
 int compute_wait_copy(int slot) { FQ_PRE(); FQ_HIP(hipStreamWaitEvent(g_stream, g_cur->copy_done[slot & 1], 0)); return 0; }
+
+static int prio_stream_get(int dev) {
+  if (g_prio_stream[dev]) return 0;
+  int lo = 0, hi = 0;
+  FQ_HIP(hipDeviceGetStreamPriorityRange(&lo, &hi));
+  FQ_HIP(hipStreamCreateWithPriority(&g_prio_stream[dev], hipStreamNonBlocking, hi));
+  return 0;
+}
+int filter_ahead_begin(int slot) {
+  FQ_PRE();
+  State *s = g_cur;
+  const int dev = s->device;
+  if (s->ahead) { g_err = "filter_ahead_begin: already on the filter stream"; return -3; }
+  if (!s->ahead_fork) FQ_HIP(hipEventCreateWithFlags(&s->ahead_fork, hipEventDisableTiming));
+  for (auto &e : s->filter_done) if (!e) FQ_HIP(hipEventCreateWithFlags(&e, hipEventDisableTiming | hipEventBlockingSync));
+  hipStream_t fs = nullptr;
+  {
+    std::lock_guard<std::mutex> lk(g_dev_mu);
+    if (s->tune.prep_priority) { if (prio_stream_get(dev)) return -3; fs = g_prio_stream[dev]; }
+    else {
+      if (!g_filter_stream[dev]) FQ_HIP(hipStreamCreateWithFlags(&g_filter_stream[dev], hipStreamNonBlocking));
+      fs = g_filter_stream[dev];
+    }
+  }
+  if (s->filter_stream && s->filter_stream != fs) FQ_HIP(hipStreamSynchronize(s->filter_stream));
+  FQ_HIP(hipEventRecord(s->ahead_fork, s->main_stream));
+  g_filter_mu[dev].lock();
+  hipError_t e = hipStreamWaitEvent(fs, s->ahead_fork, 0);
+  if (e == hipSuccess) e = hipStreamWaitEvent(fs, s->copy_done[slot & 1], 0);
+  if (e != hipSuccess) { g_filter_mu[dev].unlock(); g_err = std::string("filter_ahead_begin: ") + hipGetErrorString(e); return -3; }
+  s->filter_stream = fs;
+  s->own_stream = s->stream; s->stream = fs; s->scr_cur = 1; s->ahead = true;
+  return 0;
+}
+int filter_ahead_end(int slot) {
+  State *s = g_cur;
+  if (!s || !s->ahead) return 0;
+  int rc = copy_flush();
+  s->n_small = 0;
+  const hipError_t e = hipEventRecord(s->filter_done[slot & 1], s->stream);
+  s->stream = s->own_stream; s->scr_cur = 0; s->ahead = false;
+  g_filter_mu[s->device].unlock();
+  if (e != hipSuccess) { g_err = std::string("filter_ahead_end: ") + hipGetErrorString(e); rc = -3; }
+  return rc;
+}
+int filter_ahead_wait(int slot) {
+  if (!g_cur->filter_done[slot & 1]) return 0;
+  FQ_HIP(hipEventSynchronize(g_cur->filter_done[slot & 1]));
+  return 0;
+}
 
 struct FqCopySet { uint8_t *dst[8]; const uint8_t *src[8]; size_t bytes[8]; };
 __global__ void __launch_bounds__(256) k_copy_bytes(FqCopySet cs) {
@@ -750,8 +813,8 @@
   if (i == 0) out[n] = blk_off[gridDim.x];
 }
 
-#define g_scan_tmp (g_cur->scan_tmp)
-#define g_scan_tmp_n (g_cur->scan_tmp_n)
+#define g_scan_tmp (g_cur->scr[g_cur->scr_cur].scan_tmp)
+#define g_scan_tmp_n (g_cur->scr[g_cur->scr_cur].scan_tmp_n)
 int launch_scan(const uint32_t *in, uint64_t *out, uint32_t n) {
   FQ_PRE();
   if (n == 0) { uint64_t z = 0; return h2d(out, &z, 8) ? -3 : sync(); }
@@ -806,9 +869,9 @@
   }
   if (p == 0) { counts[0] = (int32_t)read_off[gridDim.x]; counts[1] = (int32_t)pair_off[gridDim.x]; }
 }
-#define g_cmp_cnt (g_cur->cmp_cnt)
-#define g_cmp_off (g_cur->cmp_off)
-#define g_cmp_n (g_cur->cmp_n)
+#define g_cmp_cnt (g_cur->scr[g_cur->scr_cur].cmp_cnt)
+#define g_cmp_off (g_cur->scr[g_cur->scr_cur].cmp_off)
+#define g_cmp_n (g_cur->scr[g_cur->scr_cur].cmp_n)
 int launch_compact(const uint8_t *filtered, int n_pairs, int32_t *read_list, int32_t *sidx, int32_t *pair_list, int32_t *counts) {
   FQ_PRE();
   if (n_pairs <= 0) return dzero(counts, 8);
@@ -1058,10 +1121,10 @@
   if (!g_cur->tune.filter_no_turns) {
     const int dev = g_cur->device;
     std::lock_guard<std::mutex> lk(g_dev_mu);
-    if (g_prep_last[dev] && g_prep_owner[dev] != g_cur) FQ_HIP(hipStreamWaitEvent(g_stream, g_prep_last[dev], 0));
+    if (g_prep_last[dev] && (g_prep_owner[dev] != g_cur || g_prep_stream[dev] != g_stream)) FQ_HIP(hipStreamWaitEvent(g_stream, g_prep_last[dev], 0));
     hipExtLaunchKernelGGL(k_prep, dim3(nblk((uint64_t)a.n_reads, 256)), dim3(256), 0, g_stream, e0, e1, 0, a);
     FQ_HIP(hipEventRecord(g_cur->prep_done, g_stream));
-    g_prep_last[dev] = g_cur->prep_done; g_prep_owner[dev] = g_cur;
+    g_prep_last[dev] = g_cur->prep_done; g_prep_owner[dev] = g_cur; g_prep_stream[dev] = g_stream;
   } else {
     hipExtLaunchKernelGGL(k_prep, dim3(nblk((uint64_t)a.n_reads, 256)), dim3(256), 0, g_stream, e0, e1, 0, a);
   }
@@ -1090,27 +1153,23 @@
   kernel_events(FQ_K_PREP_KERNEL, &e0, &e1);
   const dim3 grid(nblk((uint64_t)a.n_reads, 256));
   hipStream_t st = g_stream;
-  if (g_cur->tune.prep_priority) {
+  if (g_cur->tune.prep_priority && !g_cur->ahead) {
     {
       std::lock_guard<std::mutex> lk(g_dev_mu);
-      if (!g_prio_stream[g_cur->device]) {
-        int lo = 0, hi = 0;
-        FQ_HIP(hipDeviceGetStreamPriorityRange(&lo, &hi));
-        FQ_HIP(hipStreamCreateWithPriority(&g_prio_stream[g_cur->device], hipStreamNonBlocking, hi));
-      }
+      if (prio_stream_get(g_cur->device)) return -3;
     }
     if (!g_cur->prio_fork) FQ_HIP(hipEventCreateWithFlags(&g_cur->prio_fork, hipEventDisableTiming));
     FQ_HIP(hipEventRecord(g_cur->prio_fork, g_stream));
     FQ_HIP(hipStreamWaitEvent(g_prio_stream[g_cur->device], g_cur->prio_fork, 0));
     st = g_prio_stream[g_cur->device];
   }
-  if (!g_cur->tune.filter_no_turns) {
+  if (!g_cur->tune.filter_no_turns || g_cur->ahead) {
     const int dev = g_cur->device;
     std::lock_guard<std::mutex> lk(g_dev_mu);
-    if (g_prep_last[dev] && g_prep_owner[dev] != g_cur) FQ_HIP(hipStreamWaitEvent(st, g_prep_last[dev], 0));
+    if (g_prep_last[dev] && (g_prep_owner[dev] != g_cur || g_prep_stream[dev] != st)) FQ_HIP(hipStreamWaitEvent(st, g_prep_last[dev], 0));
     hipExtLaunchKernelGGL(k_prep_packed, grid, dim3(256), 0, st, e0, e1, 0, a);
     FQ_HIP(hipEventRecord(g_cur->prep_done, st));
-    g_prep_last[dev] = g_cur->prep_done; g_prep_owner[dev] = g_cur;
+    g_prep_last[dev] = g_cur->prep_done; g_prep_owner[dev] = g_cur; g_prep_stream[dev] = st;
     if (st != g_stream) FQ_HIP(hipStreamWaitEvent(g_stream, g_cur->prep_done, 0));
   } else {
     hipExtLaunchKernelGGL(k_prep_packed, grid, dim3(256), 0, st, e0, e1, 0, a);
```
